# GATB/dsk

Hardware: AMD Instinct MI355X
Metric: distinct k-mers counted/sec (whole node), k=31 (higher is better)
Workload: dtype u64

## Files before the change

### dsk_amd/csrc/dskgpu.hip

```cpp
#include <algorithm>
#include <cstdio>
#include <cstring>
#include <cstdlib>
#include <cmath>
#include <string>
#include <vector>

#include <thread>
#include <system_error>
#include "engine.h"
#include "kernels.h"
#include "superkmer_recv.h"
#include "rawparse.h"

#include <rocprim/device/device_radix_sort.hpp>

#define DSKGPU_VERSION "dskgpu 0.1 (gfx950)"

namespace {

thread_local std::string g_create_err;

__global__ __launch_bounds__(1024) void k_place_probe(unsigned long long* __restrict__ out, unsigned long long n) {
    const unsigned long long per_block = n / gridDim.x, per_stream = per_block / 512;
    unsigned long long* base = out + (unsigned long long)blockIdx.x * per_block;
    const int r = threadIdx.x >> 5, l = threadIdx.x & 31;
    for (unsigned long long off = 0; off + 32 <= per_stream; off += 32)
        for (int p = r; p < 512; p += 32) base[(unsigned long long)p * per_stream + off + l] = off;
}
int g_place_k = -1;
float place_probe_ms(void* p, size_t bytes) {
    hipEvent_t a, b;
    if (hipEventCreate(&a) != hipSuccess || hipEventCreate(&b) != hipSuccess) return 0.f;
    float best = 1e30f;
    for (int i = 0; i < 3; ++i) {
        (void)hipEventRecord(a, 0);
        hipLaunchKernelGGL(k_place_probe, dim3(256), dim3(1024), 0, 0, static_cast<unsigned long long*>(p), (unsigned long long)(bytes / 8));
        (void)hipEventRecord(b, 0);
        (void)hipEventSynchronize(b);
        float ms = 0.f; (void)hipEventElapsedTime(&ms, a, b);
        if (i && ms < best) best = ms;
    }
    (void)hipEventDestroy(a); (void)hipEventDestroy(b);
    return best;
}
}

hipError_t placed_malloc(void** out, size_t bytes) {
    if (g_place_k < 0) { const char* e = getenv("DSKGPU_PLACE"); g_place_k = e ? atoi(e) : 0; }
    size_t free_b = 0, total_b = 0;
    if (g_place_k < 2 || bytes < (size_t(1) << 28) || hipMemGetInfo(&free_b, &total_b) != hipSuccess) return hipMalloc(out, bytes);
    const int K = (int)std::min<size_t>((size_t)g_place_k, free_b / 2 / bytes);
    if (K < 2) return hipMalloc(out, bytes);
    std::vector<void*> cand; std::vector<float> ms;
    for (int i = 0; i < K; ++i) {
        void* q = nullptr;
        if (hipMalloc(&q, bytes) != hipSuccess) { (void)hipGetLastError(); break; }
        static const size_t probe_max = getenv("DSKGPU_PLACE_GB") ? (size_t)(atof(getenv("DSKGPU_PLACE_GB")) * (1ull << 30)) : ~size_t(0);
        cand.push_back(q); ms.push_back(place_probe_ms(q, std::min(bytes, probe_max)));
    }
    if (cand.empty()) return hipErrorOutOfMemory;
    size_t best = 0;
    for (size_t i = 1; i < cand.size(); ++i) if (ms[i] < ms[best]) best = i;
    for (size_t i = 0; i < cand.size(); ++i) if (i != best) (void)hipFree(cand[i]);
    if (getenv("DSKGPU_VERBOSE")) {
        fprintf(stderr, "[dskgpu] placement of %.2f GB: probe ms", bytes * 1e-9);
        for (size_t i = 0; i < cand.size(); ++i) fprintf(stderr, " %.3f%s", ms[i], i == best ? "*" : "");
        fprintf(stderr, "\n");
    }
    *out = cand[best];
    return hipSuccess;
}

namespace {

__global__ void k_gather_back(const u32* __restrict__ sc, const u32* __restrict__ nsolid_total, const u32* __restrict__ nk, const u64* __restrict__ gstats,
                              u64* __restrict__ out) {
    if (threadIdx.x == 0) {
        out[0] = sc[SC_OVERFLOW]; out[1] = *nsolid_total; out[2] = nk ? *nk : 0u; out[3] = sc[SC_OVF2]; out[4] = sc[SC_OVF1]; out[5] = sc[SC_EXT];
        out[6] = gstats[0]; out[7] = gstats[1]; out[8] = gstats[2]; out[9] = gstats[3];
    }
}
struct ScalarSet { u32 v[SC_COUNT]; };
__global__ __launch_bounds__(256) void k_setup_pass(u32* __restrict__ sc, ScalarSet h, u64* __restrict__ ghist, u32 nh, u64* __restrict__ gstats, u32 nstats,
                                                    u32* __restrict__ zero, u64 nzero) {
    const u32 t = blockIdx.x * 256 + threadIdx.x;
    if (t < SC_COUNT) sc[t] = h.v[t];
    if (t < nstats) gstats[t] = 0ull;
    for (u32 i = t; i < nh; i += gridDim.x * 256) ghist[i] = 0ull;
    for (u64 i = t; i < nzero; i += (u64)gridDim.x * 256) zero[i] = 0u;
}
}

namespace {

#define LAND_BYTES (64u << 10)
void* landing(dskgpu_ctx* ctx, size_t bytes) {
    if (bytes > LAND_BYTES) return nullptr;
    if (!ctx->land && hipHostMalloc(reinterpret_cast<void**>(&ctx->land), LAND_BYTES, hipHostMallocDefault) != hipSuccess) { ctx->land = nullptr; (void)hipGetLastError(); }
    return ctx->land;
}

bool sentinel_is_a_kmer(int W, unsigned k) {
    u64 v[4] = {0, 0, 0, 0};
    if (W == 1) v[0] = kunmix(~0ull);
    else if (W == 2) { KN<2> x; x.w[0] = x.w[1] = ~0ull; kunmixN(x); v[0] = x.w[0]; v[1] = x.w[1]; }
    else { KN<4> x; for (int i = 0; i < 4; ++i) x.w[i] = ~0ull; kunmixN(x); for (int i = 0; i < 4; ++i) v[i] = x.w[i]; }
    auto base = [&](const u64* a, unsigned i) { return (unsigned)((a[i >> 5] >> (2 * (i & 31))) & 3u); };
    for (unsigned i = k; i < 128; ++i) if (base(v, i)) return false;
    u64 r[4] = {0, 0, 0, 0};
    for (unsigned i = 0; i < k; ++i) { const unsigned c = base(v, i) ^ 2u, j = k - 1 - i; r[j >> 5] |= (u64)c << (2 * (j & 31)); }
    for (int x = 3; x >= 0; --x) if (v[x] != r[x]) return v[x] < r[x];
    return true;
}


int run_encode(dskgpu_ctx* ctx, const uint8_t* d_bytes, u64 n, u64* nwords_out) {
    const u64 nwords = (n + 31) / 32;
    ctx->enc_fresh = false;
    CK(ctx->packed.ensure((nwords + 1) * 8));
    CK(ctx->inval.ensure((nwords + 1) * 4));
    if (const int rc = encode_into(ctx, d_bytes, n, ctx->packed.as<u64>(), ctx->inval.as<u32>())) return rc;
    *nwords_out = nwords;
    return DSKGPU_OK;
}

}

int encode_current(dskgpu_ctx* ctx, u64* nwords_out) {
    if (ctx->enc_keep) { *nwords_out = (ctx->n_bytes + 31) / 32; ctx->enc_fresh = false; return DSKGPU_OK; }
    if (!ctx->d_reads && ctx->n_bytes) return fail(ctx, DSKGPU_E_STATE, "the reads were released (dskgpu_encode_reads) and their 2-bit form has been overwritten: set the reads again");
    return run_encode(ctx, ctx->d_reads, ctx->n_bytes, nwords_out);
}

int encode_into(dskgpu_ctx* ctx, const uint8_t* d_bytes, u64 n, u64* packed, u32* inval) {
    const u64 nwords = (n + 31) / 32;
    if (!nwords) return DSKGPU_OK;
    const u64 nb = (nwords + 255) / 256;
    const unsigned grid = (unsigned)std::min<u64>(nb, (u64)ctx->num_cu * 16);
    if ((reinterpret_cast<uintptr_t>(d_bytes) & 15) == 0)
        hipLaunchKernelGGL(k_encode<true>, dim3(grid), dim3(256), 0, ctx->stream, d_bytes, n, packed, inval, nwords);
    else
        hipLaunchKernelGGL(k_encode<false>, dim3(grid), dim3(256), 0, ctx->stream, d_bytes, n, packed, inval, nwords);
    CKL("k_encode");
    return DSKGPU_OK;
}

int run_scan(dskgpu_ctx* ctx, u32* a, const u32* d_len, u64 max_len) {
    const u64 nb = std::max<u64>(1, (max_len + SCAN_BLK - 1) / SCAN_BLK);
    CK(ctx->sums.ensure((nb + 1) * 4));
    hipLaunchKernelGGL(k_scan_reduce, dim3((unsigned)nb), dim3(SCAN_NT), 0, ctx->stream, a, d_len, ctx->sums.as<u32>());
    hipLaunchKernelGGL(k_scan_sums, dim3(1), dim3(1024), 0, ctx->stream, ctx->sums.as<u32>(), d_len, a);
    hipLaunchKernelGGL(k_scan_apply, dim3((unsigned)nb), dim3(SCAN_NT), 0, ctx->stream, a, d_len, ctx->sums.as<u32>());
    CKL("k_scan");
    return DSKGPU_OK;
}

int allow_big_lds(dskgpu_ctx* ctx, const void* fn, int bytes) {
    for (const void* f : ctx->big_lds_fns) if (f == fn) return DSKGPU_OK;
    CK(hipFuncSetAttribute(fn, hipFuncAttributeMaxDynamicSharedMemorySize, bytes));
    ctx->big_lds_fns.push_back(fn);
    return DSKGPU_OK;
}

namespace {

size_t scatter_lds(int W, u32 P, bool opt = false) { return (size_t)SC_NT * (16 / W) * 8 * W + (size_t)P * (opt ? 20 : 16) + 4 + 17 * 4 + 16 + (opt ? 8 + L0_MAX_PASSES * 8 : 0); }

template <int W, int SRC, int MODE>
int launch_hist_m(dskgpu_ctx* ctx, const typename KeyT<W>::T* keys, const ChunkDesc* descs, const u32* d_nch,
                  u64 max_chunks, u32* matrix, DigitSpec ds, u32 P) {
    const unsigned grid = (unsigned)std::max<u64>(1, std::min<u64>(max_chunks, (u64)ctx->num_cu));
    hipLaunchKernelGGL((k_hist<W, SRC, MODE>), dim3(grid), dim3(SC_NT), 0, ctx->stream, ctx->packed.as<u64>(),
                       ctx->inval.as<u32>(), keys, descs, d_nch, matrix, (int)ctx->cfg.kmer_size, ds, P);
    CKL("k_hist");
    return DSKGPU_OK;
}
template <int W, int SRC>
int launch_hist(dskgpu_ctx* ctx, const typename KeyT<W>::T* keys, const ChunkDesc* descs, const u32* d_nch,
                u64 max_chunks, u32* matrix, DigitSpec ds, u32 P) {
    const bool mp = ds.mode == 1 && ds.npass > 1;
    if (SRC == 0) return ds.mode == 0 ? launch_hist_m<W, 0, 0>(ctx, keys, descs, d_nch, max_chunks, matrix, ds, P)
                       : mp ? launch_hist_m<W, 0, 3>(ctx, keys, descs, d_nch, max_chunks, matrix, ds, P)
                            : launch_hist_m<W, 0, 1>(ctx, keys, descs, d_nch, max_chunks, matrix, ds, P);
    return ds.mode == 2 ? launch_hist_m<W, 1, 2>(ctx, keys, descs, d_nch, max_chunks, matrix, ds, P)
                   : mp ? launch_hist_m<W, 1, 3>(ctx, keys, descs, d_nch, max_chunks, matrix, ds, P)
                        : launch_hist_m<W, 1, 1>(ctx, keys, descs, d_nch, max_chunks, matrix, ds, P);
}

unsigned scatter_grid(const dskgpu_ctx* ctx, int W, u32 P, u64 max_chunks, bool opt = false) {
    const size_t lds = scatter_lds(W, P, opt);
    const u64 per_cu = std::max<u64>(1, std::min<u64>(2048 / SC_NT, (160 * 1024) / lds));
    return (unsigned)std::max<u64>(1, std::min<u64>(max_chunks, (u64)ctx->num_cu * per_cu));
}
template <int W, int SRC, int MODE, bool OPT = false, bool HEAVY = false>
int launch_scatter_m(dskgpu_ctx* ctx, const typename KeyT<W>::T* keys, const ChunkDesc* descs, const u32* d_nch,
                     u64 max_chunks, const u32* scanned, typename KeyT<W>::T* out, DigitSpec ds, u32 P, Opt1Spec o1 = Opt1Spec{nullptr, 0u, 0u, nullptr, nullptr, 0u, nullptr, nullptr, nullptr, 0u, nullptr, 0ull, {0ull, 0ull, 0ull, 0ull}, 0u}) {
    const size_t lds = scatter_lds(W, P, OPT && !o1.uslice);
    const unsigned grid = scatter_grid(ctx, W, P, max_chunks, OPT && !o1.uslice);
    { const int e = allow_big_lds(ctx, reinterpret_cast<const void*>(&k_scatter<W, SRC, MODE, OPT, HEAVY>)); if (e) return e; }
    hipLaunchKernelGGL((k_scatter<W, SRC, MODE, OPT, HEAVY>), dim3(grid), dim3(SC_NT), lds, ctx->stream, SRC == 2 ? ctx->rec_src : ctx->packed.as<u64>(),
                       SRC == 2 ? nullptr : ctx->inval.as<u32>(), keys, descs, d_nch, scanned, out, (int)ctx->cfg.kmer_size, ds, P, o1);
    CKL("k_scatter");
    return DSKGPU_OK;
}
template <int W, int MODE, bool OPT = false, bool SLICED = false>
int launch_scatter_al(dskgpu_ctx* ctx, const typename KeyT<W>::T* keys, const ChunkDesc* descs, const u32* d_nch,
                      u64 max_chunks, const u32* scanned, typename KeyT<W>::T* out, DigitSpec ds, u32 P, OptSpec os = OptSpec{0u, nullptr, nullptr, nullptr, 0u, 0u, 0ull, 0u, 0u, nullptr, nullptr, nullptr, nullptr, nullptr, nullptr}) {
    const size_t lds = ascatter_lds(W, P);
    const unsigned grid = (unsigned)std::max<u64>(1, std::min<u64>(max_chunks, (u64)ctx->num_cu));
    { const int e = allow_big_lds(ctx, reinterpret_cast<const void*>(&k_scatter_al<W, MODE, OPT, SLICED>)); if (e) return e; }
    hipLaunchKernelGGL((k_scatter_al<W, MODE, OPT, SLICED>), dim3(grid), dim3(SC_NT), lds, ctx->stream, keys, descs, d_nch, scanned, out, ds, P, os);
    CKL("k_scatter_al");
    return DSKGPU_OK;
}

template <int W, int SRC>
int launch_scatter(dskgpu_ctx* ctx, const typename KeyT<W>::T* keys, const ChunkDesc* descs, const u32* d_nch,
                   u64 max_chunks, const u32* scanned, typename KeyT<W>::T* out, DigitSpec ds, u32 P) {
    const bool mp = ds.mode == 1 && ds.npass > 1;
    if (SRC == 1 && ascatter_lds(W, P) <= 160 * 1024 && !ctx->tune.no_aligned)
        return ds.mode == 2 ? launch_scatter_al<W, 2>(ctx, keys, descs, d_nch, max_chunks, scanned, out, ds, P)
                       : mp ? launch_scatter_al<W, 3>(ctx, keys, descs, d_nch, max_chunks, scanned, out, ds, P)
                            : launch_scatter_al<W, 1>(ctx, keys, descs, d_nch, max_chunks, scanned, out, ds, P);
    if (SRC == 0) return ds.mode == 0 ? launch_scatter_m<W, 0, 0>(ctx, keys, descs, d_nch, max_chunks, scanned, out, ds, P)
                       : mp ? launch_scatter_m<W, 0, 3>(ctx, keys, descs, d_nch, max_chunks, scanned, out, ds, P)
                            : launch_scatter_m<W, 0, 1>(ctx, keys, descs, d_nch, max_chunks, scanned, out, ds, P);
    return ds.mode == 2 ? launch_scatter_m<W, 1, 2>(ctx, keys, descs, d_nch, max_chunks, scanned, out, ds, P)
                   : mp ? launch_scatter_m<W, 1, 3>(ctx, keys, descs, d_nch, max_chunks, scanned, out, ds, P)
                        : launch_scatter_m<W, 1, 1>(ctx, keys, descs, d_nch, max_chunks, scanned, out, ds, P);
}

inline void launch_count_impl(dskgpu_ctx* ctx, unsigned grid, u64* keys, u64* solid_keys, u32* solid_ab, u32* ovf, const CountParams& cp) {
    if (cp.cap && cp.cap <= CNT_V3_KEYS * CNT_NT) {
        hipLaunchKernelGGL((k_count1v3<CNT_NT, CNT_KPT, CNT_V3_KEYS>), dim3(grid), dim3(CNT_NT), 0, ctx->stream, keys, solid_keys, solid_ab,
                           ctx->nsolid.as<u32>(), ctx->ghist.as<u64>(), ctx->gstats.as<u64>(), ovf, cp, cp.subcnt);
        return;
    }
    if (cp.cap) hipLaunchKernelGGL(k_count1<true>, dim3(grid), dim3(CNT_NT), 0, ctx->stream, keys, solid_keys, ctx->fstart.as<u32>(), solid_ab,
                                   ctx->nsolid.as<u32>(), ctx->ghist.as<u64>(), ctx->gstats.as<u64>(), ovf, cp, cp.subcnt);
    else hipLaunchKernelGGL(k_count1<false>, dim3(grid), dim3(CNT_NT), 0, ctx->stream, keys, solid_keys, ctx->fstart.as<u32>(), solid_ab,
                            ctx->nsolid.as<u32>(), ctx->ghist.as<u64>(), ctx->gstats.as<u64>(), ovf, cp, (const u32*)ctx->fstart.as<u32>());
}
template <int W>
inline void launch_count_impl(dskgpu_ctx* ctx, unsigned grid, KN<W>* keys, KN<W>* solid_keys, u32* solid_ab, u32* ovf, const CountParams& cp) {
    if constexpr (W == 2) {
        if (cp.cap && cp.cap <= C2V_NKEYS * CNT_NT && !ctx->mw_v3_off) {
            CountParams c2 = cp; c2.maxload = std::min<u32>(cp.maxload, C2V_MAXLOAD);
            hipLaunchKernelGGL((k_count2v3<CNT_NT, C2V_KPT, C2V_NKEYS>), dim3(grid), dim3(CNT_NT), 0, ctx->stream, (const K2*)keys, solid_keys, solid_ab,
                               ctx->nsolid.as<u32>(), ctx->ghist.as<u64>(), ctx->gstats.as<u64>(), ovf, c2, cp.subcnt);
            return;
        }
    }
    if (cp.cap) hipLaunchKernelGGL((k_count_mw<W, true>), dim3(grid), dim3(CNT_NT), 0, ctx->stream, keys, solid_keys, ctx->fstart.as<u32>(), solid_ab,
                                   ctx->nsolid.as<u32>(), ctx->ghist.as<u64>(), ctx->gstats.as<u64>(), ovf, cp);
    else hipLaunchKernelGGL((k_count_mw<W, false>), dim3(grid), dim3(CNT_NT), 0, ctx->stream, keys, solid_keys, ctx->fstart.as<u32>(), solid_ab,
                            ctx->nsolid.as<u32>(), ctx->ghist.as<u64>(), ctx->gstats.as<u64>(), ovf, cp);
}
template <int W>
inline void launch_count(dskgpu_ctx* ctx, unsigned grid, typename KeyT<W>::T* keys, typename KeyT<W>::T* solid_keys, u32* solid_ab, u32* ovf, const CountParams& cp) {
    launch_count_impl(ctx, grid, keys, solid_keys, solid_ab, ovf, cp);
}

struct Plan {
    int levels;
    u32 P1, P2, F;
    DigitSpec d1, d2;
};

#define TARGET_KEYS 2900
#define TARGET_KEYS2 2560
#ifndef TARGET_KEYS4
#define TARGET_KEYS4 640
#endif
#ifndef OPT_GROUPS4
#define OPT_GROUPS4 OPT_GROUPS
#endif
#define MAX_LEVEL_BINS 2048
#define ONE_LEVEL_BINS 1024
#define CH2 65536u
#define OPT_GROUPS 545u
#define OPT_GROUPS2 1023u
inline u32 opt_groups(int W) { return W == 2 ? (AL_G2 == 8 ? 1022u : OPT_GROUPS2) : (W == 1 && AL_G1 == 16) ? 546u : W == 4 ? OPT_GROUPS4 : OPT_GROUPS; }
inline u64 target_keys(int W) { return W == 1 ? TARGET_KEYS : W == 2 ? TARGET_KEYS2 : TARGET_KEYS4; }
#define OPT_CAP 4360u

bool make_plan(u64 n_upper, int extra_bits, int W, u32 num_cu, Plan* pl) {
    const u64 target = target_keys(W);
    u64 F = ((n_upper + target - 1) / target) << extra_bits;
    if (F < 2) F = 2;
    if (F <= ONE_LEVEL_BINS) { pl->levels = 1; pl->P1 = (u32)F; pl->P2 = 1; }
    else {
        u64 p2max = MAX_LEVEL_BINS; while (p2max > 64 && ascatter_lds(W, (u32)p2max) > 160 * 1024) --p2max;
        u64 p1 = 1; while (p1 * p1 < F) ++p1;
        const bool large = F >= (u64)num_cu * 64;
        if (large) {
            p1 = std::max<u64>((F + p2max - 2) / (p2max - 1), num_cu);
            p1 = (p1 + num_cu - 1) / num_cu * num_cu;
            if (p1 > MAX_LEVEL_BINS - 8) p1 = MAX_LEVEL_BINS - 8;
        }
        u64 p2 = (F + p1 - 1) / p1;
        if (p2 % 2 == 0 && p2 + 1 <= p2max) ++p2;
        if (p1 > MAX_LEVEL_BINS || p2 > MAX_LEVEL_BINS) return false;
        pl->levels = 2; pl->P1 = (u32)p1; pl->P2 = (u32)p2;
    }
    pl->F = pl->P1 * pl->P2;
    pl->d1 = DigitSpec{1u, pl->P1, 0u, 1u, 1u, 0u};
    pl->d2 = DigitSpec{2u, pl->P1, pl->P2, 1u, 1u, 0u};
    return true;
}

void build_descs1(dskgpu_ctx* ctx, u64 n_units_total, u64 tile, u64 max_chunks, u32* nch_out) {
    const u64 ntiles = std::max<u64>(1, (n_units_total + tile - 1) / tile);
    u64 nch = std::min<u64>(ntiles, max_chunks);
    const u64 tpc = (ntiles + nch - 1) / nch;
    nch = (ntiles + tpc - 1) / tpc;
    ctx->h_descs1.resize(nch);
    for (u64 c = 0; c < nch; ++c) {
        ChunkDesc d;
        d.begin = c * tpc * tile;
        d.end = std::min<u64>(n_units_total, (c + 1) * tpc * tile);
        if (d.begin > d.end) d.begin = d.end;
        d.flat_base = (u32)c;
        d.stride = (u32)nch;
        ctx->h_descs1[c] = d;
    }
    *nch_out = (u32)nch;
}

void build_descs1_slices(dskgpu_ctx* ctx, u64 tile, u64 max_chunks, u32* nch_out) {
    const size_t S = ctx->rec_slice_end.size();
    ctx->h_descs1.clear(); ctx->h_slice_chunk.assign(S + 1, 0);
    const u64 per_slice = std::max<u64>(1, max_chunks / S);
    u64 rb = 0;
    for (size_t sl = 0; sl < S; ++sl) {
        const u64 re = ctx->rec_slice_end[sl];
        ctx->h_slice_chunk[sl] = (u32)ctx->h_descs1.size();
        if (re > rb) {
            const u64 ntiles = (re - rb + tile - 1) / tile;
            u64 nch = std::min<u64>(ntiles, per_slice);
            const u64 tpc = (ntiles + nch - 1) / nch;
            nch = (ntiles + tpc - 1) / tpc;
            for (u64 c = 0; c < nch; ++c) {
                ChunkDesc d;
                d.begin = rb + c * tpc * tile; d.end = std::min<u64>(re, rb + (c + 1) * tpc * tile);
                d.flat_base = 0; d.stride = 0;
                ctx->h_descs1.push_back(d);
            }
        }
        rb = re;
    }
    ctx->h_slice_chunk[S] = (u32)ctx->h_descs1.size();
    for (auto& d : ctx->h_descs1) d.stride = (u32)ctx->h_descs1.size();
    *nch_out = (u32)ctx->h_descs1.size();
}

#define REC_RESIZE 1001
int rec_gate_upto(dskgpu_ctx* ctx, u32 upto) {
    if (!ctx->rec_gate) return DSKGPU_OK;
    const u32 n = (u32)ctx->rec_slice_end.size();
    for (; ctx->rec_gated < std::min(upto, n); ++ctx->rec_gated)
        if (ctx->rec_gate(ctx->rec_gate_user, ctx->rec_gated) != 0) ctx->rec_gate_failed = true;
    return ctx->rec_gate_failed ? fail(ctx, DSKGPU_E_STATE, "a slice of the exchange did not arrive (the caller's gate failed)") : DSKGPU_OK;
}
int rec_gate_all(dskgpu_ctx* ctx) { return rec_gate_upto(ctx, 0xFFFFFFFFu); }

int sk_sizes(dskgpu_ctx* ctx, u64* total_out) {
    const u64 nrec = ctx->rec_n; const u32 R = ctx->sender.sp.R;
    { const int e = rec_gate_all(ctx); if (e) return e; }
    u64 nch = std::min<u64>((nrec + SKX_NT - 1) / SKX_NT, (u64)ctx->num_cu * 16);
    u64 rpc = (nrec + nch - 1) / nch;
    rpc = (rpc + SKX_NT - 1) / SKX_NT * SKX_NT;
    nch = (nrec + rpc - 1) / rpc;
    if (rpc * SK_MAXN >= 0xFFFFFFFFull) return fail(ctx, DSKGPU_E_ARG, "too many records per chunk");
    CK(ctx->sk_sums.ensure(nch * 4)); CK(ctx->sk_cbase.ensure(nch * 8));
    ctx->h_sk_sums.assign(nch, 0); ctx->h_sk_cbase.assign(nch, 0);
    hipLaunchKernelGGL(k_sk_count, dim3((unsigned)nch), dim3(SKX_NT), 0, ctx->stream, ctx->rec_src, nrec, R, (u32)rpc, ctx->sk_sums.as<u32>());
    CKL("k_sk_count");
    CK(hipMemcpyAsync(ctx->h_sk_sums.data(), ctx->sk_sums.p, nch * 4, hipMemcpyDeviceToHost, ctx->stream));
    CK(hipStreamSynchronize(ctx->stream));
    u64 total = 0;
    for (u64 c = 0; c < nch; ++c) { ctx->h_sk_cbase[c] = total; total += ctx->h_sk_sums[c]; }
    CK(hipMemcpyAsync(ctx->sk_cbase.p, ctx->h_sk_cbase.data(), nch * 8, hipMemcpyHostToDevice, ctx->stream));
    ctx->rec_nch = nch; ctx->rec_rpc = rpc; ctx->rec_sized = true;
    *total_out = total;
    return DSKGPU_OK;
}

template <int W>
int expand_records(dskgpu_ctx* ctx, u64 total) {
    typedef typename KeyT<W>::T Key;
    if (ctx->rec_expanded) return DSKGPU_OK;
    if (!ctx->rec_sized) {
        u64 real = 0;
        const int e = sk_sizes(ctx, &real);
        if (e) return e;
        if (real != total && ctx->rec_hint_est) { ctx->rec_hint = real; return REC_RESIZE; }
        if (real != total) return fail(ctx, DSKGPU_E_ARG, "dskgpu_mg_count_sized: n_kmers does not match the k-mers inside the records");
    }
    { const int e = rec_gate_all(ctx); if (e) return e; }
    CK(ctx->sk_keys.ensure((total + 1) * sizeof(Key)));
    hipLaunchKernelGGL(k_sk_expand<W>, dim3((unsigned)ctx->rec_nch), dim3(SKX_NT), 0, ctx->stream, ctx->rec_src, ctx->rec_n, ctx->sender.sp.R,
                       (int)ctx->cfg.kmer_size, (u32)ctx->rec_rpc, ctx->sk_cbase.as<u64>(), ctx->sk_keys.as<Key>());
    CKL("k_sk_expand");
    ctx->rec_expanded = true;
    ctx->mark("mg_expand");
    return DSKGPU_OK;
}
template <> int expand_records<4>(dskgpu_ctx*, u64) { return DSKGPU_E_STATE; }

template <int W> struct HvLayout { static constexpr size_t keys = 0, counts = (size_t)HV_KEYS * W, rows = (size_t)HV_KEYS * (W + 1), ab = (size_t)HV_KEYS * (2 * W + 1), words = (size_t)HV_KEYS * (2 * W + 2); };
template <int W>
int find_heavy(dskgpu_ctx* ctx, bool from_reads, const typename KeyT<W>::T* d_keys_in, u32 nts, const Plan& pl, std::vector<double>& load, u32* nheavy_out) {
    typedef typename KeyT<W>::T Key;
    struct HK { u64 w[W]; bool operator<(const HK& o) const { for (int x = W - 1; x >= 0; --x) if (w[x] != o.w[x]) return w[x] < o.w[x]; return false; }
                bool operator==(const HK& o) const { for (int x = 0; x < W; ++x) if (w[x] != o.w[x]) return false; return true; } };
    static_assert(sizeof(HK) == sizeof(Key), "host mirror of a device key");
    *nheavy_out = 0;
    const u32 P1 = pl.P1;
    std::vector<double> sorted(load);
    std::nth_element(sorted.begin(), sorted.begin() + P1 / 2, sorted.end());
    const double median = sorted[P1 / 2];
    std::vector<u32> flagged;
    for (u32 b = 0; b < P1; ++b) if (load[b] > 1.2 * median + 4096.0) flagged.push_back(b);
    if (ctx->tune.verbose) fprintf(stderr, "[dskgpu] find_heavy: median load %.0f, %zu bins above 1.2 x\n", median, flagged.size());
    if (flagged.empty()) return DSKGPU_OK;
    std::sort(flagged.begin(), flagged.end(), [&](u32 a, u32 b) { return load[a] > load[b]; });
    if (flagged.size() > HV_SLOTS) flagged.resize(HV_SLOTS);
    ctx->h_hv_lut.assign(P1, 0xFF);
    for (size_t f = 0; f < flagged.size(); ++f) ctx->h_hv_lut[flagged[f]] = (unsigned char)f;
    const size_t nf = flagged.size();
    CK(ctx->hv_lut.ensure(P1));
    const unsigned grid = (unsigned)std::min<u64>(nts, (u64)ctx->num_cu * 2);
    const size_t per_slot = (size_t)grid * HV_BLOCK_KEYS;
    CK(ctx->hv_collect.ensure((size_t)HV_SLOTS * per_slot * sizeof(Key) + (size_t)HV_SLOTS * grid * 4 + HV_SLOTS * 4));
    u32* d_kept = reinterpret_cast<u32*>(ctx->hv_collect.as<Key>() + (size_t)HV_SLOTS * per_slot);
    u32* d_step = d_kept + (size_t)HV_SLOTS * grid;
    ctx->h_hv_step.assign(HV_SLOTS, 1);
    for (size_t f = 0; f < flagged.size(); ++f) ctx->h_hv_step[f] = (u32)std::max<u64>(1, ctx->h_mom[2 * (size_t)flagged[f]] / HV_COLLECT);
    CK(hipMemcpyAsync(ctx->hv_lut.p, ctx->h_hv_lut.data(), P1, hipMemcpyHostToDevice, ctx->stream));
    CK(hipMemcpyAsync(d_step, ctx->h_hv_step.data(), HV_SLOTS * 4, hipMemcpyHostToDevice, ctx->stream));
    u32* sc = ctx->scalars.as<u32>();
    const bool mp = pl.d1.npass > 1;
    auto launch = [&](auto kern) {
        hipLaunchKernelGGL(kern, dim3(grid), dim3(SC_NT), 0, ctx->stream, (const u64*)ctx->packed.as<u64>(), (const u32*)ctx->inval.as<u32>(), d_keys_in,
                           (const ChunkDesc*)ctx->smp_descs.as<ChunkDesc>(), (const u32*)(sc + SC_NCH_S), (int)ctx->cfg.kmer_size, pl.d1, P1,
                           (const unsigned char*)ctx->hv_lut.as<unsigned char>(), d_kept, ctx->hv_collect.as<Key>(), (const u32*)d_step);
    };
    if (from_reads) { if (mp) launch(k_collect_heavy<W, 0, 3>); else launch(k_collect_heavy<W, 0, 1>); }
    else { if (mp) launch(k_collect_heavy<W, 1, 3>); else launch(k_collect_heavy<W, 1, 1>); }
    CKL("k_collect_heavy");
    ctx->h_hv_cnt.resize(nf * grid);
    ctx->h_hv_coll.resize(nf * per_slot * W);
    CK(hipMemcpyAsync(ctx->h_hv_cnt.data(), d_kept, nf * grid * 4, hipMemcpyDeviceToHost, ctx->stream));
    CK(hipMemcpyAsync(ctx->h_hv_coll.data(), ctx->hv_collect.p, nf * per_slot * sizeof(Key), hipMemcpyDeviceToHost, ctx->stream));
    CK(hipStreamSynchronize(ctx->stream));
    struct Cand { double est; HK key; u32 bin; };
    std::vector<Cand> cands;
    for (size_t f = 0; f < nf; ++f) {
        HK* kk = reinterpret_cast<HK*>(ctx->h_hv_coll.data()) + f * per_slot;
        u32 n = 0;
        for (unsigned g = 0; g < grid; ++g) {
            const u32 c = std::min<u32>(ctx->h_hv_cnt[f * grid + g], HV_BLOCK_KEYS);
            for (u32 i = 0; i < c; ++i) kk[n++] = kk[(size_t)g * HV_BLOCK_KEYS + i];
        }
        if (n < 256) continue;
        std::sort(kk, kk + n);
        const u32 bin = flagged[f];
        u32 found = 0;
        for (u32 i = 0; i < n;) {
            u32 j = i + 1;
            while (j < n && kk[j] == kk[i]) ++j;
            if ((u64)(j - i) * 20 >= n) { cands.push_back({load[bin] * (double)(j - i) / (double)n, kk[i], bin}); ++found; }
            i = j;
        }
        if (ctx->tune.verbose) fprintf(stderr, "[dskgpu]   bin %u load %.0f: %u keys collected, %u dominant\n", bin, load[bin], n, found);
    }
    std::sort(cands.begin(), cands.end(), [](const Cand& a, const Cand& b) { return a.est > b.est; });
    if (cands.size() > HV_KEYS) cands.resize(HV_KEYS);
    ctx->h_hv_keys.assign((size_t)HV_KEYS * W, DSK_EMPTY);
    for (size_t x = 0; x < cands.size(); ++x) {
        for (int y = 0; y < W; ++y) ctx->h_hv_keys[x * W + y] = cands[x].key.w[y];
        load[cands[x].bin] -= cands[x].est;
    }
    u32 nheavy = (u32)cands.size();
    if (nheavy) {
        CK(ctx->hv_buf.ensure(HvLayout<W>::words * 8));
        u64* hvb = ctx->hv_buf.as<u64>();
        CK(hipMemsetAsync(hvb + HvLayout<W>::keys, 0xFF, (size_t)HV_KEYS * W * 8, ctx->stream));
        CK(hipMemsetAsync(hvb + HvLayout<W>::counts, 0, HV_KEYS * 8, ctx->stream));
        CK(hipMemcpyAsync(hvb + HvLayout<W>::keys, ctx->h_hv_keys.data(), (size_t)HV_KEYS * W * 8, hipMemcpyHostToDevice, ctx->stream));
    }
    *nheavy_out = nheavy;
    return DSKGPU_OK;
}

template <int W> struct KeySource { bool from_reads, from_rec; const typename KeyT<W>::T* keys; u64 nkeys, nwords; };

template <int W>
struct PassState {
    typedef typename KeyT<W>::T Key;
    KeySource<W>& src;
    u32 pass, npass; u64 cap;
    u64 nvalid;
    u32* sc;
    Plan pl{};
    u32 opt_cap = 0, max_ext = 0; u64 nregions = 0;
    bool opt1 = false; Opt1Spec o1{}; unsigned grid1 = 0;
    u32 nch1 = 0, nheavy = 0;
    std::vector<double> load, spread;
    Key* fkeys = nullptr;
    DevBuf* scratch = nullptr;
    Key* solid_keys = nullptr; u32* solid_ab = nullptr;
    u32 flags = 0, nsolid = 0, nkeys = 0, ovf2 = 0, ovf1 = 0, ext = 0; u64 stats[4] = {0, 0, 0, 0};
    bool too_big = false; u64 rows = 0;
};

template <int W>
int upload_descs1(dskgpu_ctx* ctx, PassState<W>& ps) {
    const KeySource<W>& src = ps.src;
    const u64 max_chunks1 = (u64)ctx->num_cu * 8;
    if (src.from_reads) build_descs1(ctx, src.nwords, Tile<W>::WORDS, max_chunks1, &ps.nch1);
    else if (src.from_rec && ctx->rec_slice_end.size() > 1) build_descs1_slices(ctx, RecTile<W>::NR, max_chunks1, &ps.nch1);
    else if (src.from_rec) build_descs1(ctx, ctx->rec_n, RecTile<W>::NR, max_chunks1, &ps.nch1);
    else build_descs1(ctx, src.nkeys, Tile<W>::KEYS, max_chunks1, &ps.nch1);
    CK(ctx->descs1.ensure(ctx->h_descs1.size() * sizeof(ChunkDesc)));
    CK(hipMemcpyAsync(ctx->descs1.p, ctx->h_descs1.data(), ctx->h_descs1.size() * sizeof(ChunkDesc), hipMemcpyHostToDevice, ctx->stream));
    return DSKGPU_OK;
}

template <int W>
int records_to_keys(dskgpu_ctx* ctx, PassState<W>& ps) {
    const int e = expand_records<W>(ctx, ps.src.nkeys);
    if (e) return e;
    ps.src.keys = ctx->sk_keys.template as<typename KeyT<W>::T>(); ps.src.from_rec = false;
    return upload_descs1(ctx, ps);
}

template <class Hist>
int positional_sample(dskgpu_ctx* ctx, u64 units, u64 tile, u32 P, Hist&& hist, u64* ntiles_out, u64* nts_out, u64* stot_out) {
    u32* sc = ctx->scalars.as<u32>();
    const u64 ntiles = std::max<u64>(1, (units + tile - 1) / tile);
    const u64 nts = std::min<u64>(ntiles, 1024);
    ctx->h_descs_s.resize(nts);
    for (u64 i = 0; i < nts; ++i) {
        const u64 t = i * ntiles / nts;
        ChunkDesc d; d.begin = t * tile; d.end = std::min<u64>(units, (t + 1) * tile); d.flat_base = (u32)i; d.stride = (u32)nts;
        ctx->h_descs_s[i] = d;
    }
    const u64 Ms = (u64)P * nts;
    CK(ctx->smp_descs.ensure(nts * sizeof(ChunkDesc)));
    CK(ctx->smp_mat.ensure((Ms + 4) * 4 + (size_t)P * 16));
    CK(hipMemcpyAsync(ctx->smp_descs.p, ctx->h_descs_s.data(), nts * sizeof(ChunkDesc), hipMemcpyHostToDevice, ctx->stream));
    ctx->h_sc[SC_NCH_S] = (u32)nts;
    CK(hipMemcpyAsync(sc + SC_NCH_S, &ctx->h_sc[SC_NCH_S], 4, hipMemcpyHostToDevice, ctx->stream));
    { const int e = hist(ctx->smp_descs.as<ChunkDesc>(), (const u32*)(sc + SC_NCH_S), nts, ctx->smp_mat.as<u32>()); if (e) return e; }
    u64* mom = reinterpret_cast<u64*>(ctx->smp_mat.as<u32>() + ((Ms + 2) & ~(u64)1));
    hipLaunchKernelGGL(k_bin_moments, dim3((P + 3) / 4), dim3(256), 0, ctx->stream, (const u32*)ctx->smp_mat.as<u32>(), (u32)nts, P, mom);
    CKL("k_bin_moments");
    ctx->h_mom.resize((size_t)P * 2);
    void* lz = landing(ctx, (size_t)P * 16);
    CK(hipMemcpyAsync(lz ? lz : (void*)ctx->h_mom.data(), mom, (size_t)P * 16, hipMemcpyDeviceToHost, ctx->stream));
    CK(hipStreamSynchronize(ctx->stream));
    if (lz) std::memcpy(ctx->h_mom.data(), lz, (size_t)P * 16);
    u64 stot = 0;
    for (u32 b = 0; b < P; ++b) stot += ctx->h_mom[2 * b];
    *ntiles_out = ntiles; *nts_out = nts; *stot_out = stot;
    return DSKGPU_OK;
}

template <int W>
int pass_plan(dskgpu_ctx* ctx, PassState<W>& ps, int extra_bits) {
    typedef typename KeyT<W>::T Key;
    Plan& pl = ps.pl;
    const u64 plan_n = (ps.src.from_reads && ctx->have_nvalid) ? std::min<u64>(ps.cap, ps.npass == 1 ? ps.nvalid + 1 : ps.nvalid / ps.npass + ps.nvalid / ps.npass / 50 + 4096) : ps.cap;
    if (!make_plan(plan_n, extra_bits, W, (u32)ctx->num_cu, &pl))
        return fail(ctx, DSKGPU_E_OVERFLOW, "cannot partition finer (table overflow persists)");
    pl.d1.world = pl.d2.world = ctx->cfg.world_size; pl.d1.npass = pl.d2.npass = ps.npass; pl.d1.pass = pl.d2.pass = ps.pass;
    pl.d1.ones_is_key = pl.d2.ones_is_key = ctx->sentinel_ok ? 0u : 1u;
    { const int e = upload_descs1(ctx, ps); if (e) return e; }
    if (pl.levels == 2 && ctx->sentinel_ok && !ctx->opt2_off && !ctx->tune.no_opt2 && ascatter_lds(W, pl.P2) <= 160 * 1024)
        ps.opt_cap = opt_groups(W) * (8u / W);
    if (ps.opt_cap && ctx->tune.opt_cap) ps.opt_cap = ctx->tune.opt_cap;
    if (W > 1 && (u64)pl.F * ps.opt_cap >= 0xFFFF0000ull) ps.opt_cap = 0;
    const u32 opt_cap = ps.opt_cap;
    if (opt_cap && W <= 2) {
        u64 want = std::min<u64>((u64)pl.F / 8 + 4096, 0x7FFFFFFFull / opt_cap - 1);
        if (ctx->tune.max_ext >= 0) want = (u64)ctx->tune.max_ext;
        if (W > 1) { const u64 room = 0xFFFF0000ull / opt_cap; want = room > (u64)pl.F + 1 ? std::min<u64>(want, room - pl.F - 1) : 0; }
        ps.max_ext = (u32)want;
    }
    ps.nregions = (u64)pl.F + ps.max_ext;
    if (!opt_cap) { CK(ctx->bufA.ensure((ps.cap + 1) * sizeof(Key))); CK(ctx->bufB.ensure((ps.cap + 1) * sizeof(Key))); }
    if (opt_cap) {
        const u64 slots = (u64)pl.F * opt_cap + ATile<W>::KEYS + 16;
        CK(ctx->bufA.ensure(std::max<u64>(W == 1 ? slots * 4 : slots * sizeof(Key), (ps.cap + 1) * sizeof(Key))));
        if (W > 1) CK(ctx->abund2.ensure(slots * 4));
    }
    ps.opt1 = opt_cap && !ctx->opt1_off && !ctx->tune.no_opt1 && (ps.npass == 1 || ps.src.from_reads || W <= 2);
    if (ps.src.from_rec && (!ps.opt1 || W > 2 || ctx->tune.no_recsrc)) { const int e = records_to_keys(ctx, ps); if (e) return e; }
    if (ps.opt1 && scatter_lds(W, pl.P1, false) > 160 * 1024) ps.opt1 = false;
    return DSKGPU_OK;
}

template <int W>
int pass_layout1(dskgpu_ctx* ctx, PassState<W>& ps) {
    typedef typename KeyT<W>::T Key;
    const KeySource<W>& src = ps.src;
    const Plan& pl = ps.pl;
    Opt1Spec& o1 = ps.o1;
    o1 = Opt1Spec{nullptr, 0u, 0u, ps.sc + SC_OVF1, nullptr, ctx->sender.sp.R, ctx->gstats.as<u64>() + 2, nullptr, nullptr, 0u, nullptr, 0ull, {0ull, 0ull, 0ull, 0ull}, 0u};
    const bool uniform1 = scatter_lds(W, pl.P1, true) > 160 * 1024;
    if (ps.opt1) {
        const u32 nch1 = ps.nch1;
        const unsigned grid1 = ps.grid1 = scatter_grid(ctx, W, pl.P1, nch1, !uniform1);
        const u64 cpb = (nch1 + grid1 - 1) / grid1;
        double share = (double)cpb / (double)nch1;
        if (src.from_rec && ctx->rec_slice_end.size() > 1) {
            share = 0.0;
            u64 rb = 0;
            for (size_t sl = 0; sl < ctx->rec_slice_end.size(); ++sl) {
                const u64 re = ctx->rec_slice_end[sl], nc = ctx->h_slice_chunk[sl + 1] - ctx->h_slice_chunk[sl];
                if (nc) share += (double)((nc + grid1 - 1) / grid1) / (double)nc * (double)(re - rb) / (double)ctx->rec_n;
                rb = re;
            }
        }
        const double pass_keys = (double)(ps.nvalid / ps.npass);
        ps.load.assign(pl.P1, pass_keys / pl.P1);
        ps.spread.assign(pl.P1, 0.0);
        bool sampled = false;
        const Key* d_keys_s = src.keys;
        double smp_density = 1.0;
        bool rec_sample_ok = ctx->sentinel_ok;
        u64 rec_units = 0;
        if constexpr (W <= 2) {
          if (src.from_rec && !ctx->tune.no_sample && !uniform1) {
            const u64 nrec_s = ctx->rec_slice_end.size() > 1 ? ctx->rec_slice_end[0] : ctx->rec_n;
            const u64 NR = RecTile<W>::NR;
            const u64 nchk_all = (nrec_s + NR - 1) / NR;
            const u64 nchk = std::min<u64>(nchk_all, 256);
            if (nchk == 0) rec_sample_ok = false;
            else {
                { const int e = rec_gate_upto(ctx, 1); if (e) return e; }
                std::vector<u64>& cbeg = ctx->h_cbeg;
                cbeg.resize(nchk);
                for (u64 i = 0; i < nchk; ++i) cbeg[i] = (i * nchk_all / nchk) * NR;
                rec_units = nchk * NR * SK_MAXN;
                CK(ctx->smp_keys.ensure(rec_units * sizeof(Key) + nchk * 8 + 64));
                u64* d_cbeg = reinterpret_cast<u64*>(ctx->smp_keys.as<char>() + rec_units * sizeof(Key));
                CK(hipMemcpyAsync(d_cbeg, cbeg.data(), nchk * 8, hipMemcpyHostToDevice, ctx->stream));
                hipLaunchKernelGGL(k_sk_sample_keys<W>, dim3((unsigned)nchk), dim3(SKX_NT), 0, ctx->stream, ctx->rec_src, ctx->rec_n, ctx->sender.sp.R, (int)ctx->cfg.kmer_size,
                                   (const u64*)d_cbeg, (u32)NR, ctx->smp_keys.as<Key>());
                CKL("k_sk_sample_keys");
                d_keys_s = ctx->smp_keys.as<Key>();
            }
          }
        }
        const bool smp_rec = src.from_rec && rec_units != 0;
        if ((!src.from_rec || smp_rec) && rec_sample_ok && !ctx->tune.no_sample && !uniform1) {
            const u64 units = src.from_reads ? src.nwords : smp_rec ? rec_units : src.nkeys, tile = src.from_reads ? Tile<W>::WORDS : Tile<W>::KEYS;
            auto hist = [&](const ChunkDesc* dd, const u32* d_nch, u64 n, u32* mat) {
                return src.from_reads ? launch_hist<W, 0>(ctx, nullptr, dd, d_nch, n, mat, pl.d1, pl.P1) : launch_hist<W, 1>(ctx, d_keys_s, dd, d_nch, n, mat, pl.d1, pl.P1);
            };
            u64 ntiles = 0, nts = 0, stot = 0;
            { const int e = positional_sample(ctx, units, tile, pl.P1, hist, &ntiles, &nts, &stot); if (e) return e; }
            if (stot >= (u64)pl.P1 * 64) {
                const double scale = (src.from_reads && ps.npass > 1) ? (double)ntiles / (double)nts : pass_keys / (double)stot;
                if (smp_rec) smp_density = std::max(0.05, (double)stot / ((double)nts * (double)Tile<W>::KEYS));
                const double tiles_per_block = smp_rec ? pass_keys * share / (double)Tile<W>::KEYS : (double)ntiles * share;
                for (u32 b = 0; b < pl.P1; ++b) {
                    const double sum = (double)ctx->h_mom[2 * b], sq = (double)ctx->h_mom[2 * b + 1];
                    const double mean = sum / (double)nts, var = std::max(mean, sq / (double)nts - mean * mean);
                    ps.load[b] = sum * scale;
                    ps.spread[b] = 5.0 * std::sqrt(tiles_per_block * var / smp_density) + 4.0 * std::sqrt((double)nts * var) * scale * share;
                }
                sampled = true;
            }
            if constexpr (W <= 2) {
                if (sampled && ps.opt_cap && !ctx->tune.no_heavy) { const int e = find_heavy<W>(ctx, src.from_reads, d_keys_s, (u32)nts, pl, ps.load, &ps.nheavy); if (e) return e; }
            }
            ctx->mark("sample1");
        }
        ctx->h_boff.resize(pl.P1 + 1);
        u64 area = 0;
        if (uniform1) o1.uslice = 1u;
        for (u32 b = 0; b < pl.P1; ++b) {
            double sl = ps.load[b] * share;
            const double few = (src.from_rec && share * (double)nch1 < 16.0) ? 0.08 : 0.0;
            sl += sampled ? ps.spread[b] + sl * 0.01 + 64.0 : sl * (0.06 + few) + 160.0;
            u64 slice = ((u64)sl + 8) & ~7ull;
            if (uniform1) o1.uslice = (u32)slice;
            if (ctx->tune.opt_slice) slice = ctx->tune.opt_slice;
            ctx->h_boff[b] = (u32)std::min<u64>(area, 0xFFFFFFFFull); area += slice;
        }
        ctx->h_boff[pl.P1] = (u32)std::min<u64>(area, 0xFFFFFFFFull);
        const u64 tail = 2 * Tile<W>::KEYS;
        const u64 cells = (u64)pl.P1 * grid1;
        if (ctx->tune.verbose) fprintf(stderr, "[dskgpu] pass %u/%u: P1 %u P2 %u, %u level-1 blocks, area %llu keys per block (%.2f GB of slices), sampled %d, keys %llu, %u chunks, share %.6f, %zu slices\n", ps.pass, ps.npass, pl.P1, pl.P2, grid1,
                                       (unsigned long long)area, (double)area * grid1 * sizeof(Key) * 1e-9, (int)sampled, (unsigned long long)ps.nvalid, nch1, share, ctx->rec_slice_end.size());
        if (area < 8 || area * grid1 + tail >= 0xFFFF0000ull) ps.opt1 = false;
        else {
            o1.area = (u32)area; o1.dump = (u32)(area * grid1);
            CK(ctx->boff.ensure(((size_t)pl.P1 + 1) * 4));
            CK(hipMemcpyAsync(ctx->boff.p, ctx->h_boff.data(), ((size_t)pl.P1 + 1) * 4, hipMemcpyHostToDevice, ctx->stream));
            o1.boff = ctx->boff.as<u32>();
            CK(ctx->mat1.ensure((cells + 1) * 4));
            o1.fill = ctx->mat1.as<u32>();
            if (grid1 + 1 > SLICED_MAX) ps.opt1 = false;
            CK(ctx->bufA.ensure((area * grid1 + tail + 1) * sizeof(Key)));
        }
    }
    if (src.from_rec && !ps.opt1) { const int e = records_to_keys(ctx, ps); if (e) return e; }
    return DSKGPU_OK;
}

template <int W, int SRC, int MODE, bool HEAVY>
int scatter1_m(dskgpu_ctx* ctx, const PassState<W>& ps, const ChunkDesc* dd1, const u32* d_nch) {
    return launch_scatter_m<W, SRC, MODE, true, HEAVY>(ctx, SRC == 1 ? ps.src.keys : nullptr, dd1, d_nch, ps.nch1, nullptr, ctx->bufA.template as<typename KeyT<W>::T>(),
                                                       ps.pl.d1, ps.pl.P1, ps.o1);
}
template <int W>
int launch_scatter1(dskgpu_ctx* ctx, const PassState<W>& ps, const ChunkDesc* dd1, const u32* d_nch) {
    const bool mp = ps.npass > 1, heavy = ps.nheavy != 0, rec = ps.src.from_rec, reads = ps.src.from_reads;
    if constexpr (W <= 2) {
        if (rec && heavy) return mp ? scatter1_m<W, 2, 3, true>(ctx, ps, dd1, d_nch) : scatter1_m<W, 2, 1, true>(ctx, ps, dd1, d_nch);
        if (rec) return mp ? scatter1_m<W, 2, 3, false>(ctx, ps, dd1, d_nch) : scatter1_m<W, 2, 1, false>(ctx, ps, dd1, d_nch);
        if (heavy && reads) return mp ? scatter1_m<W, 0, 3, true>(ctx, ps, dd1, d_nch) : scatter1_m<W, 0, 1, true>(ctx, ps, dd1, d_nch);
        if (heavy) return mp ? scatter1_m<W, 1, 3, true>(ctx, ps, dd1, d_nch) : scatter1_m<W, 1, 1, true>(ctx, ps, dd1, d_nch);
        if (!reads && mp) return scatter1_m<W, 1, 3, false>(ctx, ps, dd1, d_nch);
    } else if (rec || heavy || (!reads && mp)) return DSKGPU_E_STATE;
    if (reads) return mp ? scatter1_m<W, 0, 3, false>(ctx, ps, dd1, d_nch) : scatter1_m<W, 0, 1, false>(ctx, ps, dd1, d_nch);
    return scatter1_m<W, 1, 1, false>(ctx, ps, dd1, d_nch);
}

template <int W>
int pass_scatter1(dskgpu_ctx* ctx, PassState<W>& ps) {
    typedef typename KeyT<W>::T Key;
    const KeySource<W>& src = ps.src;
    const Plan& pl = ps.pl;
    const u32 nch1 = ps.nch1;
    const u64 M1 = (u64)pl.P1 * nch1;
    u32* h_sc = ctx->h_sc;
    std::memset(h_sc, 0, sizeof(ctx->h_sc));
    h_sc[SC_NCH1] = nch1; h_sc[SC_MLEN1] = (u32)M1; h_sc[SC_F] = pl.F;
    if (ps.opt1) h_sc[SC_NCH2] = pl.P1;
    h_sc[SC_WORK2] = (u32)std::min<u64>(pl.P1, (u64)ctx->num_cu);
    {
        static_assert(sizeof(ctx->h_sc) == sizeof(ScalarSet), "scalar block");
        ScalarSet hs; std::memcpy(hs.v, h_sc, sizeof hs.v);
        const u32 nh = ctx->cfg.histo_max + 1;
        u64 nzero = 0;
        if (pl.levels == 2 && ps.opt_cap) { nzero = ps.nregions + 1; CK(ctx->mat2.ensure((size_t)nzero * 4)); }
        const u64 work = std::max<u64>(nh, nzero);
        hipLaunchKernelGGL(k_setup_pass, dim3((unsigned)std::min<u64>(1024, (work + 255) / 256)), dim3(256), 0, ctx->stream, ps.sc, hs, ctx->ghist.as<u64>(), nh, ctx->gstats.as<u64>(), 4u,
                           nzero ? ctx->mat2.as<u32>() : (u32*)nullptr, nzero);
        CKL("k_setup_pass");
    }
    ctx->mark("setup");
    int rc;
    const ChunkDesc* dd1 = ctx->descs1.as<ChunkDesc>();
    if (ps.opt1) {
        Opt1Spec& o1 = ps.o1;
        if constexpr (W <= 2) { if (ps.nheavy) { o1.hv_keys = ctx->hv_buf.as<u64>() + HvLayout<W>::keys; o1.hv_cnt = reinterpret_cast<unsigned long long*>(ctx->hv_buf.as<u64>() + HvLayout<W>::counts); } }
        if (src.from_rec && ctx->rec_slice_end.size() > 1) {
            const size_t S = ctx->rec_slice_end.size();
            CK(ctx->cur_state.ensure((size_t)ps.grid1 * pl.P1 * 4));
            o1.cur_state = ctx->cur_state.as<u32>();
            rc = DSKGPU_OK;
            for (size_t sl = 0; sl < S && rc == DSKGPU_OK; ++sl) {
                if ((rc = rec_gate_upto(ctx, (u32)sl + 1))) break;
                o1.g0 = ctx->h_slice_chunk[sl]; o1.gn = ctx->h_slice_chunk[sl + 1] - ctx->h_slice_chunk[sl];
                o1.resume = sl > 0 ? 1u : 0u; o1.last = sl + 1 == S ? 1u : 0u;
                rc = launch_scatter1<W>(ctx, ps, dd1, ps.sc + SC_NCH1);
            }
        }
        else if (src.from_rec) { if (!(rc = rec_gate_all(ctx))) rc = launch_scatter1<W>(ctx, ps, dd1, ps.sc + SC_NCH1); }
        else rc = launch_scatter1<W>(ctx, ps, dd1, ps.sc + SC_NCH1);
        if (rc) return rc;
        ctx->mark("scatter1");
        return DSKGPU_OK;
    }
    CK(ctx->mat1.ensure((M1 + 1) * 4));
    if (src.from_reads) rc = launch_hist<W, 0>(ctx, nullptr, dd1, ps.sc + SC_NCH1, nch1, ctx->mat1.as<u32>(), pl.d1, pl.P1);
    else rc = launch_hist<W, 1>(ctx, src.keys, dd1, ps.sc + SC_NCH1, nch1, ctx->mat1.as<u32>(), pl.d1, pl.P1);
    if (rc) return rc;
    ctx->mark("hist1");
    if ((rc = run_scan(ctx, ctx->mat1.as<u32>(), ps.sc + SC_MLEN1, M1))) return rc;
    ctx->mark("scan1");
    if (ps.npass > 1) {
        CK(hipMemcpyAsync(&ps.nkeys, ctx->mat1.as<u32>() + M1, 4, hipMemcpyDeviceToHost, ctx->stream));
        CK(hipStreamSynchronize(ctx->stream));
        if ((u64)ps.nkeys > ps.cap) { ps.too_big = true; return DSKGPU_OK; }
    }
    if (src.from_reads) rc = launch_scatter<W, 0>(ctx, nullptr, dd1, ps.sc + SC_NCH1, nch1, ctx->mat1.as<u32>(), ctx->bufA.as<Key>(), pl.d1, pl.P1);
    else rc = launch_scatter<W, 1>(ctx, src.keys, dd1, ps.sc + SC_NCH1, nch1, ctx->mat1.as<u32>(), ctx->bufA.as<Key>(), pl.d1, pl.P1);
    if (rc) return rc;
    ctx->mark("scatter1");
    return DSKGPU_OK;
}

template <int W>
int pass_scatter2(dskgpu_ctx* ctx, PassState<W>& ps) {
    const Plan& pl = ps.pl;
    int rc;
    ps.fkeys = ctx->bufA.as<typename KeyT<W>::T>();
    ps.scratch = &ctx->bufB;
    CK(ctx->fstart.ensure(((size_t)pl.F + 2) * 4));
    CK(ctx->nsolid.ensure(((size_t)pl.F + 2) * 4));
    if (pl.levels == 2 && ps.opt_cap) {
        CK(ctx->bufB.ensure((ps.nregions * ps.opt_cap + ATile<W>::KEYS + 16) * sizeof(typename KeyT<W>::T)));
        CK(ctx->descs2.ensure(((size_t)pl.P1 * 2 + 1) * sizeof(ChunkDesc)));
        CK(ctx->seg.ensure((size_t)pl.P1 * sizeof(SegInfo)));
        CK(ctx->mat2.ensure(((size_t)ps.nregions + 1) * 4));
        CK(ctx->chain_next.ensure(((size_t)ps.nregions + 1 + ps.max_ext + 1) * 4));
        if (ps.opt1) {
            ctx->h_descs2.resize(pl.P1);
            std::vector<u32> order(pl.P1);
            for (u32 sgm = 0; sgm < pl.P1; ++sgm) order[sgm] = sgm;
            double mean_work = 0.0; for (double w : ps.load) mean_work += w; mean_work = std::max(1.0, mean_work / pl.P1);
            auto wclass = [&](u32 a) { return (long long)(ps.load[a] / (0.05 * mean_work)); };
            std::stable_sort(order.begin(), order.end(), [&](u32 a, u32 b) { return wclass(a) > wclass(b); });
            for (u32 i = 0; i < pl.P1; ++i) {
                const u32 sgm = order[i];
                ChunkDesc d; d.begin = ctx->h_boff[sgm]; d.end = ctx->h_boff[sgm + 1]; d.flat_base = sgm * pl.P2; d.stride = 1;
                ctx->h_descs2[i] = d;
            }
            CK(hipMemcpyAsync(ctx->descs2.p, ctx->h_descs2.data(), (size_t)pl.P1 * sizeof(ChunkDesc), hipMemcpyHostToDevice, ctx->stream));
        } else {
            hipLaunchKernelGGL(k_plan, dim3(1), dim3(1024), 0, ctx->stream, ctx->mat1.as<u32>(), ps.nch1, pl.P1, 0x7FFFFFFFu, pl.P2,
                               ctx->seg.as<SegInfo>(), ctx->descs2.as<ChunkDesc>(), ps.sc + SC_NCH2, ps.sc + SC_MLEN2, 1u);
            CKL("k_plan");
        }
        ctx->mark("plan2");
        OptSpec os{ps.opt_cap, ctx->mat2.as<u32>(), ps.sc + SC_OVF2, ps.opt1 ? ps.o1.fill : nullptr, 0u, ps.grid1, (u64)ps.o1.area,
                   pl.F, ps.max_ext, ctx->chain_next.as<u32>(), ps.sc + SC_EXT, ctx->chain_next.as<u32>() + ps.nregions + 1, ps.sc + SC_NCHAINED,
                   ps.sc + SC_WORK2, nullptr};
        if (ctx->tune.verbose && ps.opt1) { CK(ctx->dbg.ensure((size_t)pl.P1 * 24)); os.dbg = ctx->dbg.as<unsigned long long>(); }
        if (ps.opt1) rc = launch_scatter_al<W, 2, true, true>(ctx, ctx->bufA.as<typename KeyT<W>::T>(), ctx->descs2.as<ChunkDesc>(), ps.sc + SC_NCH2, (u64)pl.P1 * 2, nullptr,
                                                              ctx->bufB.as<typename KeyT<W>::T>(), pl.d2, pl.P2, os);
        else rc = launch_scatter_al<W, 2, true, false>(ctx, ctx->bufA.as<typename KeyT<W>::T>(), ctx->descs2.as<ChunkDesc>(), ps.sc + SC_NCH2, (u64)pl.P1 * 2, nullptr,
                                                       ctx->bufB.as<typename KeyT<W>::T>(), pl.d2, pl.P2, os);
        if (rc) return rc;
        ctx->mark("scatter2");
        if (ctx->tune.verbose && ps.opt1) {
            std::vector<unsigned long long> t((size_t)pl.P1 * 3);
            CK(hipMemcpyAsync(t.data(), ctx->dbg.p, t.size() * 8, hipMemcpyDeviceToHost, ctx->stream));
            CK(hipStreamSynchronize(ctx->stream));
            unsigned long long t0 = ~0ull, t1 = 0; for (u32 i = 0; i < pl.P1; ++i) { t0 = std::min(t0, t[3 * i]); t1 = std::max(t1, t[3 * i + 1]); }
            fprintf(stderr, "[dskgpu] level 2: %u segments, %.3f ms first start -> last end\n", pl.P1, (t1 - t0) * 1e-5);
            for (u32 i = 0; i < pl.P1; ++i)
                if (i < 6 || i + 3 >= pl.P1 || t[3 * i + 1] + 20000 > t1)
                    fprintf(stderr, "[dskgpu]   desc %u (segment %u, load %.0f) block %llu: %.3f .. %.3f ms\n", i, (u32)(ctx->h_descs2[i].flat_base / pl.P2),
                            ps.load[ctx->h_descs2[i].flat_base / pl.P2], t[3 * i + 2], (t[3 * i] - t0) * 1e-5, (t[3 * i + 1] - t0) * 1e-5);
        }
        ps.fkeys = ctx->bufB.as<typename KeyT<W>::T>();
        ps.scratch = &ctx->bufA;
    } else if (pl.levels == 2) {
        const u64 max_chunks2 = ps.cap / CH2 + pl.P1 + 1;
        const u64 M2 = max_chunks2 * pl.P2;
        if (M2 >= 0xFFFFFFFFull) return fail(ctx, DSKGPU_E_ARG, "level-2 matrix too large");
        CK(ctx->descs2.ensure(max_chunks2 * sizeof(ChunkDesc)));
        CK(ctx->seg.ensure((size_t)pl.P1 * sizeof(SegInfo)));
        CK(ctx->mat2.ensure((M2 + 1) * 4));
        hipLaunchKernelGGL(k_plan, dim3(1), dim3(1024), 0, ctx->stream, ctx->mat1.as<u32>(), ps.nch1, pl.P1, CH2, pl.P2,
                           ctx->seg.as<SegInfo>(), ctx->descs2.as<ChunkDesc>(), ps.sc + SC_NCH2, ps.sc + SC_MLEN2, 0u);
        CKL("k_plan");
        ctx->mark("plan2");
        const ChunkDesc* dd2 = ctx->descs2.as<ChunkDesc>();
        if ((rc = launch_hist<W, 1>(ctx, ctx->bufA.as<typename KeyT<W>::T>(), dd2, ps.sc + SC_NCH2, max_chunks2, ctx->mat2.as<u32>(), pl.d2, pl.P2))) return rc;
        ctx->mark("hist2");
        if ((rc = run_scan(ctx, ctx->mat2.as<u32>(), ps.sc + SC_MLEN2, M2))) return rc;
        ctx->mark("scan2");
        if ((rc = launch_scatter<W, 1>(ctx, ctx->bufA.as<typename KeyT<W>::T>(), dd2, ps.sc + SC_NCH2, max_chunks2, ctx->mat2.as<u32>(), ctx->bufB.as<typename KeyT<W>::T>(), pl.d2, pl.P2))) return rc;
        ctx->mark("scatter2");
        ps.fkeys = ctx->bufB.as<typename KeyT<W>::T>();
        ps.scratch = &ctx->bufA;
        hipLaunchKernelGGL(k_final_offsets, dim3((pl.F + 256) / 256), dim3(256), 0, ctx->stream, ctx->mat2.as<u32>(),
                           ctx->seg.as<SegInfo>(), pl.P2, 0u, ps.sc + SC_MLEN2, ctx->fstart.as<u32>(), pl.F);
    } else {
        hipLaunchKernelGGL(k_final_offsets, dim3((pl.F + 256) / 256), dim3(256), 0, ctx->stream, ctx->mat1.as<u32>(),
                           (const SegInfo*)nullptr, pl.P1, ps.nch1, ps.sc + SC_MLEN1, ctx->fstart.as<u32>(), pl.F);
    }
    CKL("k_final_offsets");
    ctx->mark("offsets");
    return DSKGPU_OK;
}

template <int W>
int count_and_sizes(dskgpu_ctx* ctx, PassState<W>& ps, const CountParams& cp) {
    typedef typename KeyT<W>::T Key;
    const Plan& pl = ps.pl;
    const unsigned cgrid = (unsigned)std::min<u64>(pl.F, (u64)ctx->num_cu * 2);
    launch_count<W>(ctx, cgrid, ps.fkeys, ps.solid_keys, ps.solid_ab, ps.sc + SC_OVERFLOW, cp);
    CKL("k_count");
    if constexpr (W <= 2) {
        if (ps.opt_cap && ps.max_ext) {
            auto kern = [] { if constexpr (W == 1) return k_count_chained; else return k_count_chained_mw<2>; }();
            hipLaunchKernelGGL(kern, dim3((unsigned)std::min<u64>(ps.max_ext, (u64)ctx->num_cu * 2)), dim3(CNT_NT), 0, ctx->stream, ps.fkeys, ps.solid_keys, ps.solid_ab,
                               ctx->nsolid.as<u32>(), ctx->ghist.as<u64>(), ctx->gstats.as<u64>(), ps.sc + SC_OVERFLOW, cp, (const u32*)cp.subcnt,
                               (const u32*)ctx->chain_next.as<u32>(), (const u32*)(ctx->chain_next.as<u32>() + ps.nregions + 1), (const u32*)(ps.sc + SC_NCHAINED), ps.max_ext);
            CKL(W == 1 ? "k_count_chained" : "k_count_chained_mw");
        }
        if (ps.nheavy) {
            const u32 slots = HV_KEYS;
            u64* hvb = ctx->hv_buf.as<u64>();
            hipLaunchKernelGGL(k_heavy_rows<W>, dim3((slots + 255) / 256), dim3(256), 0, ctx->stream, reinterpret_cast<const Key*>(hvb + HvLayout<W>::keys),
                               (const unsigned long long*)(hvb + HvLayout<W>::counts), slots, cp.amin, cp.amax, cp.histo_max, ctx->ghist.as<u64>(), ctx->gstats.as<u64>(),
                               hvb + HvLayout<W>::rows, reinterpret_cast<u32*>(hvb + HvLayout<W>::ab));
            CKL("k_heavy_rows");
        }
    }
    ctx->mark("count");
    if (int e = run_scan(ctx, ctx->nsolid.as<u32>(), ps.sc + SC_F, pl.F)) return e;
    ctx->mark("scan_solid");
    CK(ctx->back_dev.ensure(16 * 8));
    if (!ctx->back_host) CK(hipHostMalloc(reinterpret_cast<void**>(&ctx->back_host), 16 * 8, hipHostMallocDefault));
    const u32* nkp = ps.opt1 ? nullptr : (ps.opt_cap ? ctx->mat1.as<u32>() + (u64)pl.P1 * ps.nch1 : ctx->fstart.as<u32>() + pl.F);
    hipLaunchKernelGGL(k_gather_back, dim3(1), dim3(64), 0, ctx->stream, (const u32*)ps.sc, (const u32*)(ctx->nsolid.as<u32>() + pl.F), nkp,
                       (const u64*)ctx->gstats.as<u64>(), ctx->back_dev.as<u64>());
    CKL("k_gather_back");
    CK(hipMemcpyAsync(ctx->back_host, ctx->back_dev.p, 10 * 8, hipMemcpyDeviceToHost, ctx->stream));
    CK(hipStreamSynchronize(ctx->stream));
    const u64* bh = ctx->back_host;
    ps.flags = (u32)bh[0]; ps.nsolid = (u32)bh[1]; if (!ps.opt1) ps.nkeys = (u32)bh[2];
    ps.ovf2 = (u32)bh[3]; ps.ovf1 = (u32)bh[4]; ps.ext = (u32)bh[5];
    for (int x = 0; x < 4; ++x) ps.stats[x] = bh[6 + x];
    return DSKGPU_OK;
}

template <int W>
int pass_count(dskgpu_ctx* ctx, PassState<W>& ps) {
    CountParams cp;
    cp.F = ps.pl.F;
    cp.maxload = W == 1 ? CNT_MAXLOAD : C2_MAXLOAD;
    if (ctx->tune.table_maxload) cp.maxload = std::min<u32>(cp.maxload, ctx->tune.table_maxload);
    cp.amin = ctx->cfg.abundance_min; cp.amax = ctx->cfg.abundance_max; cp.histo_max = ctx->cfg.histo_max;
    cp.cap = ps.opt_cap; cp.subcnt = ps.opt_cap ? ctx->mat2.as<u32>() : nullptr;
    ps.solid_keys = W == 1 ? ps.fkeys : ps.scratch->template as<typename KeyT<W>::T>();
    ps.solid_ab = W == 1 ? ps.scratch->template as<u32>() : ctx->abund2.as<u32>();
    if constexpr (W == 2) CK(hipMemcpyAsync(ctx->gstats.as<u64>() + 3, ctx->gstats.as<u64>() + 2, 8, hipMemcpyDeviceToDevice, ctx->stream));
    if (int e = count_and_sizes<W>(ctx, ps, cp)) return e;
    if constexpr (W == 2) {
        if ((ps.flags & (CNT_OVF_VERIFY | CNT_OVF_SENTINEL)) && !((ps.opt_cap && ps.ovf2) || (ps.opt1 && ps.ovf1))) {
            if (ctx->tune.verbose) fprintf(stderr, "[dskgpu] pass %u/%u: the top-word table met k-mers it cannot tell apart (flags %u): counting again with k_count_mw\n", ps.pass, ps.npass, ps.flags);
            ctx->mw_v3_off = true;
            ctx->stats.n_retries += 1;
            CK(hipMemsetAsync(ctx->ghist.p, 0, ((size_t)ctx->cfg.histo_max + 1) * 8, ctx->stream));
            CK(hipMemsetAsync(ctx->gstats.p, 0, 2 * 8, ctx->stream));
            CK(hipMemcpyAsync(ctx->gstats.as<u64>() + 2, ctx->gstats.as<u64>() + 3, 8, hipMemcpyDeviceToDevice, ctx->stream));
            CK(hipMemsetAsync(ps.sc + SC_OVERFLOW, 0, 4, ctx->stream));
            if (int e = count_and_sizes<W>(ctx, ps, cp)) return e;
        }
    }
    if (ps.opt1) ps.nkeys = (u32)ps.stats[2];
    return DSKGPU_OK;
}

template <int W>
SparseRows sparse_rows(dskgpu_ctx* ctx, const PassState<W>& ps, const RowsOut& ro, const u32* rows_ab, u32 n_tail) {
    SparseRows r;
    r.W = W; r.keys = ps.solid_keys; r.ab = (const u32*)ps.solid_ab; r.soff = ctx->nsolid.as<u32>(); r.fstart = ctx->fstart.as<u32>(); r.cap = ps.opt_cap; r.F = ps.pl.F;
    r.n_sparse = ps.nsolid; r.n_tail = W <= 2 ? n_tail : 0u;
    if (r.n_tail) { for (int x = 0; x < W; ++x) r.tail_w.w[x] = ro.w[x] + r.n_sparse; r.tail_ab = rows_ab + r.n_sparse; }
    return r;
}

template <int W>
int pass_rows(dskgpu_ctx* ctx, PassState<W>& ps) {
    typedef typename KeyT<W>::T Key;
    const Plan& pl = ps.pl;
    const u32 h_nsolid = ps.nsolid;
    const u64 nhs = ps.nheavy ? ps.stats[1] : 0;
    const u64 ns = ps.rows = h_nsolid + nhs;
    const bool to_sink = ctx->sink.active && ctx->sink.rows + ns + 1 <= ctx->sink.cap;
    RowsOut ro{};
    u32* rows_ab = nullptr;
    if (to_sink) {
        rows_ab = ctx->sink.ab + ctx->sink.rows;
        for (int x = 0; x < W; ++x) ro.w[x] = ctx->sink.w[x] + ctx->sink.rows;
        ctx->sink.took = true;
    } else {
        CK(ctx->out_ab.ensure((ns + 1) * 4));
        rows_ab = ctx->out_ab.as<u32>();
        for (int x = 0; x < W; ++x) { CK(ctx->out_w[x].ensure((ns + 1) * 8)); ro.w[x] = ctx->out_w[x].as<u64>(); }
    }
    if constexpr (W <= 2) {
      if (nhs) {
        for (int x = 0; x < W; ++x)
            CK(hipMemcpyAsync(ro.w[x] + h_nsolid, ctx->hv_buf.as<u64>() + HvLayout<W>::rows + (size_t)x * HV_KEYS, nhs * 8, hipMemcpyDeviceToDevice, ctx->stream));
        CK(hipMemcpyAsync(rows_ab + h_nsolid, ctx->hv_buf.as<u64>() + HvLayout<W>::ab, nhs * 4, hipMemcpyDeviceToDevice, ctx->stream));
      }
    }
    ctx->stats.n_heavy += ps.nheavy;
    bool sparse_sort = false;
    if constexpr (W <= 2) {
        sparse_sort = ps.npass == 1 && ctx->job_passes == 1 && ns > 0 && ns <= rs_max_rows(ctx) && !(ctx->cfg.flags & DSKGPU_F_NO_SORT) &&
                      !ctx->tune.rs_slab_rows && !ctx->bank_job.active && (W == 1 || 2u * ctx->cfg.kmer_size > 64u);
    } else {
        sparse_sort = (ctx->cfg.flags & DSKGPU_F_PARTITION_ORDER) && ps.npass == 1 && ctx->job_passes == 1 && ns > 0 && ns < 0xFFFF0000ull &&
                      !(ctx->cfg.flags & DSKGPU_F_NO_SORT) && !ctx->tune.rs_slab_rows && !ctx->bank_job.active;
    }
    if (sparse_sort) ctx->sp_rows = sparse_rows<W>(ctx, ps, ro, rows_ab, (u32)nhs);
    PartPasses& mp = ctx->rs.mp;
    bool mp_part = false;
    {
        mp_part = !sparse_sort && ctx->job_passes > 1 && mp.ok && ns > 0 && h_nsolid < 0xFFFF0000ull && (W == 1 || 2u * ctx->cfg.kmer_size > 64u);
        if (!sparse_sort && ctx->job_passes > 1 && ns > 0 && !mp_part) mp.ok = false;
        if (mp_part) {
            const SparseRows rows = sparse_rows<W>(ctx, ps, ro, rows_ab, (u32)nhs);
            if (mp.part_off.ensure_keep(((size_t)mp.off_used + part_sort_nparts(rows) + 2) * 4, (size_t)mp.off_used * 4, ctx->stream)) return fail(ctx, DSKGPU_E_NOMEM, "partition offsets");
            u32 np = 0;
            if (const int prc = launch_part_sort(ctx, rows, ro, rows_ab, mp.part_off.as<u32>() + mp.off_used, mp.flag.as<u32>(), &np)) return prc;
            mp.passes.push_back(PartPasses::Pass{mp.row_base, np, mp.off_used});
            mp.off_used += np + 1;
        }
    }
    if (!sparse_sort && !mp_part) {
        hipLaunchKernelGGL(k_compact<W>, dim3((pl.F + 3) / 4), dim3(256), 0, ctx->stream, (const Key*)ps.solid_keys, (const u32*)ps.solid_ab,
                           ctx->fstart.as<u32>(), ctx->nsolid.as<u32>(), pl.F, ro, rows_ab, ps.opt_cap);
        CKL("k_compact");
    }
    ctx->mark("compact");
    ctx->stats.n_ext_regions += std::min<u32>(ps.ext, ps.max_ext);
    return DSKGPU_OK;
}

struct PassResult { u64 rows = 0, kmers = 0, distinct = 0, keys_seen = 0; Plan plan{}; bool too_big = false; };

template <int W>
int run_one_pass(dskgpu_ctx* ctx, bool from_reads, const typename KeyT<W>::T* d_keys_in, u64 nkeys_in, u64 nwords,
                 u32 pass, u32 npass, u64 cap, PassResult* res) {
    ctx->take_sparse_rows();
    KeySource<W> src{from_reads, !from_reads && d_keys_in == nullptr, d_keys_in, nkeys_in, nwords};
    const u64 nvalid = from_reads ? ctx->h_nvalid : nkeys_in;
    int extra_bits = 0, table_retries = 0;
    for (;;) {
        PassState<W> ps{src, pass, npass, cap, nvalid, ctx->scalars.as<u32>()};
        int e;
        if ((e = pass_plan<W>(ctx, ps, extra_bits)) || (e = pass_layout1<W>(ctx, ps)) || (e = pass_scatter1<W>(ctx, ps))) return e;
        if (ps.too_big) { ctx->resolve_marks(); res->too_big = true; res->keys_seen = ps.nkeys; return DSKGPU_OK; }
        if ((e = pass_scatter2<W>(ctx, ps)) || (e = pass_count<W>(ctx, ps))) return e;
        const bool ovf1 = ps.opt1 && ps.ovf1, ovf2 = ps.opt_cap && ps.ovf2;
        if (ovf1 || ovf2) {
            ctx->resolve_marks();
            if (ctx->tune.verbose) fprintf(stderr, "[dskgpu] pass %u/%u: %s overflowed: the exact path takes over\n", pass, npass, ovf1 ? "a level-1 slice" : "the level-2 extension pool");
            if (ovf1) ctx->opt1_off = true;
            else { ctx->opt2_off = true; ctx->opt1_off = true; }
            ctx->stats.n_retries += 1;
            ctx->mark("start");
            continue;
        }
        if (ps.flags & 1u) {
            ctx->resolve_marks();
            if (table_retries >= 3) return fail(ctx, DSKGPU_E_OVERFLOW, "hash table overflow after 3 retries");
            ++table_retries; extra_bits += 1;
            ctx->stats.n_retries += 1;
            ctx->mark("start");
            continue;
        }
        if ((e = pass_rows<W>(ctx, ps))) return e;
        res->rows = ps.rows; res->kmers = res->keys_seen = ps.nkeys; res->distinct = ps.stats[0]; res->plan = ps.pl;
        return DSKGPU_OK;
    }
}

int level0_materialise(dskgpu_ctx* ctx, u64 nwords, u32 lo, u32 npass, u64 reserve_bytes, u32* G_out, u64 (&region_keys)[L0_MAX_PASSES], u64 (&obase)[L0_MAX_PASSES]) {
    *G_out = 0;
    const u64 nper = ctx->h_nvalid / npass + 1;
    u32 nch1 = 0;
    build_descs1(ctx, nwords, Tile<1>::WORDS, (u64)ctx->num_cu * 8, &nch1);
    const unsigned grid = (unsigned)std::max<u64>(1, std::min<u64>(nch1, (u64)ctx->num_cu));
    const u64 cpb = (nch1 + grid - 1) / grid;
    const double share = (double)cpb / (double)nch1;
    const u64 tail = 2 * Tile<1>::KEYS;
    const u64 uslice = (((u64)((double)nper * share * 1.02) + 4096) + 7) & ~7ull;
    const u64 uregion = uslice * grid + tail;
    if (uregion >= 0xFFFF0000ull) return DSKGPU_OK;
    size_t free_b = 0, total_b = 0;
    CK(hipMemGetInfo(&free_b, &total_b));
    const u64 have = ctx->bufA.cap + ctx->bufB.cap + ctx->l0buf.cap;
    const u64 need = nper * 30ull + (4ull << 30) + reserve_bytes;
    const u64 room = free_b + have > need ? free_b + have - need : 0;
    u32 G = (u32)std::min<u64>(std::min<u64>(L0_MAX_PASSES, npass - lo), room / (uregion * 8));
    if (ctx->tune.l0_passes) G = std::min<u32>(std::min<u32>(ctx->tune.l0_passes, L0_MAX_PASSES), npass - lo);
    if (G < 2 && !(ctx->tune.l0_passes)) return DSKGPU_OK;
    if (G == 0) return DSKGPU_OK;
    CK(ctx->descs1.ensure(ctx->h_descs1.size() * sizeof(ChunkDesc)));
    CK(hipMemcpyAsync(ctx->descs1.p, ctx->h_descs1.data(), ctx->h_descs1.size() * sizeof(ChunkDesc), hipMemcpyHostToDevice, ctx->stream));
    u32* sc = ctx->scalars.as<u32>();
    DigitSpec ds{4u, G, 0u, ctx->cfg.world_size, npass, lo};
    std::vector<u64> slice(G, uslice);
    if (!ctx->tune.no_sample) {
        auto hist = [&](const ChunkDesc* dd, const u32* d_nch, u64 n, u32* mat) { return launch_hist_m<1, 0, 4>(ctx, nullptr, dd, d_nch, n, mat, ds, G); };
        u64 ntiles = 0, nts = 0, stot = 0;
        { const int e = positional_sample(ctx, nwords, Tile<1>::WORDS, G, hist, &ntiles, &nts, &stot); if (e) return e; }
        if (stot >= (u64)G * 4096) {
            const double scale = (double)ntiles / (double)nts, tiles_per_block = (double)ntiles * share;
            for (u32 b = 0; b < G; ++b) {
                const double sum = (double)ctx->h_mom[2 * b], sq = (double)ctx->h_mom[2 * b + 1];
                const double mean = sum / (double)nts, var = std::max(mean, sq / (double)nts - mean * mean);
                const double sl = sum * scale * share * 1.01 + 5.0 * std::sqrt(tiles_per_block * var) + 4.0 * std::sqrt((double)nts * var) * scale * share + 64.0;
                slice[b] = ((u64)sl + 8) & ~7ull;
            }
        }
        ctx->mark("sample0");
    }
    for (;;) {
        u64 tot = 0; bool ok = true;
        for (u32 b = 0; b < G; ++b) { const u64 region = slice[b] * grid + tail; if (region >= 0xFFFF0000ull) ok = false; obase[b] = tot; region_keys[b] = slice[b] * grid; tot += region; }
        if (ok && (tot * 8 <= room || ctx->tune.l0_passes)) { CK(ctx->l0buf.ensure(tot * 8 + 64)); break; }
        if (--G < 2) return DSKGPU_OK;
    }
    ds.pa = G;
    ctx->h_sc[SC_NCH1] = nch1; ctx->h_sc[SC_OVF1] = 0;
    CK(hipMemcpyAsync(sc + SC_NCH1, &ctx->h_sc[SC_NCH1], 4, hipMemcpyHostToDevice, ctx->stream));
    CK(hipMemsetAsync(sc + SC_OVF1, 0, 4, ctx->stream));
    ctx->h_boff.assign(L0_MAX_PASSES + 1 + 3 + 2 * L0_MAX_PASSES, 0);
    u64 hob[L0_MAX_PASSES];
    for (u32 i = 0; i < L0_MAX_PASSES; ++i) { ctx->h_boff[i] = (u32)slice[std::min(i, G - 1)]; hob[i] = obase[std::min(i, G - 1)]; }
    std::memcpy(&ctx->h_boff[L0_MAX_PASSES + 4], hob, sizeof hob);
    CK(ctx->boff.ensure(ctx->h_boff.size() * 4));
    CK(hipMemcpyAsync(ctx->boff.p, ctx->h_boff.data(), ctx->h_boff.size() * 4, hipMemcpyHostToDevice, ctx->stream));
    const u32* d_slen = ctx->boff.as<u32>();
    const u64* d_obase = reinterpret_cast<const u64*>(ctx->boff.as<u32>() + L0_MAX_PASSES + 4);
    hipLaunchKernelGGL(k_level0, dim3(grid), dim3(SC_NT), 0, ctx->stream, (const u64*)ctx->packed.as<u64>(), (const u32*)ctx->inval.as<u32>(), (const ChunkDesc*)ctx->descs1.as<ChunkDesc>(),
                       (const u32*)(sc + SC_NCH1), ctx->l0buf.as<u64>(), (int)ctx->cfg.kmer_size, ds, G, d_slen, d_obase, sc + SC_OVF1);
    CKL("k_level0");
    ctx->mark("level0");
    CK(hipMemcpyAsync(&ctx->h_ovf1, sc + SC_OVF1, 4, hipMemcpyDeviceToHost, ctx->stream));
    CK(hipStreamSynchronize(ctx->stream));
    if (ctx->tune.verbose) {
        u64 tot = 0; for (u32 b = 0; b < G; ++b) tot += region_keys[b];
        fprintf(stderr, "[dskgpu] level 0: passes %u..%u of %u materialised, %.2f GB in all (%.2f GB free before)%s\n", lo, lo + G - 1, npass, (double)tot * 8e-9, (double)free_b * 1e-9,
                ctx->h_ovf1 ? " -- a slice overflowed: these passes read the reads" : "");
    }
    if (ctx->h_ovf1) return DSKGPU_OK;
    *G_out = G;
    return DSKGPU_OK;
}

template <int W>
int run_pipeline(dskgpu_ctx* ctx, bool from_reads, const typename KeyT<W>::T* d_keys_in, u64 nkeys_in) {
    typedef typename KeyT<W>::T Key;
    ctx->drop_result();
    ctx->sink = dskgpu_ctx::RowSink{};
    if (from_reads) { ctx->st_names.clear(); ctx->st_ms.clear(); }
    ctx->marks.clear(); ctx->ev_used = 0;
    const u64 n_upper = from_reads ? ctx->n_bytes : nkeys_in;
    u64 nwords = 0;
    ctx->mark("start");
    if (from_reads) {
        int rc = encode_current(ctx, &nwords);
        if (rc) return rc;
        ctx->mark("encode");
    }
    CK(ctx->scalars.ensure(SC_COUNT * 4));
    CK(ctx->ghist.ensure(((size_t)ctx->cfg.histo_max + 1 + 2) * 8));
    CK(ctx->gstats.ensure(4 * 8));
    ctx->have_nvalid = false;
    if (from_reads && nwords) {
        CK(hipMemsetAsync(ctx->gstats.p, 0, 4 * 8, ctx->stream));
        hipLaunchKernelGGL(k_count_valid, dim3((unsigned)std::min<u64>((nwords + 255) / 256, (u64)ctx->num_cu * 8)), dim3(256), 0, ctx->stream,
                           ctx->inval.as<u32>(), nwords, (int)ctx->cfg.kmer_size, ctx->gstats.as<u64>() + 3);
        CKL("k_count_valid");
        {
            void* lz = landing(ctx, 8);
            CK(hipMemcpyAsync(lz ? lz : (void*)&ctx->h_nvalid, ctx->gstats.as<u64>() + 3, 8, hipMemcpyDeviceToHost, ctx->stream));
            CK(hipStreamSynchronize(ctx->stream));
            if (lz) std::memcpy(&ctx->h_nvalid, lz, 8);
        }
        ctx->have_nvalid = true;
    }
    const u64 max_keys = ctx->max_keys_per_pass ? ctx->max_keys_per_pass : 0xD0000000ull;
    const u64 n_keys = (from_reads && ctx->have_nvalid) ? std::max<u64>(1, ctx->h_nvalid) : n_upper;
    u64 pass_keys = max_keys;
    if (W == 1 && from_reads && ctx->have_nvalid && n_keys > max_keys && !ctx->max_keys_per_pass && !ctx->tune.no_level0)
        pass_keys = ctx->tune.mp_pass_mkeys ? (u64)ctx->tune.mp_pass_mkeys * 1000000ull : 1000000000ull;
    const u64 hard_max = W == 2 && !ctx->max_keys_per_pass ? std::min<u64>(max_keys, 2400000000ull) : max_keys;
    u32 npass = (u32)std::max<u64>(1, (n_keys + pass_keys - 1) / pass_keys);
    bool rec_l0 = W <= 2 && from_reads && ctx->have_nvalid && ctx->sk_mode && ctx->cfg.world_size == 1 && !ctx->tune.no_level0 && !ctx->tune.l0_keys && !ctx->rec_l0_off &&
                  (npass > 1 || n_keys > hard_max);
    RecL0 rl;
    if (rec_l0) {
        ctx->sender.prepared = false; ctx->enc_fresh = false;
        u64 want = ctx->max_keys_per_pass ? max_keys : ctx->tune.mp_pass_mkeys ? (u64)ctx->tune.mp_pass_mkeys * 1000000ull : (W == 1 ? 1200000000ull : 1000000000ull);
        u64 G = (n_keys + want - 1) / want;
        if (G < 2) G = 2;
        if (G > SK_MAX_OWNERS) G = SK_MAX_OWNERS;
        if (n_keys / G + n_keys / G / 7 > hard_max && !ctx->max_keys_per_pass) rec_l0 = false;
        else {
            const int rc = rec_l0_prepare(ctx, ctx->l0_sender, nwords, (u32)G, &rl);
            if (rc == REC_L0_NO) rec_l0 = false; else if (rc) return rc;
            else npass = (u32)G;
        }
    }
    u64 cap_floor = 0;
    for (;;) {
        if (npass > 4096) return fail(ctx, DSKGPU_E_OVERFLOW, "too many passes (one k-mer alone exceeds a pass)");
        const u64 cap = npass == 1 ? n_upper : std::min<u64>(n_upper, std::max<u64>(cap_floor, n_keys / npass + n_keys / npass / 16 + (1u << 20)));
        if (cap >= 0xFFFF0000ull) { npass *= 2; cap_floor = 0; continue; }
        if (W > 1) CK(ctx->abund2.ensure((cap + 1) * 4));
        ctx->hist.assign((size_t)ctx->cfg.histo_max + 1, 0);
        std::vector<u64> pass_hist(ctx->hist.size());
        u64 tot_rows = 0, tot_kmers = 0, tot_distinct = 0;
        Plan pl{};
        bool too_big = false; u64 seen = 0;
        u32 l0_lo = 0, l0_n = 0; u64 l0_keys[L0_MAX_PASSES] = {0}; u64 l0_base[L0_MAX_PASSES] = {0};
        bool l0_try = W == 1 && from_reads && npass > 1 && ctx->have_nvalid && !ctx->tune.no_level0 && !rec_l0;
        u32 r_hi = 0; u64 r_base[SK_MAX_OWNERS] = {0};
        bool restart = false;
        u64 sweeps = 0;
        bool rows_sized = false;
        ctx->job_passes = npass;
        PartPasses& mp = ctx->rs.mp;
        mp.passes.clear(); mp.off_used = 0;
        mp.ok = npass > 1 && (ctx->cfg.flags & DSKGPU_F_PARTITION_ORDER) && !(ctx->cfg.flags & DSKGPU_F_NO_SORT) && !ctx->bank_job.active;
        if (mp.ok) { CK(mp.flag.ensure(256)); CK(hipMemsetAsync(mp.flag.p, 0, 4, ctx->stream)); }
        for (u32 p = 0; p < npass; ++p) {
            PassResult r{};
            r.plan = pl;
            int rc;
            mp.row_base = tot_rows;
            ctx->sink = dskgpu_ctx::RowSink{};
            if (npass > 1 && rows_sized) {
                ctx->sink.active = true; ctx->sink.rows = tot_rows; ctx->sink.ab = ctx->acc_ab.as<u32>();
                u64 cap_rows = ctx->acc_ab.cap / 4;
                for (int x = 0; x < W; ++x) { ctx->sink.w[x] = ctx->acc_w[x].as<u64>(); cap_rows = std::min<u64>(cap_rows, ctx->acc_w[x].cap / 8); }
                ctx->sink.cap = cap_rows;
            }
            if (npass > 1) { ctx->opt1_off = false; ctx->opt2_off = false; ctx->mw_v3_off = false; }
            if (rec_l0) {
                if (p >= r_hi) {
                    size_t free_b = 0, total_b = 0;
                    CK(hipMemGetInfo(&free_b, &total_b));
                    const u64 nper = n_keys / npass + 1;
                    const u64 have = ctx->bufA.cap + ctx->bufB.cap + ctx->l0buf.cap;
                    const u64 rows_have = ctx->acc_ab.cap + ctx->acc_w[0].cap + (W > 1 ? ctx->acc_w[1].cap : 0);
                    const u64 rows_want = rows_sized ? 0 : n_keys / 16 * (8ull * W + 4);
                    const u64 need = nper * (W == 1 ? 30ull : 50ull) + (4ull << 30) + (rows_want > rows_have ? rows_want - rows_have : 0);
                    const u64 room = free_b + have > need ? free_b + have - need : 0;
                    const u64 R8 = (u64)ctx->l0_sender.sp.R * 8;
                    u64 left = 0; for (u32 o = p; o < npass; ++o) left += rl.region[o] * R8;
                    const u64 nsw = std::max<u64>(1, (left + std::max<u64>(room, 1) - 1) / std::max<u64>(room, 1));
                    const u64 target = (left + nsw - 1) / nsw;
                    u64 acc = 0; u32 hi = p;
                    while (hi < npass && (hi == p || (acc + rl.region[hi] * R8 <= room && acc < target))) { acc += rl.region[hi] * R8; ++hi; }
// ... 254 lines not shown
                   (ctx->cfg.flags & DSKGPU_F_HISTO2D) ? 1u : 0u};
    u64 n_solid = 0;
    if (nu) {
        RowsIn ri{}; RowsOut ro{};
        for (int x = 0; x < W; ++x) ri.w[x] = ctx->s_w[x].as<u64>();
        hipLaunchKernelGGL(k_merge_banks<W>, dim3(gb), dim3(256), 0, ctx->stream, ri,
                           ctx->s_val.as<u64>(), nu, mp, ctx->m_flag.as<u32>(), ctx->m_sum.as<u32>(), ctx->ghist.as<u64>(), ctx->gh2d.as<u64>(), ctx->gstats.as<u64>());
        hipLaunchKernelGGL(k_copy_u32, dim3(gb), dim3(256), 0, ctx->stream, ctx->m_pos.as<u32>(), ctx->m_flag.as<u32>(), nu);
        CKL("k_merge_banks");
        ctx->h_sc[SC_F] = (u32)nu;
        CK(hipMemcpyAsync(ctx->scalars.as<u32>() + SC_F, &ctx->h_sc[SC_F], 4, hipMemcpyHostToDevice, ctx->stream));
        if ((rc = run_scan(ctx, ctx->m_pos.as<u32>(), ctx->scalars.as<u32>() + SC_F, nu))) return rc;
        CK(hipMemcpyAsync(&ctx->h_back[1], ctx->m_pos.as<u32>() + nu, 4, hipMemcpyDeviceToHost, ctx->stream));
        CK(hipStreamSynchronize(ctx->stream));
        n_solid = ctx->h_back[1];
        CK(ctx->out_ab.ensure((n_solid + 1) * 4));
        for (int x = 0; x < W; ++x) { CK(ctx->out_w[x].ensure((n_solid + 1) * 8)); ro.w[x] = ctx->out_w[x].as<u64>(); }
        hipLaunchKernelGGL(k_pick_rows<W>, dim3(gb), dim3(256), 0, ctx->stream, ri,
                           ctx->m_sum.as<u32>(), ctx->m_flag.as<u32>(), ctx->m_pos.as<u32>(), nu, ro, ctx->out_ab.as<u32>());
        CKL("k_pick_rows");
    }
    ctx->hist.assign(nh, 0); ctx->hist2d.assign(nh * 11, 0);
    CK(hipMemcpyAsync(ctx->hist.data(), ctx->ghist.p, nh * 8, hipMemcpyDeviceToHost, ctx->stream));
    CK(hipMemcpyAsync(ctx->hist2d.data(), ctx->gh2d.p, nh * 11 * 8, hipMemcpyDeviceToHost, ctx->stream));
    CK(hipMemcpyAsync(&ctx->h_stats[0], ctx->gstats.p, 32, hipMemcpyDeviceToHost, ctx->stream));
    CK(hipStreamSynchronize(ctx->stream));
    for (int x = 0; x < 4; ++x) ctx->res_w[x] = x < W ? ctx->out_w[x].as<u64>() : nullptr;
    ctx->res_ab = ctx->out_ab.as<u32>();
    ctx->n_rows = n_solid;
    ctx->stats.n_bytes = total; ctx->stats.n_kmers = tot_kmers; ctx->stats.n_distinct = ctx->h_stats[0]; ctx->stats.n_solid = n_solid;
    ctx->stats.n_passes = passes; ctx->stats.n_retries = retries;
    ctx->stats.n_partitions = ctx->cfg.nb_partitions ? ctx->cfg.nb_partitions : 4u;
    ctx->have_result = true;
    return DSKGPU_OK;
}
template <int W>
int run_banks(dskgpu_ctx* ctx) {
    int rc = banks_begin(ctx);
    if (rc) return rc;
    const u32 B = (u32)ctx->bank_job.ends.size();
    for (u32 b = 0; b < B; ++b) {
        banks_select(ctx, b);
        if ((rc = run_pipeline<W>(ctx, true, nullptr, 0)) || (rc = banks_add<W>(ctx, b))) { banks_abort(ctx); return rc; }
    }
    return banks_finish<W>(ctx);
}

}

__attribute__((visibility("hidden"))) bool dskgpu_i_per_bank(dskgpu_ctx* ctx) {
    const bool banks = ctx->bank_ends.size() > 1 || (!ctx->bank_ends.empty() && ctx->bank_ends.back() < ctx->n_bytes);
    return banks && (ctx->cfg.solidity_kind != DSKGPU_SOLIDITY_SUM || (ctx->cfg.flags & DSKGPU_F_HISTO2D));
}
__attribute__((visibility("hidden"))) uint32_t dskgpu_i_banks(dskgpu_ctx* ctx) { return banks_of(ctx); }
__attribute__((visibility("hidden"))) int dskgpu_i_banks_begin(dskgpu_ctx* ctx) { return banks_begin(ctx); }
__attribute__((visibility("hidden"))) void dskgpu_i_banks_select(dskgpu_ctx* ctx, uint32_t b) { banks_select(ctx, b); }
__attribute__((visibility("hidden"))) void dskgpu_i_banks_abort(dskgpu_ctx* ctx) { banks_abort(ctx); }
__attribute__((visibility("hidden"))) int dskgpu_i_banks_add(dskgpu_ctx* ctx, uint32_t b) {
    return ctx->W == 1 ? banks_add<1>(ctx, b) : ctx->W == 2 ? banks_add<2>(ctx, b) : banks_add<4>(ctx, b);
}
__attribute__((visibility("hidden"))) int dskgpu_i_banks_finish(dskgpu_ctx* ctx) {
    return ctx->W == 1 ? banks_finish<1>(ctx) : ctx->W == 2 ? banks_finish<2>(ctx) : banks_finish<4>(ctx);
}

static_assert(((size_t)32 << 20) / RP_BLOCK <= (size_t)RP_NT * RP_SCAN_PER, "k_rp_scan walks the block summaries of one staging piece (PIN_CHUNK) with RP_SCAN_PER per thread");
template <int FMT>
static void launch_raw_chunk(dskgpu_ctx* ctx, u32 n, uint8_t* out) {
    const u32 nb = (n + RP_BLOCK - 1) / RP_BLOCK;
    const unsigned char* in = ctx->raw_in.as<unsigned char>();
    RawState* st = ctx->raw_state.as<RawState>();
    hipLaunchKernelGGL((k_rp_count<FMT>), dim3(nb), dim3(RP_NT), 0, ctx->stream, in, n, ctx->raw_blk.as<RpBlock>());
    hipLaunchKernelGGL((k_rp_scan<FMT>), dim3(1), dim3(RP_NT), 0, ctx->stream, in, n, nb, ctx->raw_blk.as<RpBlock>(), st,
                       ctx->raw_boff.as<unsigned long long>(), ctx->raw_bstate.as<u32>(), out);
    hipLaunchKernelGGL((k_rp_write<FMT>), dim3(nb), dim3(RP_NT), 0, ctx->stream, in, n, ctx->raw_boff.as<unsigned long long>(),
                       ctx->raw_bstate.as<u32>(), st, out);
}

int raw_finish(dskgpu_ctx* ctx, u64* lines) {
    if (!ctx->raw_pending) return DSKGPU_OK;
    RawState s;
    CK(hipMemcpyAsync(&s, ctx->raw_state.p, sizeof(RawState), hipMemcpyDeviceToHost, ctx->stream));
    CK(hipStreamSynchronize(ctx->stream));
    ctx->raw_pending = false;
    uint8_t* dst = ctx->reads_own.as<uint8_t>();
    if (!rp_file_ok(s)) s.bad = 1;
    if (s.bad) {
        ctx->reads_len = ctx->raw_base;
        ctx->d_reads = dst; ctx->n_bytes = ctx->reads_len;
        return fail(ctx, DSKGPU_E_FORMAT, "dskgpu_push_raw: the text is not 4-line FASTQ / FASTA as declared (the raw pushes were dropped: parse on the host and push the reads)");
    }
    if (s.out_len + 1 > ctx->reads_own.cap) return fail(ctx, DSKGPU_E_STATE, "dskgpu_push_raw: stream longer than its bound");
    CK(hipMemsetAsync(dst + s.out_len, '\n', 1, ctx->stream));
    ctx->reads_len = s.out_len + 1;
    if (lines) *lines = s.recs;
    ctx->d_reads = dst; ctx->n_bytes = ctx->reads_len; ctx->enc_keep = false; ctx->reads_changed();
    return DSKGPU_OK;
}

extern "C" {

const char* dskgpu_version(void) { return DSKGPU_VERSION; }

int dskgpu_device_count(void) { int n = 0; return hipGetDeviceCount(&n) == hipSuccess ? n : 0; }

const char* dskgpu_last_error(const dskgpu_ctx* ctx) { return ctx ? ctx->err.c_str() : g_create_err.c_str(); }

int dskgpu_create(const dskgpu_config* cfg, dskgpu_ctx** out) {
    if (!cfg || !out) { g_create_err = "null argument"; return DSKGPU_E_ARG; }
    *out = nullptr;
    if (cfg->kmer_size < 1 || cfg->kmer_size > 128) { g_create_err = "kmer_size must be in 1..128"; return DSKGPU_E_ARG; }
    if (cfg->solidity_kind > DSKGPU_SOLIDITY_CUSTOM) { g_create_err = "unknown solidity_kind"; return DSKGPU_E_ARG; }
    if (g_place_k < 0) { const char* e = getenv("DSKGPU_PLACE"); g_place_k = e ? atoi(e) : 0; }
    if ((cfg->flags & DSKGPU_F_PLACE) && g_place_k < 2) g_place_k = 8;
    const u32 ws = cfg->world_size ? cfg->world_size : 1;
    if ((ws & (ws - 1)) != 0 || ws > 64 || cfg->rank >= ws) { g_create_err = "world_size must be a power of two <= 64 and rank < world_size"; return DSKGPU_E_ARG; }
    int ndev = 0;
    hipError_t e = hipGetDeviceCount(&ndev);
    if (e != hipSuccess || ndev == 0) { g_create_err = std::string("no HIP device: ") + hipGetErrorString(e); return DSKGPU_E_DEVICE; }
    if (cfg->device < 0 || cfg->device >= ndev) { g_create_err = "bad device ordinal"; return DSKGPU_E_ARG; }
    e = hipSetDevice(cfg->device);
    if (e != hipSuccess) { g_create_err = std::string("hipSetDevice: ") + hipGetErrorString(e); return DSKGPU_E_DEVICE; }
    dskgpu_ctx* ctx = new dskgpu_ctx();
    ctx->cfg = *cfg;
    ctx->cfg.world_size = ws;
    if (ctx->cfg.histo_max == 0) ctx->cfg.histo_max = 10000;
    if (ctx->cfg.abundance_max == 0) ctx->cfg.abundance_max = 0x7FFFFFFFu;
    if (ctx->cfg.minimizer_size == 0) ctx->cfg.minimizer_size = 10;
    ctx->W = cfg->kmer_size <= 32 ? 1 : cfg->kmer_size <= 64 ? 2 : 4;
    ctx->words_out = (int)((cfg->kmer_size + 31) / 32);
    ctx->sentinel_ok = !sentinel_is_a_kmer(ctx->W, cfg->kmer_size);
    ctx->max_keys_per_pass = (u64)cfg->max_pass_mkeys * 1000000ull;
    ctx->tune.read();
    ctx->sk_mode = cfg->kmer_size >= 20 && cfg->kmer_size <= 64 && !(cfg->flags & DSKGPU_F_MG_EXPLICIT);
    if (ctx->sk_mode) {
        SkParams& sp = ctx->sender.sp;
        sp.k = cfg->kmer_size; sp.G = ws;
        sp.m = std::min<u32>(std::min<u32>(ctx->cfg.minimizer_size, 16u), cfg->kmer_size - 15u);
        sp.R = sk_record_words(cfg->kmer_size);
        ctx->l0_sender.sp = sp;
    }
    { int cus = 0; if (hipDeviceGetAttribute(&cus, hipDeviceAttributeMultiprocessorCount, cfg->device) == hipSuccess && cus > 0) ctx->num_cu = cus; }
    e = hipStreamCreateWithFlags(&ctx->stream, hipStreamNonBlocking);
    if (e != hipSuccess) { g_create_err = std::string("hipStreamCreate: ") + hipGetErrorString(e); delete ctx; return DSKGPU_E_DEVICE; }
    ctx->own_stream = true;
    *out = ctx;
    return DSKGPU_OK;
}

void dskgpu_destroy(dskgpu_ctx* ctx) {
    if (!ctx) return;
    (void)hipSetDevice(ctx->cfg.device);
    (void)hipStreamSynchronize(ctx->stream);
    DevBuf* bufs[] = {&ctx->reads_own, &ctx->raw_in, &ctx->raw_blk, &ctx->raw_boff, &ctx->raw_bstate, &ctx->raw_state, &ctx->packed, &ctx->inval, &ctx->bufA, &ctx->bufB, &ctx->mat1, &ctx->mat2, &ctx->sums,
                      &ctx->descs1, &ctx->descs2, &ctx->seg, &ctx->fstart, &ctx->nsolid, &ctx->scalars, &ctx->ghist, &ctx->gstats, &ctx->chain_next, &ctx->smp_mat, &ctx->smp_descs, &ctx->boff, &ctx->hv_lut, &ctx->hv_collect, &ctx->hv_buf, &ctx->dbg, &ctx->l0buf,
                      &ctx->out_ab, &ctx->srt_ab, &ctx->srt_tmp,
                      &ctx->srt_idx, &ctx->srt_idx2, &ctx->srt_k, &ctx->srt_k2, &ctx->abund2, &ctx->acc_ab, &ctx->u_val,
                      &ctx->s_val, &ctx->m_flag, &ctx->m_pos, &ctx->m_sum, &ctx->gh2d,
                      &ctx->sk_sums, &ctx->sk_cbase, &ctx->sk_keys, &ctx->cur_state, &ctx->smp_keys, &ctx->back_dev};
    if (ctx->back_host) (void)hipHostFree(ctx->back_host);
    ctx->rs.release();
    ctx->sender.release(); ctx->l0_sender.release();
    ctx->query.release();
    ctx->unitigs.release();
    ctx->threading.release();
    ctx->variants.release();
    ctx->readsum.release();
    ctx->colors.release();
    ctx->filtered.release();
    if (ctx->land) (void)hipHostFree(ctx->land);
    for (DevBuf* b : bufs) b->release();
    for (int i = 0; i < 4; ++i) { ctx->out_w[i].release(); ctx->srt_w[i].release(); ctx->acc_w[i].release(); ctx->u_w[i].release(); ctx->s_w[i].release(); }
    for (hipEvent_t e : ctx->ev_pool) (void)hipEventDestroy(e);
    for (int i = 0; i < 2; ++i) { if (ctx->pin[i]) (void)hipHostFree(ctx->pin[i]); if (ctx->pin_ev[i]) (void)hipEventDestroy(ctx->pin_ev[i]); }
    if (ctx->own_stream) (void)hipStreamDestroy(ctx->stream);
    delete ctx;
}

int dskgpu_set_stream(dskgpu_ctx* ctx, void* hip_stream) {
    if (!ctx) return DSKGPU_E_ARG;
    CK(hipSetDevice(ctx->cfg.device));
    CK(hipStreamSynchronize(ctx->stream));
    if (hip_stream) {
        if (ctx->own_stream) { (void)hipStreamDestroy(ctx->stream); ctx->own_stream = false; }
        ctx->stream = reinterpret_cast<hipStream_t>(hip_stream);
    } else if (!ctx->own_stream) {
        CK(hipStreamCreateWithFlags(&ctx->stream, hipStreamNonBlocking));
        ctx->own_stream = true;
    }
    return DSKGPU_OK;
}

#define PIN_CHUNK ((size_t)32 << 20)
static_assert(PIN_CHUNK == ((size_t)32 << 20), "launch_raw_chunk's capacity check is written for 32 MB pieces");
static void stage_copy(void* dst, const void* src, size_t n) {
    const unsigned T = n >= ((size_t)16 << 20) ? 8u : n >= ((size_t)8 << 20) ? 4u : n >= ((size_t)2 << 20) ? 2u : 1u;
    if (T == 1) { std::memcpy(dst, src, n); return; }
    const size_t per = (((n + T - 1) / T) + 4095) & ~(size_t)4095;
    auto part = [=](unsigned t) { const size_t a = (size_t)t * per; if (a < n) std::memcpy((char*)dst + a, (const char*)src + a, std::min(per, n - a)); };
    std::thread th[7];
    unsigned started = 1;
    try { for (; started < T; ++started) th[started - 1] = std::thread(part, started); }
    catch (const std::system_error&) {}
    part(0);
    for (unsigned t = started; t < T; ++t) part(t);
    for (unsigned t = 1; t < started; ++t) th[t - 1].join();
}

static int ensure_pinned(dskgpu_ctx* ctx) {
    if (ctx->pin[0] && ctx->pin[1]) return DSKGPU_OK;
    for (int i = 0; i < 2; ++i) {
        if (!ctx->pin[i]) CK(hipHostMalloc(&ctx->pin[i], PIN_CHUNK, hipHostMallocDefault));
        if (!ctx->pin_ev[i]) CK(hipEventCreateWithFlags(&ctx->pin_ev[i], hipEventDisableTiming));
    }
    return DSKGPU_OK;
}

int dskgpu_push_reads(dskgpu_ctx* ctx, const char* bytes, uint64_t nbytes) {
    if (!ctx || (!bytes && nbytes)) return DSKGPU_E_ARG;
    CK(hipSetDevice(ctx->cfg.device));
    if (ctx->raw_pending) { const int e = raw_finish(ctx, nullptr); if (e) return e; }
    const u64 need = ctx->reads_len + nbytes + 1;
    if (need > ctx->reads_own.cap) {
        DevBuf nb;
        CK(nb.ensure(std::max<u64>(need, std::max<u64>(ctx->reads_own.cap * 2, (u64)256 << 20))));
        if (ctx->reads_len) CK(hipMemcpyAsync(nb.p, ctx->reads_own.p, ctx->reads_len, hipMemcpyDeviceToDevice, ctx->stream));
        CK(hipStreamSynchronize(ctx->stream));
        ctx->reads_own.release();
        ctx->reads_own = nb;
    }
    uint8_t* dst = ctx->reads_own.as<uint8_t>();
    if (nbytes) {
        const size_t CH = PIN_CHUNK;
        { const int e = ensure_pinned(ctx); if (e) return e; }
        for (u64 off = 0; off < nbytes; off += CH, ctx->pin_next ^= 1) {
            const int slot = ctx->pin_next;
            const size_t len = (size_t)std::min<u64>(CH, nbytes - off);
            if (ctx->pin_used[slot]) CK(hipEventSynchronize(ctx->pin_ev[slot]));
            stage_copy(ctx->pin[slot], bytes + off, len);
            CK(hipMemcpyAsync(dst + ctx->reads_len + off, ctx->pin[slot], len, hipMemcpyHostToDevice, ctx->stream));
            CK(hipEventRecord(ctx->pin_ev[slot], ctx->stream));
            ctx->pin_used[slot] = true;
        }
    }
    CK(hipMemsetAsync(dst + ctx->reads_len + nbytes, '\n', 1, ctx->stream));
    ctx->reads_len += nbytes + 1;
    ctx->d_reads = dst; ctx->n_bytes = ctx->reads_len; ctx->enc_keep = false; ctx->reads_changed();
    return DSKGPU_OK;
}

int dskgpu_raw_finish(dskgpu_ctx* ctx, uint64_t* stream_bytes, uint64_t* records) {
    if (!ctx) return DSKGPU_E_ARG;
    CK(hipSetDevice(ctx->cfg.device));
    u64 ln = 0;
    const int rc = raw_finish(ctx, &ln);
    if (stream_bytes) *stream_bytes = ctx->reads_len;
    if (records) *records = ln;
    return rc;
}

int dskgpu_push_raw(dskgpu_ctx* ctx, const char* text, uint64_t nbytes, int format, int new_file) {
    if (!ctx || (!text && nbytes) || (format != DSKGPU_RAW_FASTA && format != DSKGPU_RAW_FASTQ)) return DSKGPU_E_ARG;
    CK(hipSetDevice(ctx->cfg.device));
    if (!ctx->raw_pending) {
        CK(ctx->raw_state.ensure(sizeof(RawState)));
        CK(ctx->raw_in.ensure(PIN_CHUNK));
        const u64 maxb = PIN_CHUNK / RP_BLOCK;
        CK(ctx->raw_blk.ensure(maxb * sizeof(RpBlock)));
        CK(ctx->raw_boff.ensure(maxb * 8));
        CK(ctx->raw_bstate.ensure((maxb + 1) * 4));
        ctx->raw_base = ctx->raw_ub = ctx->reads_len;
        hipLaunchKernelGGL(k_rp_init, dim3(1), dim3(1), 0, ctx->stream, ctx->raw_state.as<RawState>(), (unsigned long long)ctx->reads_len);
        CKL("k_rp_init");
        ctx->raw_pending = true;
    } else if (new_file) {
        hipLaunchKernelGGL(k_rp_fresh, dim3(1), dim3(1), 0, ctx->stream, ctx->raw_state.as<RawState>());
        CKL("k_rp_fresh");
    }
    const u64 need = ctx->raw_ub + nbytes + 2;
    if (need > ctx->reads_own.cap) {
        DevBuf nb;
        CK(nb.ensure(std::max<u64>(need, std::max<u64>(ctx->reads_own.cap * 2, (u64)256 << 20))));
        if (ctx->raw_ub) CK(hipMemcpyAsync(nb.p, ctx->reads_own.p, ctx->raw_ub, hipMemcpyDeviceToDevice, ctx->stream));
        CK(hipStreamSynchronize(ctx->stream));
        ctx->reads_own.release();
        ctx->reads_own = nb;
    }
    uint8_t* out = ctx->reads_own.as<uint8_t>();
    if (nbytes) {
        const size_t CH = PIN_CHUNK;
        { const int e = ensure_pinned(ctx); if (e) return e; }
        for (u64 off = 0; off < nbytes; off += CH, ctx->pin_next ^= 1) {
            const int slot = ctx->pin_next;
            const size_t len = (size_t)std::min<u64>(CH, nbytes - off);
            if (ctx->pin_used[slot]) CK(hipEventSynchronize(ctx->pin_ev[slot]));
            stage_copy(ctx->pin[slot], text + off, len);
            CK(hipMemcpyAsync(ctx->raw_in.p, ctx->pin[slot], len, hipMemcpyHostToDevice, ctx->stream));
            CK(hipEventRecord(ctx->pin_ev[slot], ctx->stream));
            ctx->pin_used[slot] = true;
            if (format == DSKGPU_RAW_FASTQ) launch_raw_chunk<RP_FASTQ>(ctx, (u32)len, out);
            else launch_raw_chunk<RP_FASTA>(ctx, (u32)len, out);
            CKL("k_rp_write");
        }
    }
    ctx->raw_ub += nbytes + 1;
    return DSKGPU_OK;
}

int dskgpu_stream_bytes(dskgpu_ctx* ctx, uint64_t* stream_bytes) {
    if (!ctx || !stream_bytes) return DSKGPU_E_ARG;
    CK(hipSetDevice(ctx->cfg.device));
    RAW_SYNC(ctx);
    *stream_bytes = ctx->reads_len;
// ... 321 lines not shown
```

### dsk_amd/csrc/engine.h

```cpp
#pragma once
#include <algorithm>
#include <cstring>
#include <string>
#include <vector>

#include "../../include/dskgpu.h"
#include "layouts.h"

hipError_t placed_malloc(void** out, size_t bytes);

struct DevBuf {
    void* p = nullptr;
    size_t cap = 0;
    hipError_t ensure(size_t bytes) {
        if (bytes <= cap) return hipSuccess;
        size_t want = ((p ? bytes + bytes / 16 : bytes) + 255) & ~size_t(255);
        if (p) { (void)hipFree(p); p = nullptr; cap = 0; }
        hipError_t e = placed_malloc(&p, want);
        if (e == hipSuccess) cap = want; else p = nullptr;
        return e;
    }
    int ensure_keep(size_t bytes, size_t keep, hipStream_t stream) {
        if (bytes <= cap) return 0;
        void* np = nullptr;
// ... 59 lines not shown
        rs_block_rows = (u32)num("DSKGPU_RS_BLOCK_ROWS", 0); rs_bbits = (u32)num("DSKGPU_RS_BBITS", 0); rs_heavy = (u32)num("DSKGPU_RS_HEAVY", 0);
    }
};

struct SparseRows {
    int W = 0;
    const void* keys = nullptr; const u32 *ab = nullptr, *soff = nullptr, *fstart = nullptr; u32 cap = 0, F = 0;
    u64 n_sparse = 0; u32 n_tail = 0; RowsIn tail_w{}; const u32* tail_ab = nullptr;
    template <class S> S as(u32 qpc = 0) const { return S{static_cast<decltype(S::keys)>(keys), ab, soff, fstart, cap, F, qpc}; }
    Rows2C tail2() const { return Rows2C{tail_w.w[1], tail_w.w[0], tail_ab}; }
};

struct PartPasses {
    struct Pass { u64 row_base; u32 nparts, off_index; };
    std::vector<Pass> passes; DevBuf part_off, flag; u32 off_used = 0; bool ok = false; u64 row_base = 0;
    std::vector<u32> h_off;
};

struct RowSort {
    DevBuf fix_list;
    DevBuf g[4];
    DevBuf del, lens;
    std::vector<u64> h_del; std::vector<u32> h_lens, h_lin;
    DevBuf ovs;
    u32 flag = 0, listed = 0;
    u64* hist_pin = nullptr; size_t hist_pin_n = 0;
    bool part_mode = false; u32 n_parts = 0; u32* h_part_off = nullptr; size_t h_part_cap = 0; DevBuf part_off;
    std::vector<u64> h_part_off64;
    PartPasses mp;
    void release() {
        for (DevBuf* b : {&fix_list, &g[0], &g[1], &g[2], &g[3], &del, &lens, &ovs, &part_off, &mp.part_off, &mp.flag}) b->release();
        if (hist_pin) (void)hipHostFree(hist_pin);
        if (h_part_off) (void)hipHostFree(h_part_off);
        hist_pin = nullptr; h_part_off = nullptr;
    }
};

struct Query {
    DevBuf table, packed, inval, deg;
    u64 cap = 0;
    bool valid = false;
    void release() { table.release(); packed.release(); inval.release(); deg.release(); cap = 0; valid = false; }
    void invalidate() { valid = false; }
};

struct Components {
    DevBuf comp, first, cols;
    dskgpu_component_stats stats{};
    bool valid = false;
    void release() { for (DevBuf* b : {&comp, &first, &cols}) b->release(); stats = dskgpu_component_stats{}; valid = false; }
    void invalidate() { stats = dskgpu_component_stats{}; valid = false; }
};

struct Unitigs {
    DevBuf unitig, pos, offsets, ab_sum, kind;
    DevBuf ends, e_offsets, e_targets;
    Components cc;
    dskgpu_unitig_stats stats{};
    dskgpu_unitig_edge_stats e_stats{};
    bool valid = false;
    bool e_valid = false;
    void release_edges() { for (DevBuf* b : {&ends, &e_offsets, &e_targets}) b->release(); e_stats = dskgpu_unitig_edge_stats{}; e_valid = false; cc.release(); }
    void release() { for (DevBuf* b : {&unitig, &pos, &offsets, &ab_sum, &kind}) b->release(); stats = dskgpu_unitig_stats{}; valid = false; release_edges(); }
    void invalidate() { stats = dskgpu_unitig_stats{}; e_stats = dskgpu_unitig_edge_stats{}; valid = false; e_valid = false; cc.invalidate(); }
};

struct Threading {
    DevBuf offsets, steps, first, last, ends, usup, esup;
    dskgpu_thread_stats stats{};
    u64 n_unitigs = 0, n_edges = 0;
    bool valid = false;
    void release() { for (DevBuf* b : {&offsets, &steps, &first, &last, &ends, &usup, &esup}) b->release(); stats = dskgpu_thread_stats{}; n_unitigs = n_edges = 0; valid = false; }
};

struct Variants {
    DevBuf rec, off, stream;
    dskgpu_variant_stats stats{};
    bool valid = false;
    void release() { for (DevBuf* b : {&rec, &off, &stream}) b->release(); stats = dskgpu_variant_stats{}; valid = false; }
};

struct ReadSummaries {
    DevBuf table;
    dskgpu_read_summary_stats stats{};
    bool valid = false;
    void release() { table.release(); stats = dskgpu_read_summary_stats{}; valid = false; }
};

struct Colors {
    DevBuf C;
    u32 n_colors = 0;
    u64 n_rows = 0;
    bool valid = false;
    void release() { C.release(); n_colors = 0; n_rows = 0; valid = false; }
};

struct Filtered {
    DevBuf w[2][4], ab[2];
    int cur = -1;
    std::vector<u64> part_off;
    DevBuf scan, tmp, rec, off_in, info, len, bits, keep, ends;
    void release() {
        for (int s = 0; s < 2; ++s) { for (int x = 0; x < 4; ++x) w[s][x].release(); ab[s].release(); }
        for (DevBuf* b : {&scan, &tmp, &rec, &off_in, &info, &len, &bits, &keep, &ends}) b->release();
        cur = -1; part_off.clear();
    }
};

struct Sender {
    SkParams sp{};
    std::vector<uint8_t> h_table;
    bool table_dirty = true;
    DevBuf table, load;
    DevBuf sent;
    DevBuf lay;
    DevBuf cb64;
    bool prepared = false;
    bool slices = false;
    bool exact = false;
    u32 nslices = 0;
    std::vector<u64> h_rstart;
    std::vector<u32> h_cells;
    std::vector<u64> h_cb64;
    u64 h_sent[SK_MAX_OWNERS] = {0};
    u64 h_est[SK_MAX_OWNERS] = {0};
    void release() { for (DevBuf* b : {&table, &load, &sent, &lay, &cb64}) b->release(); table_dirty = true; prepared = false; nslices = 0; }
};

struct BankJob { dskgpu_config cfg; const uint8_t* base; u64 total; std::vector<u64> ends; u64 nu, tot_kmers; u32 passes, retries; bool active = false; };

struct dskgpu_ctx {
    dskgpu_config cfg{};
    BankJob bank_job{};
    Tuning tune;
    int W = 1;
    int words_out = 1;
    hipStream_t stream = nullptr;
    bool own_stream = false;
    int num_cu = 256;
    std::string err;

    DevBuf reads_own; u64 reads_len = 0;
    void* pin[2] = {nullptr, nullptr}; hipEvent_t pin_ev[2] = {nullptr, nullptr}; bool pin_used[2] = {false, false}; int pin_next = 0;
    const uint8_t* d_reads = nullptr; u64 n_bytes = 0;
    DevBuf raw_in, raw_blk, raw_boff, raw_bstate, raw_state;
    bool raw_pending = false; u64 raw_base = 0, raw_ub = 0;

    DevBuf packed, inval;
    DevBuf bufA, bufB;
    DevBuf mat1, mat2, sums, descs1, descs2, seg, fstart, nsolid, scalars, ghist, gstats, chain_next;
    RowSort rs;
    DevBuf smp_keys;
    DevBuf smp_mat, smp_descs, boff;
    DevBuf dbg, l0buf; DevBuf hv_lut, hv_collect, hv_buf;
    std::vector<unsigned char> h_hv_lut; std::vector<u32> h_hv_cnt, h_hv_step; std::vector<u64> h_hv_coll, h_hv_keys;
    std::vector<ChunkDesc> h_descs_s, h_descs1, h_descs2; std::vector<u64> h_cbeg; std::vector<u32> h_boff; std::vector<u64> h_mom;
    DevBuf out_w[4], srt_w[4], acc_w[4];
    DevBuf out_ab, srt_ab, srt_tmp, srt_idx, srt_idx2, srt_k, srt_k2, abund2, acc_ab;
    u64 max_keys_per_pass = 0;
    std::vector<u64> bank_ends;
    DevBuf u_w[4], s_w[4], u_val, s_val, m_flag, m_pos, m_sum, gh2d;
    std::vector<u64> hist2d;
    std::vector<u32> h_starts;
    bool enc_keep = false;
    bool enc_fresh = false;
    bool sk_mode = false;
    Sender sender, l0_sender;
    DevBuf sk_sums, sk_cbase, sk_keys;
    std::vector<u32> h_sk_sums; std::vector<u64> h_sk_cbase;
    const u64* rec_src = nullptr; u64 rec_n = 0; u64 rec_nch = 0, rec_rpc = 0; bool rec_expanded = false;
    bool rec_sized = false;
    u64 rec_hint = 0;
    bool rec_hint_est = false;
    std::vector<u64> rec_slice_end;
    dskgpu_slice_gate rec_gate = nullptr; void* rec_gate_user = nullptr; u32 rec_gated = 0;
    bool rec_gate_failed = false;
    std::vector<u32> h_slice_chunk;
    DevBuf cur_state;
    u64 last_rows = 0;
    bool rec_l0_off = false;
    u64* land = nullptr;
    DevBuf back_dev; u64* back_host = nullptr;
    u32 h_back[3] = {0}; u64 h_stats[4] = {0}; u32 h_ovf1 = 0; u64 h_nvalid = 0; bool have_nvalid = false;
    bool sentinel_ok = true;
    bool opt1_off = false;
    bool mw_v3_off = false;
    bool opt2_off = false;
    std::vector<const void*> big_lds_fns;
    u32 h_sc[SC_COUNT] = {0};

    u32 job_passes = 1;
    SparseRows sp_rows;
    SparseRows take_sparse_rows() { const SparseRows r = sp_rows; sp_rows = SparseRows{}; return r; }
    struct RowSink { bool active = false, took = false; u32* ab = nullptr; u64* w[4] = {nullptr, nullptr, nullptr, nullptr}; u64 rows = 0, cap = 0; } sink;
    bool have_result = false;
    u64 n_rows = 0;
    const u64* res_w[4] = {nullptr, nullptr, nullptr, nullptr}; const u32* res_ab = nullptr;
    dskgpu_stats stats{};
    std::vector<u64> hist;
    Query query;
    Unitigs unitigs;
    Threading threading;
    Variants variants;
    ReadSummaries readsum;
    Colors colors;
    Filtered filtered;
    void drop_result() { have_result = false; query.release(); unitigs.release(); threading.release(); variants.release(); readsum.release(); colors.release(); filtered.release(); }
    void reads_changed() { enc_fresh = false; sender.prepared = false; sender.exact = false; opt2_off = false; opt1_off = false; mw_v3_off = false; rec_l0_off = false; last_rows = 0; }

    std::vector<Stage> marks;
    std::vector<hipEvent_t> ev_pool; size_t ev_used = 0;
    std::vector<const char*> st_names; std::vector<float> st_ms;

    void mark(const char* name) {
        if (!(cfg.flags & DSKGPU_F_TIMING)) return;
        if (ev_used == ev_pool.size()) { hipEvent_t e; (void)hipEventCreate(&e); ev_pool.push_back(e); }
        hipEvent_t e = ev_pool[ev_used++];
        (void)hipEventRecord(e, stream);
        marks.push_back({name, e});
    }
    void resolve_marks() {
        for (size_t i = 0; i + 1 < marks.size(); ++i) {
            float ms = 0; (void)hipEventElapsedTime(&ms, marks[i].ev, marks[i + 1].ev);
            size_t at = 0;
            while (at < st_names.size() && std::strcmp(st_names[at], marks[i + 1].name) != 0) ++at;
            if (at == st_names.size()) { st_names.push_back(marks[i + 1].name); st_ms.push_back(ms); } else st_ms[at] += ms;
        }
        marks.clear(); ev_used = 0;
    }
};

#define CK(expr)                                                                             \
    do {                                                                                     \
        hipError_t e_ = (expr);                                                              \
        if (e_ != hipSuccess) {                                                              \
            ctx->err = std::string(#expr) + ": " + hipGetErrorString(e_);                    \
            return (e_ == hipErrorOutOfMemory) ? DSKGPU_E_NOMEM : DSKGPU_E_DEVICE;           \
        }                                                                                    \
    } while (0)

#define CKL(what)                                                                            \
    do {                                                                                     \
        hipError_t e_ = hipGetLastError();                                                   \
        if (e_ != hipSuccess) {                                                              \
            ctx->err = std::string(what) + ": " + hipGetErrorString(e_);                     \
            return DSKGPU_E_DEVICE;                                                          \
        }                                                                                    \
    } while (0)

inline int fail(dskgpu_ctx* ctx, int code, const std::string& msg) { ctx->err = msg; return code; }
inline unsigned blocks(u64 items, u64 per_block) { return (unsigned)((items + per_block - 1) / per_block); }

int encode_current(dskgpu_ctx* ctx, u64* nwords_out);
int raw_finish(dskgpu_ctx* ctx, u64* lines);
#define RAW_SYNC(ctx) do { if ((ctx)->raw_pending) { const int e_ = raw_finish(ctx, nullptr); if (e_) return e_; } } while (0)
int encode_into(dskgpu_ctx* ctx, const uint8_t* d_bytes, u64 n, u64* packed, u32* inval);
int run_scan(dskgpu_ctx* ctx, u32* a, const u32* d_len, u64 max_len);
int allow_big_lds(dskgpu_ctx* ctx, const void* fn, int bytes = 160 * 1024);

#define REC_L0_NO 2001
struct RecL0 { u32 G = 0; u64 nch = 0; u32 slice[SK_MAX_OWNERS] = {0}; u64 region[SK_MAX_OWNERS] = {0}; };
int rec_l0_prepare(dskgpu_ctx* ctx, Sender& s, u64 nwords, u32 G, RecL0* rl);
int rec_l0_sweep(dskgpu_ctx* ctx, Sender& s, const RecL0& rl, u32 olo, u32 ohi, u64 (&base_words)[SK_MAX_OWNERS]);
uint64_t sk_send_capacity_words(dskgpu_ctx* ctx);
int sk_scatter(dskgpu_ctx* ctx, void* d_send, uint64_t capacity_words, uint64_t* send_words);

int order_rows(dskgpu_ctx* ctx, u64 n, u32 npass);
u64 rs_max_rows(const dskgpu_ctx* ctx);
int sort_index_multiword(dskgpu_ctx* ctx, const u64* const* rows, u64 n, int W);
u32 part_sort_nparts(const SparseRows& rows);
int launch_part_sort(dskgpu_ctx* ctx, const SparseRows& rows, RowsOut out, u32* out_ab, u32* d_part_off, u32* d_flag, u32* nparts_out);
u32 rows_partitions(const dskgpu_ctx* ctx);
void rows_partition_range(const dskgpu_ctx* ctx, u32 p, u64* b, u64* e);

struct QTable;
int ensure_index(dskgpu_ctx* ctx);
QTable query_table(const dskgpu_ctx* ctx);
int query_ensure(dskgpu_ctx* ctx, DevBuf& b, size_t bytes, const char* what);
void query_begin(dskgpu_ctx* ctx);
int query_finish(dskgpu_ctx* ctx);

int ensure_compaction(dskgpu_ctx* ctx, const char* who);
int ensure_edges(dskgpu_ctx* ctx, const char* who);

enum { REC_COUNTERS = 4, REC_ROWS = 3 };
int abandon(dskgpu_ctx* ctx, int rc);
int begin_record(dskgpu_ctx* ctx, bool with_offsets, std::vector<u64>& old_off);
int filter_scan(dskgpu_ctx* ctx, const unsigned char* keep, const std::vector<u64>& old_off);
int read_record(dskgpu_ctx* ctx, std::vector<u64>& h, u64 n_off);
int filter_apply(dskgpu_ctx* ctx, const unsigned char* keep, const u64* new_off, u64 n_off);
int flag_rows(dskgpu_ctx* ctx, unsigned char* d_row_flag, bool want_keep);
typedef int (*RoundEnqueue)(dskgpu_ctx* ctx, const void* params, unsigned char* d_row_flag, bool want_keep);
int round_once(dskgpu_ctx* ctx, const char* who, const char* stage, RoundEnqueue enqueue, const void* params, void* d_row_flag, void* d_unitig_bits, u64* counters);
int rounds_run(dskgpu_ctx* ctx, const char* who, const char* stage, u64 max_rounds, RoundEnqueue enqueue, const void* params, u64* counters, u64* n_rounds);

int bubble_candidates(dskgpu_ctx* ctx, u32 max_nodes);
```

### dsk_amd/csrc/kernels.h

```cpp
#pragma once
#include "layouts.h"

#ifndef SC_NT
#define SC_NT 1024
#endif
template <int W> struct Tile {
    static constexpr int KPT = 16 / W;
    static constexpr int KEYS = SC_NT * KPT;
    static constexpr int WORDS = KEYS / 32;
};
#define MAX_BINS 2048


template <bool ALIGNED>
__global__ __launch_bounds__(256) void k_encode(const uint8_t* __restrict__ s, u64 n,
                                                u64* __restrict__ packed, u32* __restrict__ inval, u64 nwords) {
    const u64 stride = (u64)gridDim.x * blockDim.x;
    for (u64 w = (u64)blockIdx.x * blockDim.x + threadIdx.x; w < nwords; w += stride) {
        const u64 base = w * 32;
        u32 x[8];
        if (ALIGNED && base + 32 <= n) {
            const uint4 a = *reinterpret_cast<const uint4*>(s + base);
            const uint4 b = *reinterpret_cast<const uint4*>(s + base + 16);
            x[0] = a.x; x[1] = a.y; x[2] = a.z; x[3] = a.w; x[4] = b.x; x[5] = b.y; x[6] = b.z; x[7] = b.w;
        } else {
#pragma unroll
            for (int q = 0; q < 8; ++q) {
                u32 v = 0;
#pragma unroll
                for (int b = 0; b < 4; ++b) {
                    const u64 p = base + q * 4 + b;
                    const u32 c = p < n ? s[p] : (u32)'\n';
                    v |= c << (8 * b);
                }
                x[q] = v;
            }
        }
        u64 pk = 0; u32 iv = 0;
        constexpr u32 BASES = (1u << 1) | (1u << 3) | (1u << 7) | (1u << 20);
#pragma unroll
        for (int q = 0; q < 8; ++q) {
            const u32 xx = x[q];
            const u32 codes = ((((xx >> 1) & 0x03030303u) * 0x40100401u) >> 24);
            const u32 hi = (xx & 0xC0C0C0C0u) ^ 0x40404040u;
            u32 ok = 0;
#pragma unroll
            for (int b = 0; b < 4; ++b) ok |= ((BASES >> ((xx >> (8 * b)) & 31u)) & 1u) << (8 * b);
            const u32 hz = (((hi & 0x7F7F7F7Fu) + 0x7F7F7F7Fu) | hi) >> 7;
            const u32 good = ok & ~hz & 0x01010101u;
            const u32 bad4 = (((good ^ 0x01010101u) * 0x08040201u) >> 24) & 0xFu;
            pk |= (u64)codes << (56 - 8 * q);
            iv |= bad4 << (28 - 4 * q);
        }
        packed[w] = pk;
        inval[w] = iv;
    }
}

template <int W> struct KeyT { typedef KN<W> T; };
template <> struct KeyT<1> { typedef u64 T; };

__device__ __forceinline__ u64 digit_word(u64 h) { return h; }
template <int W> __device__ __forceinline__ u64 digit_word(const KN<W>& h) { return h.w[W - 1]; }

struct DigitSpec { u32 mode, pa, pb, world, npass, pass, ones_is_key; };
__device__ __forceinline__ u32 key_pass(u64 w, const DigitSpec& ds) {
    const u32 frac = (((u32)(w >> 12) & 0xFFFFFu) * ds.world) & 0xFFFFFu;
    return (frac * ds.npass) >> 20;
}
template <int MODE>
__device__ __forceinline__ u32 key_digit(u64 w, const DigitSpec& ds) {
    if (MODE == 1 || MODE == 3) return __umulhi((u32)(w >> 32), ds.pa);
    if (MODE == 2) return __umulhi((u32)(w >> 32) * ds.pa, ds.pb);
    if (MODE == 4) return key_pass(w, ds) - ds.pass;
    return (((u32)(w >> 12) & 0xFFFFFu) * ds.pa) >> 20;
}
template <int MODE>
__device__ __forceinline__ bool key_in_pass(u64 w, const DigitSpec& ds) {
    if (MODE == 3) return key_pass(w, ds) == ds.pass;
    if (MODE == 4) return key_pass(w, ds) - ds.pass < ds.pa;
    return true;
}

template <int NP>
__device__ __forceinline__ u32 gen_kmers_multi(const u64* __restrict__ packed, const u32* __restrict__ inval, u64 wi, int t0, int k, K2 (&c)[NP]) {
    return gen_kmers2<NP>(packed, inval, wi, t0, k, c);
}
template <int W, int NP>
__device__ __forceinline__ u32 gen_kmers_multi(const u64* __restrict__ packed, const u32* __restrict__ inval, u64 wi, int t0, int k, KN<W> (&c)[NP]) {
    return gen_kmersN<W, NP>(packed, inval, wi, t0, k, c);
}

template <int W>
__device__ __forceinline__ u32 tile_keys_reads(const u64* __restrict__ packed, const u32* __restrict__ inval,
                                               u64 w0, u64 wend, int k, KN<W> (&h)[Tile<W>::KPT]) {
    constexpr int KPT = Tile<W>::KPT, TPW = 32 / KPT;
    const u64 wi = w0 + (threadIdx.x / TPW);
    if (wi >= wend) return 0u;
    const u32 vm = gen_kmers_multi(packed, inval, wi, (int)(threadIdx.x % TPW) * KPT, k, h);
#pragma unroll
    for (int j = 0; j < KPT; ++j) kmixN(h[j]);
    return vm;
}
__device__ __forceinline__ u32 tile_keys_reads(const u64* __restrict__ packed, const u32* __restrict__ inval,
                                               u64 w0, u64 wend, int k, u64 (&h)[16]) {
    const u64 wi = w0 + (threadIdx.x >> 1);
    if (wi >= wend) return 0u;
    const u32 vm = gen_kmers1<16>(packed, inval, wi, (threadIdx.x & 1) * 16, k, h);
#pragma unroll
    for (int j = 0; j < 16; ++j) h[j] = kmix(h[j]);
    return vm;
}

__device__ __forceinline__ bool is_pad_key(u64 h, const DigitSpec&) { return h == DSK_EMPTY; }
template <int W> __device__ __forceinline__ bool is_pad_key(const KN<W>& h, const DigitSpec& ds) {
    bool e = !ds.ones_is_key;
#pragma unroll
    for (int x = 0; x < W; ++x) e = e && (h.w[x] == DSK_EMPTY);
    return e;
}
__device__ __forceinline__ bool keys_same(u64 a, u64 b) { return a == b; }
template <int W> __device__ __forceinline__ bool keys_same(const KN<W>& a, const KN<W>& b) { return key_eq(a, b); }
template <int W>
__device__ __forceinline__ u32 tile_keys_array(const typename KeyT<W>::T* __restrict__ in, u64 k0, u64 kend,
                                               typename KeyT<W>::T (&h)[Tile<W>::KPT], const DigitSpec& ds) {
    const typename KeyT<W>::T* base = in + k0;
    const u64 left = kend - k0;
    const u32 n = left < (u64)Tile<W>::KEYS ? (u32)left : (u32)Tile<W>::KEYS;
    u32 vm = 0;
#pragma unroll
    for (int j = 0; j < Tile<W>::KPT; ++j) {
        const u32 o = threadIdx.x + (u32)j * SC_NT;
        const bool ok = o < n;
        h[j] = base[ok ? o : n - 1];
        vm |= ((ok && !is_pad_key(h[j], ds)) ? 1u : 0u) << j;
    }
    return vm;
}

template <int W, int SRC, int MODE>
__global__ __launch_bounds__(SC_NT) void k_hist(const u64* __restrict__ packed, const u32* __restrict__ inval,
                                                const typename KeyT<W>::T* __restrict__ keys,
                                                const ChunkDesc* __restrict__ descs, const u32* __restrict__ d_nchunks,
                                                u32* __restrict__ matrix, int k, DigitSpec ds, u32 P) {
    __shared__ u32 lh[MAX_BINS + 1];
    constexpr int KPT = Tile<W>::KPT;
    const u32 nchunks = *d_nchunks;
    for (u32 g = blockIdx.x; g < nchunks; g += gridDim.x) {
        const ChunkDesc d = descs[g];
        for (u32 b = threadIdx.x; b <= P; b += SC_NT) lh[b] = 0;
        __syncthreads();
        const u64 step = SRC == 0 ? Tile<W>::WORDS : Tile<W>::KEYS;
        typename KeyT<W>::T ha[KPT], hb[KPT]; u32 vma = 0, vmb = 0;
        auto process = [&](typename KeyT<W>::T (&h)[KPT], u32 vm) {
            u32 dg[KPT];
#pragma unroll
            for (int j = 0; j < KPT; ++j)
                dg[j] = ((vm & (1u << j)) && key_in_pass<MODE>(digit_word(h[j]), ds)) ? key_digit<MODE>(digit_word(h[j]), ds) : P;
#pragma unroll
            for (int j = 0; j < KPT; ++j) atomicAdd(&lh[dg[j]], 1u);
        };
        if (SRC == 0) {
            for (u64 t0 = d.begin; t0 < d.end; t0 += step) {
                vma = tile_keys_reads(packed, inval, t0, d.end, k, ha);
                process(ha, vma);
            }
        } else {
            if (d.begin < d.end) vma = tile_keys_array<W>(keys, d.begin, d.end, ha, ds);
            for (u64 t0 = d.begin; t0 < d.end; t0 += 2 * step) {
                if (t0 + step < d.end) vmb = tile_keys_array<W>(keys, t0 + step, d.end, hb, ds);
                process(ha, vma);
                const u64 t1 = t0 + step;
                if (t1 >= d.end) break;
                if (t1 + step < d.end) vma = tile_keys_array<W>(keys, t1 + step, d.end, ha, ds);
                process(hb, vmb);
            }
        }
        __syncthreads();
        for (u32 b = threadIdx.x; b < P; b += SC_NT) matrix[d.flat_base + (u64)b * d.stride] = lh[b];
        __syncthreads();
    }
}

#define SCAN_NT 256
#define SCAN_IPT 16
#define SCAN_BLK (SCAN_NT * SCAN_IPT)

__global__ __launch_bounds__(SCAN_NT) void k_scan_reduce(const u32* __restrict__ a, const u32* __restrict__ d_len,
                                                         u32* __restrict__ sums) {
    __shared__ u32 ws[SCAN_NT / 64];
    const u64 len = *d_len;
    const u64 b0 = (u64)blockIdx.x * SCAN_BLK;
    if (b0 >= len) return;
    u32 s = 0;
#pragma unroll
    for (int j = 0; j < SCAN_IPT; ++j) {
        const u64 i = b0 + threadIdx.x + (u64)j * SCAN_NT;
        if (i < len) s += a[i];
    }
#pragma unroll
    for (int d = 32; d >= 1; d >>= 1) s += __shfl_down(s, d);
    if ((threadIdx.x & 63) == 0) ws[threadIdx.x >> 6] = s;
    __syncthreads();
    if (threadIdx.x == 0) { u32 t = 0; for (int i = 0; i < SCAN_NT / 64; ++i) t += ws[i]; sums[blockIdx.x] = t; }
}

__global__ __launch_bounds__(1024) void k_scan_sums(u32* __restrict__ sums, const u32* __restrict__ d_len,
                                                    u32* __restrict__ a) {
    __shared__ u32 ws[16]; __shared__ u32 carry_s;
    const u64 len = *d_len;
    const u32 nb = (u32)((len + SCAN_BLK - 1) / SCAN_BLK);
    const int lane = threadIdx.x & 63, wave = threadIdx.x >> 6;
    if (threadIdx.x == 0) carry_s = 0;
    __syncthreads();
    for (u32 c0 = 0; c0 < nb; c0 += 1024) {
        const u32 i = c0 + threadIdx.x;
        const u32 x = i < nb ? sums[i] : 0u;
        u32 y = x;
#pragma unroll
        for (int d = 1; d < 64; d <<= 1) { const u32 t = __shfl_up(y, d); if (lane >= d) y += t; }
        if (lane == 63) ws[wave] = y;
        __syncthreads();
        if (wave == 0) {
            const u32 wx = lane < 16 ? ws[lane] : 0u; u32 wy = wx;
#pragma unroll
            for (int d = 1; d < 16; d <<= 1) { const u32 t = __shfl_up(wy, d); if (lane >= d) wy += t; }
            if (lane < 16) ws[lane] = wy - wx;
        }
        __syncthreads();
        const u32 carry = carry_s;
        const u32 excl = carry + ws[wave] + y - x;
        if (i < nb) sums[i] = excl;
        __syncthreads();
        if (threadIdx.x == 1023) carry_s = excl + x;
        __syncthreads();
    }
    if (threadIdx.x == 0) a[len] = carry_s;
}

__global__ __launch_bounds__(SCAN_NT) void k_scan_apply(u32* __restrict__ a, const u32* __restrict__ d_len,
                                                        const u32* __restrict__ sums) {
    __shared__ u32 ws[SCAN_NT / 64];
    const u64 len = *d_len;
    const u64 b0 = (u64)blockIdx.x * SCAN_BLK;
    if (b0 >= len) return;
    const u64 i0 = b0 + (u64)threadIdx.x * SCAN_IPT;
    u32 v[SCAN_IPT]; u32 s = 0;
#pragma unroll
    for (int j = 0; j < SCAN_IPT; ++j) { v[j] = (i0 + j < len) ? a[i0 + j] : 0u; s += v[j]; }
    const int lane = threadIdx.x & 63, wave = threadIdx.x >> 6;
    u32 y = s;
#pragma unroll
    for (int d = 1; d < 64; d <<= 1) { const u32 t = __shfl_up(y, d); if (lane >= d) y += t; }
    if (lane == 63) ws[wave] = y;
    __syncthreads();
    u32 wpre = 0;
    for (int w = 0; w < wave; ++w) wpre += ws[w];
    u32 run = sums[blockIdx.x] + wpre + y - s;
#pragma unroll
    for (int j = 0; j < SCAN_IPT; ++j) { if (i0 + j < len) a[i0 + j] = run; run += v[j]; }
}


struct OptSpec { u32 cap; u32* subcnt; u32* ovf; const u32* fill; u32 slice, nsl; u64 sstride;
                 u32 F, max_ext; u32* next; u32* ext_cursor; u32* chain_list; u32* chain_cnt;
                 u32* work;
                 unsigned long long* dbg; };
#define CHAIN_BIT 0x80000000u
#define HV_KEYS 4
__device__ __forceinline__ bool is_empty_key(u64 h) { return h == DSK_EMPTY; }
template <int W> __device__ __forceinline__ bool is_empty_key(const KN<W>& h) {
    bool e = true;
#pragma unroll
    for (int x = 0; x < W; ++x) e = e && (h.w[x] == DSK_EMPTY);
    return e;
}
template <int W> __device__ __forceinline__ typename KeyT<W>::T empty_key();
template <> __device__ __forceinline__ u64 empty_key<1>() { return DSK_EMPTY; }
template <> __device__ __forceinline__ K2 empty_key<2>() { K2 k; k.w[0] = k.w[1] = DSK_EMPTY; return k; }
template <> __device__ __forceinline__ KN<4> empty_key<4>() { KN<4> k; k.w[0] = k.w[1] = k.w[2] = k.w[3] = DSK_EMPTY; return k; }


__device__ __forceinline__ u64 sk_key1(const u64* r, int j, int k);
__device__ __forceinline__ K2 sk_key2(const u64* r, int j, int k);
__device__ __forceinline__ void sk_key(const u64* r, int j, int k, u64& out) { out = sk_key1(r, j, k); }
__device__ __forceinline__ void sk_key(const u64* r, int j, int k, K2& out) { out = sk_key2(r, j, k); }
template <int W> __device__ __forceinline__ void sk_key(const u64*, int, int, KN<W>&) {}

template <int W> struct RecTile { static constexpr int NR = W == 1 ? 3 * SC_NT : SC_NT; static constexpr int RPT = NR / SC_NT;
                                  static constexpr int RS = W == 1 ? 2 : 3; };
template <int W> struct RecPre { u64 w[RecTile<W>::RPT * RecTile<W>::RS]; };
template <int W>
__device__ __forceinline__ void rec_prefetch(RecPre<W>& pre, const u64* __restrict__ rec, u32 R, u64 r0, u64 rend) {
    constexpr int RPT = RecTile<W>::RPT, RS = RecTile<W>::RS;
#pragma unroll
    for (int u = 0; u < RPT; ++u) {
        const u64 r = r0 + (u64)threadIdx.x * RPT + u;
        const u64* p = rec + (r < rend ? r : r0) * R;
        pre.w[u * RS] = p[0]; pre.w[u * RS + 1] = p[1];
        if (RS == 3) pre.w[u * RS + 2] = (R == 3) ? p[2] : 0ull;
    }
}
// ... 1609 lines not shown
    const u64 wi = t >> 1;
    if (wi >= nwords) return;
    const int t0 = (int)(t & 1) * 16;
    u32 vm;
    if (W == 1) {
        u64 c[16];
        vm = gen_kmers1<16>(packed, inval, wi, t0, k, c);
        for (int j = 0; j < 16; ++j) {
            const u64 p = wi * 32 + t0 + j;
            if (p < nbytes) { const bool v = vm & (1u << j); out[p] = v ? c[j] : 0ull; valid[p] = v; }
        }
    } else {
        constexpr int WW = W > 1 ? W : 2;
        KN<WW> c[16];
        vm = gen_kmers_multi(packed, inval, wi, t0, k, c);
        for (int j = 0; j < 16; ++j) {
            const u64 p = wi * 32 + t0 + j;
            if (p < nbytes) {
                const bool v = vm & (1u << j);
                for (int x = 0; x < WW; ++x) if (x < ow) out[(u64)ow * p + x] = v ? c[j].w[x] : 0ull;
                valid[p] = v;
            }
        }
    }
}

__global__ __launch_bounds__(256) void k_minimizers(const u64* __restrict__ packed, const u32* __restrict__ inval,
                                                    u64 nwords, u64 nbytes, int k, int m,
                                                    u32* __restrict__ minim, uint8_t* __restrict__ valid) {
    const u64 t = (u64)blockIdx.x * blockDim.x + threadIdx.x;
    const u64 p0 = t * 16;
    if (p0 >= nbytes) return;
    const u32 mmask = (m == 16) ? 0xFFFFFFFFu : ((1u << (2 * m)) - 1);
    const int halo = k - 1;
    const long long s0 = (long long)p0 - halo;
    u32 cm[16 + 127];
    u32 f = 0, r = 0; int run = 0;
    int runs[16];
    for (int i = 0; i < halo + 16; ++i) {
        const long long pos = s0 + i;
        bool ok = false; u32 c = 0;
        if (pos >= 0 && (u64)pos < nbytes) {
            const u64 w = (u64)pos >> 5; const int j = (int)(pos & 31);
            ok = !((inval[w] >> (31 - j)) & 1u);
            c = (u32)(packed[w] >> (62 - 2 * j)) & 3u;
        }
        if (!ok) { run = 0; f = 0; r = 0; }
        else { f = ((f << 2) | c) & mmask; r = (r >> 2) | ((c ^ 2u) << (2 * (m - 1))); ++run; }
        cm[i] = f < r ? f : r;
        if (i >= halo) runs[i - halo] = run;
    }
    for (int j = 0; j < 16; ++j) {
        const u64 p = p0 + j;
        if (p >= nbytes) break;
        const bool v = runs[j] >= k;
        u32 best = 0xFFFFFFFFu;
        if (v) for (int e = halo + j - (k - m); e <= halo + j; ++e) best = cm[e] < best ? cm[e] : best;
        minim[p] = v ? best : 0u;
        valid[p] = v ? 1 : 0;
    }
}

struct MergeParams { u32 nbanks, kind, mask, amin, amax, hmax, want2d; };
#define MB_LH 256
#define MB_L2 32
template <int W>
__device__ __forceinline__ bool rows_same(const RowsIn& r, u64 a, u64 b) {
    bool e = true;
#pragma unroll
    for (int x = 0; x < W; ++x) e = e && (r.w[x][a] == r.w[x][b]);
    return e;
}
template <int W>
__global__ __launch_bounds__(256) void k_merge_banks(RowsIn rows, const u64* __restrict__ val,
                                                     u64 n, MergeParams mp, u32* __restrict__ flag, u32* __restrict__ sumv,
                                                     u64* __restrict__ ghist, u64* __restrict__ gh2d, u64* __restrict__ gstats) {
    __shared__ u32 lh[MB_LH];
    __shared__ u32 l2[MB_L2 * 11];
    for (int b = threadIdx.x; b < MB_LH; b += 256) lh[b] = 0;
    for (int b = threadIdx.x; b < MB_L2 * 11; b += 256) l2[b] = 0;
    __syncthreads();
    const u64 i = (u64)blockIdx.x * 256 + threadIdx.x;
    u32 ndist = 0;
    if (i < n) {
        const bool head = i == 0 || !rows_same<W>(rows, i - 1, i);
        u32 f = 0, sv = 0;
        if (head) {
            u64 sum = 0; u32 mx = 0, genome = 0, present = 0, inwin = 0, nonzero = 0, nb = 0; u32 mn = 0xFFFFFFFFu;
            for (u64 j = i; j < n && rows_same<W>(rows, i, j) && nb < mp.nbanks; ++j, ++nb) {
                const u64 v = val[j]; const u32 bank = (u32)(v >> 32), c = (u32)v;
                sum += c; mx = c > mx ? c : mx; mn = c < mn ? c : mn;
                if (bank == 0) genome = c;
                nonzero |= 1u << bank;
                if (c >= mp.amin) present |= 1u << bank;
                if (c >= mp.amin && c <= mp.amax) inwin |= 1u << bank;
            }
            if (nb < mp.nbanks) mn = 0;
            const u32 all = mp.nbanks >= 32 ? 0xFFFFFFFFu : ((1u << mp.nbanks) - 1);
            const u32 s32 = sum > 0xFFFFFFFFull ? 0xFFFFFFFFu : (u32)sum;
            bool solid;
            switch (mp.kind) {
                case 1: solid = mn >= mp.amin && mn <= mp.amax; break;
                case 2: solid = mx >= mp.amin && mx <= mp.amax; break;
                case 3: solid = inwin != 0; break;
                case 4: solid = inwin == all; break;
                case 5: solid = (present & mp.mask) == (mp.mask & all) && (nonzero & ~mp.mask) == 0; break;
                default: solid = s32 >= mp.amin && s32 <= mp.amax;
            }
            f = solid ? 1u : 0u; sv = s32; ndist = 1;
            const u32 hb = s32 < mp.hmax ? s32 : mp.hmax;
            if (hb < MB_LH) atomicAdd(&lh[hb], 1u); else atomicAdd(&ghist[hb], 1ull);
            if (mp.want2d) {
                const u64 reads = sum - genome;
                const u32 r = reads < mp.hmax ? (u32)reads : mp.hmax, gcol = genome < 10 ? genome : 10u;
                if (r < MB_L2) atomicAdd(&l2[r * 11 + gcol], 1u); else atomicAdd(&gh2d[(u64)r * 11 + gcol], 1ull);
            }
        }
        flag[i] = f; sumv[i] = sv;
    }
    for (int d = 32; d >= 1; d >>= 1) ndist += __shfl_down(ndist, d);
    if ((threadIdx.x & 63) == 0 && ndist) atomicAdd(&gstats[0], (u64)ndist);
    __syncthreads();
    for (int b = threadIdx.x; b < MB_LH; b += 256) if (lh[b]) atomicAdd(&ghist[b < (int)mp.hmax ? b : (int)mp.hmax], (u64)lh[b]);
    if (mp.want2d) for (int b = threadIdx.x; b < MB_L2 * 11; b += 256) if (l2[b]) atomicAdd(&gh2d[b], (u64)l2[b]);
}

template <int W>
__global__ __launch_bounds__(256) void k_pick_rows(RowsIn rows, const u32* __restrict__ sumv,
                                                   const u32* __restrict__ flag_in, const u32* __restrict__ posx, u64 n,
                                                   RowsOut out, u32* __restrict__ out_ab) {
    const u64 i = (u64)blockIdx.x * 256 + threadIdx.x;
    if (i >= n || !flag_in[i]) return;
    const u32 p = posx[i];
#pragma unroll
    for (int x = 0; x < W; ++x) out.w[x][p] = rows.w[x][i];
    out_ab[p] = sumv[i];
}
__global__ void k_pack_bank(u64* __restrict__ dst, const u32* __restrict__ ab, u64 n, u32 bank) {
    const u64 i = (u64)blockIdx.x * blockDim.x + threadIdx.x;
    if (i < n) dst[i] = ((u64)bank << 32) | ab[i];
}
__global__ __launch_bounds__(256) void k_bin_moments(const u32* __restrict__ matrix, u32 nch, u32 P, u64* __restrict__ mom) {
    const u32 b = blockIdx.x * 4 + (threadIdx.x >> 6), lane = threadIdx.x & 63;
    if (b >= P) return;
    u64 s = 0, q = 0;
    for (u32 c = lane; c < nch; c += 64) { const u64 x = matrix[(u64)b * nch + c]; s += x; q += x * x; }
#pragma unroll
    for (int d = 32; d >= 1; d >>= 1) { s += __shfl_down(s, d); q += __shfl_down(q, d); }
    if (lane == 0) { mom[2 * b] = s; mom[2 * b + 1] = q; }
}
#define HV_SLOTS 16
#define HV_COLLECT 2048
#define HV_BLOCK_KEYS 32
template <int W, int SRC, int MODE>
__global__ __launch_bounds__(SC_NT) void k_collect_heavy(const u64* __restrict__ packed, const u32* __restrict__ inval, const typename KeyT<W>::T* __restrict__ keys,
                                                         const ChunkDesc* __restrict__ descs, const u32* __restrict__ d_nchunks, int k, DigitSpec ds, u32 P,
                                                         const unsigned char* __restrict__ lut, u32* __restrict__ kept, typename KeyT<W>::T* __restrict__ out, const u32* __restrict__ keep_step) {
    typedef typename KeyT<W>::T Key;
    constexpr int KPT = Tile<W>::KPT;
    __shared__ unsigned char slut[MAX_BINS + 8];
    __shared__ u32 lcnt[HV_SLOTS], lstep[HV_SLOTS];
    const int lane = threadIdx.x & 63;
    for (u32 b = threadIdx.x; b < P; b += SC_NT) slut[b] = lut[b];
    if (threadIdx.x < HV_SLOTS) { const u32 st = keep_step[threadIdx.x]; lstep[threadIdx.x] = st; lcnt[threadIdx.x] = (blockIdx.x * 7919u) % st; }
    __syncthreads();
    const u32 nchunks = *d_nchunks;
    for (u32 g = blockIdx.x; g < nchunks; g += gridDim.x) {
        const ChunkDesc d = descs[g];
        const u64 step = SRC == 0 ? Tile<W>::WORDS : Tile<W>::KEYS;
        for (u64 t0 = d.begin; t0 < d.end; t0 += step) {
            Key h[KPT];
            u32 vm;
            if constexpr (SRC == 0) vm = tile_keys_reads(packed, inval, t0, d.end, k, h); else vm = tile_keys_array<W>(keys, t0, d.end, h, ds);
#pragma unroll
            for (int j = 0; j < KPT; ++j) {
                u32 f = 0xFFu;
                if ((vm & (1u << j)) && key_in_pass<MODE>(digit_word(h[j]), ds)) f = slut[key_digit<MODE>(digit_word(h[j]), ds)];
                u64 todo = __ballot(f != 0xFFu);
                while (todo) {
                    const int lead = __ffsll((unsigned long long)todo) - 1;
                    const u32 fl = (u32)__shfl((int)f, lead);
                    const u64 grp = __ballot(f == fl);
                    u32 base = 0;
                    if (lane == lead) base = atomicAdd(&lcnt[fl], (u32)__popcll(grp));
                    base = (u32)__shfl((int)base, lead);
                    if (f == fl) {
                        const u32 idx = base + (u32)__popcll(grp & ((1ull << lane) - 1)), st = lstep[fl];
                        const u32 p0 = ((blockIdx.x * 7919u) % st + st - 1) / st;
                        if (idx % st == 0u && idx / st - p0 < HV_BLOCK_KEYS) out[((u64)fl * gridDim.x + blockIdx.x) * HV_BLOCK_KEYS + idx / st - p0] = h[j];
                    }
                    todo &= ~grp;
                }
            }
        }
    }
    __syncthreads();
    if (threadIdx.x < HV_SLOTS) {
        const u32 st = lstep[threadIdx.x];
        const u32 n = (lcnt[threadIdx.x] + st - 1) / st - ((blockIdx.x * 7919u) % st + st - 1) / st;
        kept[threadIdx.x * gridDim.x + blockIdx.x] = n < HV_BLOCK_KEYS ? n : HV_BLOCK_KEYS;
    }
}
template <int W>
__global__ void k_heavy_rows(const typename KeyT<W>::T* __restrict__ hv_keys, const unsigned long long* __restrict__ hv_cnt, u32 nslots, u32 amin, u32 amax, u32 histo_max,
                             u64* __restrict__ ghist, u64* __restrict__ gstats, u64* __restrict__ rows_k , u32* __restrict__ rows_ab) {
    const u32 i = blockIdx.x * blockDim.x + threadIdx.x;
    if (i >= nslots) return;
    const typename KeyT<W>::T key = hv_keys[i];
    const unsigned long long c64 = hv_cnt[i];
    if (is_empty_key(key) || c64 == 0ull) return;
    const u32 c = c64 > 0xFFFFFFFFull ? 0xFFFFFFFFu : (u32)c64;
    atomicAdd(&ghist[c < histo_max ? c : histo_max], 1ull);
    atomicAdd(&gstats[0], 1ull);
    atomicAdd(&gstats[2], c64);
    if (c >= amin && c <= amax) {
        const u64 at = atomicAdd(&gstats[1], 1ull);
        if constexpr (W == 1) rows_k[at] = kunmix(key);
        else {
            KN<W> kx = key; kunmixN(kx);
#pragma unroll
            for (int x = 0; x < W; ++x) rows_k[(u64)x * nslots + at] = kx.w[x];
        }
        rows_ab[at] = c;
    }
}
__global__ void k_copy_u32(u32* __restrict__ dst, const u32* __restrict__ src, u64 n) {
    const u64 i = (u64)blockIdx.x * blockDim.x + threadIdx.x;
    if (i < n) dst[i] = src[i];
}
```

### dsk_amd/csrc/layouts.h

```cpp
#pragma once
#include "kmer_device.h"

__device__ __forceinline__ void lds_barrier() { asm volatile("s_waitcnt lgkmcnt(0)\n\ts_barrier" ::: "memory"); }

struct SliceGuard { const u32* lim; u32 dump; u32 uslice, first; };
template <int NT>
__device__ __forceinline__ void tile_scan(u32* cnt, u32* off, u32* delta, u32* cur, int P, u32* wsum, u32* tot, SliceGuard sg = SliceGuard{nullptr, 0u, 0u, 0u}) {
    const int tid = threadIdx.x, lane = tid & 63, wave = tid >> 6;
    const int ipt = (P + NT - 1) / NT;
    const int base = tid * ipt;
    u32 v[4]; u32 s = 0;
#pragma unroll
    for (int j = 0; j < 4; ++j) {
        const int idx = base + j;
        v[j] = (j < ipt && idx < P) ? cnt[idx] : 0u;
        s += v[j];
    }
    const u32 inc = wave_incl_scan(s);
    if (lane == 63) wsum[wave] = inc;
    lds_barrier();
    if (wave == 0) {
        const u32 x = lane < NT / 64 ? wsum[lane] : 0u;
        const u32 y = wave_incl_scan(x);
        if (lane < NT / 64) wsum[lane] = y - x;
        if (lane == NT / 64 - 1) { *tot = y; off[P] = y; }
    }
    lds_barrier();
    u32 run = wsum[wave] + inc - s;
#pragma unroll
    for (int j = 0; j < 4; ++j) {
        const int idx = base + j;
        if (j < ipt && idx < P) {
            const u32 c = cur[idx];
            const u32 end = sg.lim ? sg.lim[idx] : sg.uslice ? sg.first + (u32)(idx + 1) * sg.uslice : 0xFFFFFFFFu;
            const bool fits = (sg.lim || sg.uslice) ? c + v[j] <= end : true;
            off[idx] = run; delta[idx] = fits ? c - run : sg.dump; cur[idx] = fits ? c + v[j] : end + 1u; cnt[idx] = 0;
            run += v[j];
        }
    }
}

struct ChunkDesc {
    u64 begin, end;
    u32 flat_base;
    u32 stride;
};

#define SK_MAX_OWNERS 64
#define SK_BUCKETS 4096
struct SkParams {
    u64 ngroups;
    u64 ntiles;
    u32 tiles_per_chunk, nchunks;
    u32 k, m, G, R;
    u32 sample_step;
    u32 slice;
    u32 c0, c0g, clen;
    u64 rbase;
    const unsigned char* table;
    u32 has_split;
    u32 olo, ohi;
    const u32* oslice; const unsigned long long* obase;
};

struct RowsOut { u64* w[4]; };
struct RowsIn { const u64* w[4]; };
struct Rows2 { u64* hi; u64* lo; u32* ab; };
struct Rows2C { const u64* hi; const u64* lo; const u32* ab; };
struct RsSparse { const u64* keys; const u32* ab; const u32* soff; const u32* fstart; u32 cap, F, qpc; };
struct Rs2Sparse { const K2* keys; const u32* ab; const u32* soff; const u32* fstart; u32 cap, F, qpc; };
struct Rs4Sparse { const KN<4>* keys; const u32* ab; const u32* soff; const u32* fstart; u32 cap, F, qpc; };

template <class T>
__global__ void k_gather(T* __restrict__ dst, const T* __restrict__ src, const u32* __restrict__ idx, u64 n) {
    const u64 i = (u64)blockIdx.x * blockDim.x + threadIdx.x;
    if (i < n) dst[i] = src[idx[i]];
}
```

Baseline: 27.61 billion.

## Generate chunk descriptors on device and batch small host-to-device parameter uploads

```diff
diff --git a/dsk_amd/csrc/dskgpu.hip b/dsk_amd/csrc/dskgpu.hip
--- a/dsk_amd/csrc/dskgpu.hip
+++ b/dsk_amd/csrc/dskgpu.hip
@@ -81,14 +81,51 @@
         out[6] = gstats[0]; out[7] = gstats[1]; out[8] = gstats[2]; out[9] = gstats[3];
     }
 }
+#define SCAN_BACK_MAXNB 1024
+__global__ __launch_bounds__(SCAN_NT) void k_scan_apply_back(u32* __restrict__ a, const u32* __restrict__ d_len, const u32* __restrict__ sums,
+                                                             const u32* __restrict__ sc, const u32* __restrict__ nk, const u64* __restrict__ gstats, u64* __restrict__ out) {
+    __shared__ u32 ws[SCAN_NT / 64], ps[SCAN_NT / 64];
+    const u64 len = *d_len;
+    const u32 nb = (u32)((len + SCAN_BLK - 1) / SCAN_BLK), last = nb ? nb - 1 : 0u;
+    if (blockIdx.x > last) return;
+    const int lane = threadIdx.x & 63, wave = threadIdx.x >> 6;
+    u32 pre = 0;
+    for (u32 i = threadIdx.x; i < blockIdx.x; i += SCAN_NT) pre += sums[i];
+#pragma unroll
+    for (int d = 32; d >= 1; d >>= 1) pre += __shfl_down(pre, d);
+    if (lane == 0) ps[wave] = pre;
+    const u64 i0 = (u64)blockIdx.x * SCAN_BLK + (u64)threadIdx.x * SCAN_IPT;
+    u32 v[SCAN_IPT]; u32 s = 0;
+#pragma unroll
+    for (int j = 0; j < SCAN_IPT; ++j) { v[j] = (i0 + j < len) ? a[i0 + j] : 0u; s += v[j]; }
+    u32 y = s;
+#pragma unroll
+    for (int d = 1; d < 64; d <<= 1) { const u32 t = __shfl_up(y, d); if (lane >= d) y += t; }
+    if (lane == 63) ws[wave] = y;
+    __syncthreads();
+    u32 base = 0, wpre = 0, all = 0;
+    for (int w = 0; w < SCAN_NT / 64; ++w) { base += ps[w]; if (w < wave) wpre += ws[w]; all += ws[w]; }
+    u32 run = base + wpre + y - s;
+#pragma unroll
+    for (int j = 0; j < SCAN_IPT; ++j) { if (i0 + j < len) a[i0 + j] = run; run += v[j]; }
+    if (blockIdx.x == last && threadIdx.x == 0) {
+        const u32 total = base + all;
+        a[len] = total;
+        out[0] = sc[SC_OVERFLOW]; out[1] = total; out[2] = nk ? *nk : 0u; out[3] = sc[SC_OVF2]; out[4] = sc[SC_OVF1]; out[5] = sc[SC_EXT];
+        out[6] = gstats[0]; out[7] = gstats[1]; out[8] = gstats[2]; out[9] = gstats[3];
+    }
+}
 struct ScalarSet { u32 v[SC_COUNT]; };
 __global__ __launch_bounds__(256) void k_setup_pass(u32* __restrict__ sc, ScalarSet h, u64* __restrict__ ghist, u32 nh, u64* __restrict__ gstats, u32 nstats,
-                                                    u32* __restrict__ zero, u64 nzero) {
+                                                    u32* __restrict__ zero, u64 nzero, ChunkDesc* __restrict__ descs1, DescSpec d1s,
+                                                    const u32* __restrict__ pb_src, u32 pb_words, u32* __restrict__ pb_dst) {
     const u32 t = blockIdx.x * 256 + threadIdx.x;
     if (t < SC_COUNT) sc[t] = h.v[t];
     if (t < nstats) gstats[t] = 0ull;
     for (u32 i = t; i < nh; i += gridDim.x * 256) ghist[i] = 0ull;
     for (u64 i = t; i < nzero; i += (u64)gridDim.x * 256) zero[i] = 0u;
+    for (u32 i = t; i < d1s.nch; i += gridDim.x * 256) descs1[i] = chunk_desc(d1s, i);
+    for (u32 i = t; i < pb_words; i += gridDim.x * 256) pb_dst[i] = pb_src[i];
 }
 }
 
@@ -169,23 +206,23 @@
 
 template <int W, int SRC, int MODE>
 int launch_hist_m(dskgpu_ctx* ctx, const typename KeyT<W>::T* keys, const ChunkDesc* descs, const u32* d_nch,
-                  u64 max_chunks, u32* matrix, DigitSpec ds, u32 P) {
+                  u64 max_chunks, u32* matrix, DigitSpec ds, u32 P, DescSpec sp = DescSpec{0ull, 0ull, 0ull, 0u, 0u, 0ull, 0u}, ChunkDesc* descs_out = nullptr) {
     const unsigned grid = (unsigned)std::max<u64>(1, std::min<u64>(max_chunks, (u64)ctx->num_cu));
     hipLaunchKernelGGL((k_hist<W, SRC, MODE>), dim3(grid), dim3(SC_NT), 0, ctx->stream, ctx->packed.as<u64>(),
-                       ctx->inval.as<u32>(), keys, descs, d_nch, matrix, (int)ctx->cfg.kmer_size, ds, P);
+                       ctx->inval.as<u32>(), keys, descs, d_nch, matrix, (int)ctx->cfg.kmer_size, ds, P, sp, descs_out);
     CKL("k_hist");
     return DSKGPU_OK;
 }
 template <int W, int SRC>
 int launch_hist(dskgpu_ctx* ctx, const typename KeyT<W>::T* keys, const ChunkDesc* descs, const u32* d_nch,
-                u64 max_chunks, u32* matrix, DigitSpec ds, u32 P) {
+                u64 max_chunks, u32* matrix, DigitSpec ds, u32 P, DescSpec sp = DescSpec{0ull, 0ull, 0ull, 0u, 0u, 0ull, 0u}, ChunkDesc* descs_out = nullptr) {
     const bool mp = ds.mode == 1 && ds.npass > 1;
-    if (SRC == 0) return ds.mode == 0 ? launch_hist_m<W, 0, 0>(ctx, keys, descs, d_nch, max_chunks, matrix, ds, P)
-                       : mp ? launch_hist_m<W, 0, 3>(ctx, keys, descs, d_nch, max_chunks, matrix, ds, P)
-                            : launch_hist_m<W, 0, 1>(ctx, keys, descs, d_nch, max_chunks, matrix, ds, P);
-    return ds.mode == 2 ? launch_hist_m<W, 1, 2>(ctx, keys, descs, d_nch, max_chunks, matrix, ds, P)
-                   : mp ? launch_hist_m<W, 1, 3>(ctx, keys, descs, d_nch, max_chunks, matrix, ds, P)
-                        : launch_hist_m<W, 1, 1>(ctx, keys, descs, d_nch, max_chunks, matrix, ds, P);
+    if (SRC == 0) return ds.mode == 0 ? launch_hist_m<W, 0, 0>(ctx, keys, descs, d_nch, max_chunks, matrix, ds, P, sp, descs_out)
+                       : mp ? launch_hist_m<W, 0, 3>(ctx, keys, descs, d_nch, max_chunks, matrix, ds, P, sp, descs_out)
+                            : launch_hist_m<W, 0, 1>(ctx, keys, descs, d_nch, max_chunks, matrix, ds, P, sp, descs_out);
+    return ds.mode == 2 ? launch_hist_m<W, 1, 2>(ctx, keys, descs, d_nch, max_chunks, matrix, ds, P, sp, descs_out)
+                   : mp ? launch_hist_m<W, 1, 3>(ctx, keys, descs, d_nch, max_chunks, matrix, ds, P, sp, descs_out)
+                        : launch_hist_m<W, 1, 1>(ctx, keys, descs, d_nch, max_chunks, matrix, ds, P, sp, descs_out);
 }
 
 unsigned scatter_grid(const dskgpu_ctx* ctx, int W, u32 P, u64 max_chunks, bool opt = false) {
@@ -311,21 +348,10 @@
 }
 
 void build_descs1(dskgpu_ctx* ctx, u64 n_units_total, u64 tile, u64 max_chunks, u32* nch_out) {
-    const u64 ntiles = std::max<u64>(1, (n_units_total + tile - 1) / tile);
-    u64 nch = std::min<u64>(ntiles, max_chunks);
-    const u64 tpc = (ntiles + nch - 1) / nch;
-    nch = (ntiles + tpc - 1) / tpc;
-    ctx->h_descs1.resize(nch);
-    for (u64 c = 0; c < nch; ++c) {
-        ChunkDesc d;
-        d.begin = c * tpc * tile;
-        d.end = std::min<u64>(n_units_total, (c + 1) * tpc * tile);
-        if (d.begin > d.end) d.begin = d.end;
-        d.flat_base = (u32)c;
-        d.stride = (u32)nch;
-        ctx->h_descs1[c] = d;
-    }
-    *nch_out = (u32)nch;
+    const DescSpec sp = level1_spec(n_units_total, tile, max_chunks);
+    ctx->h_descs1.resize(sp.nch);
+    for (u32 c = 0; c < sp.nch; ++c) ctx->h_descs1[c] = chunk_desc(sp, c);
+    *nch_out = sp.nch;
 }
 
 void build_descs1_slices(dskgpu_ctx* ctx, u64 tile, u64 max_chunks, u32* nch_out) {
@@ -435,17 +461,15 @@
     const size_t per_slot = (size_t)grid * HV_BLOCK_KEYS;
     CK(ctx->hv_collect.ensure((size_t)HV_SLOTS * per_slot * sizeof(Key) + (size_t)HV_SLOTS * grid * 4 + HV_SLOTS * 4));
     u32* d_kept = reinterpret_cast<u32*>(ctx->hv_collect.as<Key>() + (size_t)HV_SLOTS * per_slot);
-    u32* d_step = d_kept + (size_t)HV_SLOTS * grid;
-    ctx->h_hv_step.assign(HV_SLOTS, 1);
-    for (size_t f = 0; f < flagged.size(); ++f) ctx->h_hv_step[f] = (u32)std::max<u64>(1, ctx->h_mom[2 * (size_t)flagged[f]] / HV_COLLECT);
+    HvSteps steps;
+    for (u32 f = 0; f < HV_SLOTS; ++f) steps.v[f] = 1u;
+    for (size_t f = 0; f < flagged.size(); ++f) steps.v[f] = (u32)std::max<u64>(1, ctx->h_mom[2 * (size_t)flagged[f]] / HV_COLLECT);
     CK(hipMemcpyAsync(ctx->hv_lut.p, ctx->h_hv_lut.data(), P1, hipMemcpyHostToDevice, ctx->stream));
-    CK(hipMemcpyAsync(d_step, ctx->h_hv_step.data(), HV_SLOTS * 4, hipMemcpyHostToDevice, ctx->stream));
-    u32* sc = ctx->scalars.as<u32>();
     const bool mp = pl.d1.npass > 1;
     auto launch = [&](auto kern) {
         hipLaunchKernelGGL(kern, dim3(grid), dim3(SC_NT), 0, ctx->stream, (const u64*)ctx->packed.as<u64>(), (const u32*)ctx->inval.as<u32>(), d_keys_in,
-                           (const ChunkDesc*)ctx->smp_descs.as<ChunkDesc>(), (const u32*)(sc + SC_NCH_S), (int)ctx->cfg.kmer_size, pl.d1, P1,
-                           (const unsigned char*)ctx->hv_lut.as<unsigned char>(), d_kept, ctx->hv_collect.as<Key>(), (const u32*)d_step);
+                           (const ChunkDesc*)ctx->smp_descs.as<ChunkDesc>(), nts, (int)ctx->cfg.kmer_size, pl.d1, P1,
+                           (const unsigned char*)ctx->hv_lut.as<unsigned char>(), d_kept, ctx->hv_collect.as<Key>(), steps);
     };
     if (from_reads) { if (mp) launch(k_collect_heavy<W, 0, 3>); else launch(k_collect_heavy<W, 0, 1>); }
     else { if (mp) launch(k_collect_heavy<W, 1, 3>); else launch(k_collect_heavy<W, 1, 1>); }
@@ -478,7 +502,9 @@
     }
     std::sort(cands.begin(), cands.end(), [](const Cand& a, const Cand& b) { return a.est > b.est; });
     if (cands.size() > HV_KEYS) cands.resize(HV_KEYS);
+    static_assert(HvLayout<W>::counts == HvLayout<W>::keys + (size_t)HV_KEYS * W, "the counts follow the keys: one copy sets both");
     ctx->h_hv_keys.assign((size_t)HV_KEYS * W, DSK_EMPTY);
+    ctx->h_hv_keys.resize((size_t)HV_KEYS * (W + 1), 0ull);
     for (size_t x = 0; x < cands.size(); ++x) {
         for (int y = 0; y < W; ++y) ctx->h_hv_keys[x * W + y] = cands[x].key.w[y];
         load[cands[x].bin] -= cands[x].est;
@@ -487,9 +513,7 @@
     if (nheavy) {
         CK(ctx->hv_buf.ensure(HvLayout<W>::words * 8));
         u64* hvb = ctx->hv_buf.as<u64>();
-        CK(hipMemsetAsync(hvb + HvLayout<W>::keys, 0xFF, (size_t)HV_KEYS * W * 8, ctx->stream));
-        CK(hipMemsetAsync(hvb + HvLayout<W>::counts, 0, HV_KEYS * 8, ctx->stream));
-        CK(hipMemcpyAsync(hvb + HvLayout<W>::keys, ctx->h_hv_keys.data(), (size_t)HV_KEYS * W * 8, hipMemcpyHostToDevice, ctx->stream));
+        CK(hipMemcpyAsync(hvb + HvLayout<W>::keys, ctx->h_hv_keys.data(), (size_t)HV_KEYS * (W + 1) * 8, hipMemcpyHostToDevice, ctx->stream));
     }
     *nheavy_out = nheavy;
     return DSKGPU_OK;
@@ -508,6 +532,9 @@
     u32 opt_cap = 0, max_ext = 0; u64 nregions = 0;
     bool opt1 = false; Opt1Spec o1{}; unsigned grid1 = 0;
     u32 nch1 = 0, nheavy = 0;
+    DescSpec d1s{};
+    const ChunkDesc* dd2 = nullptr;
+    const u32* pb_src = nullptr; u32 pb_words = 0;
     std::vector<double> load, spread;
     Key* fkeys = nullptr;
     DevBuf* scratch = nullptr;
@@ -520,12 +547,18 @@
 int upload_descs1(dskgpu_ctx* ctx, PassState<W>& ps) {
     const KeySource<W>& src = ps.src;
     const u64 max_chunks1 = (u64)ctx->num_cu * 8;
-    if (src.from_reads) build_descs1(ctx, src.nwords, Tile<W>::WORDS, max_chunks1, &ps.nch1);
-    else if (src.from_rec && ctx->rec_slice_end.size() > 1) build_descs1_slices(ctx, RecTile<W>::NR, max_chunks1, &ps.nch1);
-    else if (src.from_rec) build_descs1(ctx, ctx->rec_n, RecTile<W>::NR, max_chunks1, &ps.nch1);
-    else build_descs1(ctx, src.nkeys, Tile<W>::KEYS, max_chunks1, &ps.nch1);
-    CK(ctx->descs1.ensure(ctx->h_descs1.size() * sizeof(ChunkDesc)));
-    CK(hipMemcpyAsync(ctx->descs1.p, ctx->h_descs1.data(), ctx->h_descs1.size() * sizeof(ChunkDesc), hipMemcpyHostToDevice, ctx->stream));
+    ps.d1s = DescSpec{0ull, 0ull, 0ull, 0u, 0u, 0ull, 0u};
+    if (src.from_rec && ctx->rec_slice_end.size() > 1) {
+        build_descs1_slices(ctx, RecTile<W>::NR, max_chunks1, &ps.nch1);
+        CK(ctx->descs1.ensure(ctx->h_descs1.size() * sizeof(ChunkDesc)));
+        CK(hipMemcpyAsync(ctx->descs1.p, ctx->h_descs1.data(), ctx->h_descs1.size() * sizeof(ChunkDesc), hipMemcpyHostToDevice, ctx->stream));
+        return DSKGPU_OK;
+    }
+    if (src.from_reads) ps.d1s = level1_spec(src.nwords, Tile<W>::WORDS, max_chunks1);
+    else if (src.from_rec) ps.d1s = level1_spec(ctx->rec_n, RecTile<W>::NR, max_chunks1);
+    else ps.d1s = level1_spec(src.nkeys, Tile<W>::KEYS, max_chunks1);
+    ps.nch1 = ps.d1s.nch;
+    CK(ctx->descs1.ensure((size_t)ps.nch1 * sizeof(ChunkDesc)));
     return DSKGPU_OK;
 }
 
@@ -539,22 +572,12 @@
 
 template <class Hist>
 int positional_sample(dskgpu_ctx* ctx, u64 units, u64 tile, u32 P, Hist&& hist, u64* ntiles_out, u64* nts_out, u64* stot_out) {
-    u32* sc = ctx->scalars.as<u32>();
-    const u64 ntiles = std::max<u64>(1, (units + tile - 1) / tile);
-    const u64 nts = std::min<u64>(ntiles, 1024);
-    ctx->h_descs_s.resize(nts);
-    for (u64 i = 0; i < nts; ++i) {
-        const u64 t = i * ntiles / nts;
-        ChunkDesc d; d.begin = t * tile; d.end = std::min<u64>(units, (t + 1) * tile); d.flat_base = (u32)i; d.stride = (u32)nts;
-        ctx->h_descs_s[i] = d;
-    }
+    const DescSpec sp = sample_spec(units, tile);
+    const u64 ntiles = sp.ntiles, nts = sp.nch;
     const u64 Ms = (u64)P * nts;
+    CK(ctx->smp_mat.ensure((Ms + 4) * 4 + (size_t)P * 16));
     CK(ctx->smp_descs.ensure(nts * sizeof(ChunkDesc)));
-    CK(ctx->smp_mat.ensure((Ms + 4) * 4 + (size_t)P * 16));
-    CK(hipMemcpyAsync(ctx->smp_descs.p, ctx->h_descs_s.data(), nts * sizeof(ChunkDesc), hipMemcpyHostToDevice, ctx->stream));
-    ctx->h_sc[SC_NCH_S] = (u32)nts;
-    CK(hipMemcpyAsync(sc + SC_NCH_S, &ctx->h_sc[SC_NCH_S], 4, hipMemcpyHostToDevice, ctx->stream));
-    { const int e = hist(ctx->smp_descs.as<ChunkDesc>(), (const u32*)(sc + SC_NCH_S), nts, ctx->smp_mat.as<u32>()); if (e) return e; }
+    { const int e = hist(sp, ctx->smp_descs.as<ChunkDesc>(), ctx->smp_mat.as<u32>()); if (e) return e; }
     u64* mom = reinterpret_cast<u64*>(ctx->smp_mat.as<u32>() + ((Ms + 2) & ~(u64)1));
     hipLaunchKernelGGL(k_bin_moments, dim3((P + 3) / 4), dim3(256), 0, ctx->stream, (const u32*)ctx->smp_mat.as<u32>(), (u32)nts, P, mom);
     CKL("k_bin_moments");
@@ -566,6 +589,35 @@
     u64 stot = 0;
     for (u32 b = 0; b < P; ++b) stot += ctx->h_mom[2 * b];
     *ntiles_out = ntiles; *nts_out = nts; *stot_out = stot;
+    return DSKGPU_OK;
+}
+
+void order_segments2(dskgpu_ctx* ctx, const Plan& pl, const std::vector<double>& load) {
+    ctx->h_descs2.resize(pl.P1);
+    std::vector<u32> order(pl.P1);
+    for (u32 sgm = 0; sgm < pl.P1; ++sgm) order[sgm] = sgm;
+    double mean_work = 0.0; for (double w : load) mean_work += w; mean_work = std::max(1.0, mean_work / pl.P1);
+    auto wclass = [&](u32 a) { return (long long)(load[a] / (0.05 * mean_work)); };
+    std::stable_sort(order.begin(), order.end(), [&](u32 a, u32 b) { return wclass(a) > wclass(b); });
+    for (u32 i = 0; i < pl.P1; ++i) {
+        const u32 sgm = order[i];
+        ChunkDesc d; d.begin = ctx->h_boff[sgm]; d.end = ctx->h_boff[sgm + 1]; d.flat_base = sgm * pl.P2; d.stride = 1;
+        ctx->h_descs2[i] = d;
+    }
+}
+
+int pblk_slot(dskgpu_ctx* ctx, size_t bytes, char** out) {
+    dskgpu_ctx::ParamBlock& pb = ctx->pblk;
+    const u32 s = pb.next; pb.next ^= 1u;
+    if (pb.busy[s]) { CK(hipStreamSynchronize(ctx->stream)); pb.busy[0] = pb.busy[1] = false; }
+    if (pb.cap[s] < bytes) {
+        if (pb.host[s]) { CK(hipHostFree(pb.host[s])); pb.host[s] = nullptr; pb.cap[s] = 0; }
+        const size_t want = std::max<size_t>((bytes + bytes / 4 + 4095) & ~size_t(4095), 64u << 10);
+        CK(hipHostMalloc(reinterpret_cast<void**>(&pb.host[s]), want, hipHostMallocDefault));
+        pb.cap[s] = want;
+    }
+    pb.busy[s] = true;
+    *out = pb.host[s];
     return DSKGPU_OK;
 }
 
@@ -659,8 +711,8 @@
         const bool smp_rec = src.from_rec && rec_units != 0;
         if ((!src.from_rec || smp_rec) && rec_sample_ok && !ctx->tune.no_sample && !uniform1) {
             const u64 units = src.from_reads ? src.nwords : smp_rec ? rec_units : src.nkeys, tile = src.from_reads ? Tile<W>::WORDS : Tile<W>::KEYS;
-            auto hist = [&](const ChunkDesc* dd, const u32* d_nch, u64 n, u32* mat) {
-                return src.from_reads ? launch_hist<W, 0>(ctx, nullptr, dd, d_nch, n, mat, pl.d1, pl.P1) : launch_hist<W, 1>(ctx, d_keys_s, dd, d_nch, n, mat, pl.d1, pl.P1);
+            auto hist = [&](const DescSpec& sp, ChunkDesc* dout, u32* mat) {
+                return src.from_reads ? launch_hist<W, 0>(ctx, nullptr, nullptr, nullptr, sp.nch, mat, pl.d1, pl.P1, sp, dout) : launch_hist<W, 1>(ctx, d_keys_s, nullptr, nullptr, sp.nch, mat, pl.d1, pl.P1, sp, dout);
             };
             u64 ntiles = 0, nts = 0, stot = 0;
             { const int e = positional_sample(ctx, units, tile, pl.P1, hist, &ntiles, &nts, &stot); if (e) return e; }
@@ -701,9 +753,19 @@
         if (area < 8 || area * grid1 + tail >= 0xFFFF0000ull) ps.opt1 = false;
         else {
             o1.area = (u32)area; o1.dump = (u32)(area * grid1);
-            CK(ctx->boff.ensure(((size_t)pl.P1 + 1) * 4));
-            CK(hipMemcpyAsync(ctx->boff.p, ctx->h_boff.data(), ((size_t)pl.P1 + 1) * 4, hipMemcpyHostToDevice, ctx->stream));
-            o1.boff = ctx->boff.as<u32>();
+            const bool seg2 = pl.levels == 2 && ps.opt_cap;
+            if (seg2) order_segments2(ctx, pl, ps.load);
+            const size_t nd = seg2 ? (size_t)pl.P1 * sizeof(ChunkDesc) : 0, nbo = ((size_t)pl.P1 + 1) * 4;
+            char* hb = nullptr;
+            { const int e = pblk_slot(ctx, nd + nbo, &hb); if (e) return e; }
+            if (nd) std::memcpy(hb, ctx->h_descs2.data(), nd);
+            std::memcpy(hb + nd, ctx->h_boff.data(), nbo);
+            CK(ctx->pblk.dev.ensure(nd + nbo));
+            void* hb_dev = nullptr;
+            if (hipHostGetDevicePointer(&hb_dev, hb, 0) == hipSuccess && hb_dev) { ps.pb_src = static_cast<const u32*>(hb_dev); ps.pb_words = (u32)((nd + nbo) / 4); }
+            else { (void)hipGetLastError(); CK(hipMemcpyAsync(ctx->pblk.dev.p, hb, nd + nbo, hipMemcpyHostToDevice, ctx->stream)); }
+            if (seg2) ps.dd2 = ctx->pblk.dev.as<ChunkDesc>();
+            o1.boff = reinterpret_cast<const u32*>(ctx->pblk.dev.as<char>() + nd);
             CK(ctx->mat1.ensure((cells + 1) * 4));
             o1.fill = ctx->mat1.as<u32>();
             if (grid1 + 1 > SLICED_MAX) ps.opt1 = false;
@@ -751,9 +813,10 @@
         const u32 nh = ctx->cfg.histo_max + 1;
         u64 nzero = 0;
         if (pl.levels == 2 && ps.opt_cap) { nzero = ps.nregions + 1; CK(ctx->mat2.ensure((size_t)nzero * 4)); }
-        const u64 work = std::max<u64>(nh, nzero);
+        const u64 work = std::max<u64>(std::max<u64>(nh, nzero), std::max<u32>(ps.d1s.nch, ps.pb_words));
         hipLaunchKernelGGL(k_setup_pass, dim3((unsigned)std::min<u64>(1024, (work + 255) / 256)), dim3(256), 0, ctx->stream, ps.sc, hs, ctx->ghist.as<u64>(), nh, ctx->gstats.as<u64>(), 4u,
-                           nzero ? ctx->mat2.as<u32>() : (u32*)nullptr, nzero);
+                           nzero ? ctx->mat2.as<u32>() : (u32*)nullptr, nzero, ctx->descs1.as<ChunkDesc>(), ps.d1s,
+                           ps.pb_src, ps.pb_words, ctx->pblk.dev.as<u32>());
         CKL("k_setup_pass");
     }
     ctx->mark("setup");
@@ -814,18 +877,7 @@
         CK(ctx->mat2.ensure(((size_t)ps.nregions + 1) * 4));
         CK(ctx->chain_next.ensure(((size_t)ps.nregions + 1 + ps.max_ext + 1) * 4));
         if (ps.opt1) {
-            ctx->h_descs2.resize(pl.P1);
-            std::vector<u32> order(pl.P1);
-            for (u32 sgm = 0; sgm < pl.P1; ++sgm) order[sgm] = sgm;
-            double mean_work = 0.0; for (double w : ps.load) mean_work += w; mean_work = std::max(1.0, mean_work / pl.P1);
-            auto wclass = [&](u32 a) { return (long long)(ps.load[a] / (0.05 * mean_work)); };
-            std::stable_sort(order.begin(), order.end(), [&](u32 a, u32 b) { return wclass(a) > wclass(b); });
-            for (u32 i = 0; i < pl.P1; ++i) {
-                const u32 sgm = order[i];
-                ChunkDesc d; d.begin = ctx->h_boff[sgm]; d.end = ctx->h_boff[sgm + 1]; d.flat_base = sgm * pl.P2; d.stride = 1;
-                ctx->h_descs2[i] = d;
-            }
-            CK(hipMemcpyAsync(ctx->descs2.p, ctx->h_descs2.data(), (size_t)pl.P1 * sizeof(ChunkDesc), hipMemcpyHostToDevice, ctx->stream));
+            if (!ps.dd2) return fail(ctx, DSKGPU_E_STATE, "level 2 over block-owned slices without its segment order");
         } else {
             hipLaunchKernelGGL(k_plan, dim3(1), dim3(1024), 0, ctx->stream, ctx->mat1.as<u32>(), ps.nch1, pl.P1, 0x7FFFFFFFu, pl.P2,
                                ctx->seg.as<SegInfo>(), ctx->descs2.as<ChunkDesc>(), ps.sc + SC_NCH2, ps.sc + SC_MLEN2, 1u);
@@ -836,7 +888,7 @@
                    pl.F, ps.max_ext, ctx->chain_next.as<u32>(), ps.sc + SC_EXT, ctx->chain_next.as<u32>() + ps.nregions + 1, ps.sc + SC_NCHAINED,
                    ps.sc + SC_WORK2, nullptr};
         if (ctx->tune.verbose && ps.opt1) { CK(ctx->dbg.ensure((size_t)pl.P1 * 24)); os.dbg = ctx->dbg.as<unsigned long long>(); }
-        if (ps.opt1) rc = launch_scatter_al<W, 2, true, true>(ctx, ctx->bufA.as<typename KeyT<W>::T>(), ctx->descs2.as<ChunkDesc>(), ps.sc + SC_NCH2, (u64)pl.P1 * 2, nullptr,
+        if (ps.opt1) rc = launch_scatter_al<W, 2, true, true>(ctx, ctx->bufA.as<typename KeyT<W>::T>(), ps.dd2, ps.sc + SC_NCH2, (u64)pl.P1 * 2, nullptr,
                                                               ctx->bufB.as<typename KeyT<W>::T>(), pl.d2, pl.P2, os);
         else rc = launch_scatter_al<W, 2, true, false>(ctx, ctx->bufA.as<typename KeyT<W>::T>(), ctx->descs2.as<ChunkDesc>(), ps.sc + SC_NCH2, (u64)pl.P1 * 2, nullptr,
                                                        ctx->bufB.as<typename KeyT<W>::T>(), pl.d2, pl.P2, os);
@@ -911,16 +963,27 @@
         }
     }
     ctx->mark("count");
-    if (int e = run_scan(ctx, ctx->nsolid.as<u32>(), ps.sc + SC_F, pl.F)) return e;
-    ctx->mark("scan_solid");
     CK(ctx->back_dev.ensure(16 * 8));
     if (!ctx->back_host) CK(hipHostMalloc(reinterpret_cast<void**>(&ctx->back_host), 16 * 8, hipHostMallocDefault));
     const u32* nkp = ps.opt1 ? nullptr : (ps.opt_cap ? ctx->mat1.as<u32>() + (u64)pl.P1 * ps.nch1 : ctx->fstart.as<u32>() + pl.F);
-    hipLaunchKernelGGL(k_gather_back, dim3(1), dim3(64), 0, ctx->stream, (const u32*)ps.sc, (const u32*)(ctx->nsolid.as<u32>() + pl.F), nkp,
-                       (const u64*)ctx->gstats.as<u64>(), ctx->back_dev.as<u64>());
-    CKL("k_gather_back");
+    const u64 nb = std::max<u64>(1, ((u64)pl.F + SCAN_BLK - 1) / SCAN_BLK);
+    if (nb <= SCAN_BACK_MAXNB) {
+        CK(ctx->sums.ensure((nb + 1) * 4));
+        hipLaunchKernelGGL(k_scan_reduce, dim3((unsigned)nb), dim3(SCAN_NT), 0, ctx->stream, (const u32*)ctx->nsolid.as<u32>(), (const u32*)(ps.sc + SC_F), ctx->sums.as<u32>());
+        hipLaunchKernelGGL(k_scan_apply_back, dim3((unsigned)nb), dim3(SCAN_NT), 0, ctx->stream, ctx->nsolid.as<u32>(), (const u32*)(ps.sc + SC_F), (const u32*)ctx->sums.as<u32>(),
+                           (const u32*)ps.sc, nkp, (const u64*)ctx->gstats.as<u64>(), ctx->back_dev.as<u64>());
+        CKL("k_scan_apply_back");
+        ctx->mark("scan_solid");
+    } else {
+        if (int e = run_scan(ctx, ctx->nsolid.as<u32>(), ps.sc + SC_F, pl.F)) return e;
+        ctx->mark("scan_solid");
+        hipLaunchKernelGGL(k_gather_back, dim3(1), dim3(64), 0, ctx->stream, (const u32*)ps.sc, (const u32*)(ctx->nsolid.as<u32>() + pl.F), nkp,
+                           (const u64*)ctx->gstats.as<u64>(), ctx->back_dev.as<u64>());
+        CKL("k_gather_back");
+    }
     CK(hipMemcpyAsync(ctx->back_host, ctx->back_dev.p, 10 * 8, hipMemcpyDeviceToHost, ctx->stream));
     CK(hipStreamSynchronize(ctx->stream));
+    ctx->pblk.busy[0] = ctx->pblk.busy[1] = false;
     const u64* bh = ctx->back_host;
     ps.flags = (u32)bh[0]; ps.nsolid = (u32)bh[1]; if (!ps.opt1) ps.nkeys = (u32)bh[2];
     ps.ovf2 = (u32)bh[3]; ps.ovf1 = (u32)bh[4]; ps.ext = (u32)bh[5];
@@ -1091,7 +1154,7 @@
     DigitSpec ds{4u, G, 0u, ctx->cfg.world_size, npass, lo};
     std::vector<u64> slice(G, uslice);
     if (!ctx->tune.no_sample) {
-        auto hist = [&](const ChunkDesc* dd, const u32* d_nch, u64 n, u32* mat) { return launch_hist_m<1, 0, 4>(ctx, nullptr, dd, d_nch, n, mat, ds, G); };
+        auto hist = [&](const DescSpec& sp, ChunkDesc* dout, u32* mat) { return launch_hist_m<1, 0, 4>(ctx, nullptr, nullptr, nullptr, sp.nch, mat, ds, G, sp, dout); };
         u64 ntiles = 0, nts = 0, stot = 0;
         { const int e = positional_sample(ctx, nwords, Tile<1>::WORDS, G, hist, &ntiles, &nts, &stot); if (e) return e; }
         if (stot >= (u64)G * 4096) {
@@ -1652,12 +1715,13 @@
     (void)hipSetDevice(ctx->cfg.device);
     (void)hipStreamSynchronize(ctx->stream);
     DevBuf* bufs[] = {&ctx->reads_own, &ctx->raw_in, &ctx->raw_blk, &ctx->raw_boff, &ctx->raw_bstate, &ctx->raw_state, &ctx->packed, &ctx->inval, &ctx->bufA, &ctx->bufB, &ctx->mat1, &ctx->mat2, &ctx->sums,
-                      &ctx->descs1, &ctx->descs2, &ctx->seg, &ctx->fstart, &ctx->nsolid, &ctx->scalars, &ctx->ghist, &ctx->gstats, &ctx->chain_next, &ctx->smp_mat, &ctx->smp_descs, &ctx->boff, &ctx->hv_lut, &ctx->hv_collect, &ctx->hv_buf, &ctx->dbg, &ctx->l0buf,
+                      &ctx->descs1, &ctx->descs2, &ctx->seg, &ctx->fstart, &ctx->nsolid, &ctx->scalars, &ctx->ghist, &ctx->gstats, &ctx->chain_next, &ctx->smp_mat, &ctx->smp_descs, &ctx->pblk.dev, &ctx->boff, &ctx->hv_lut, &ctx->hv_collect, &ctx->hv_buf, &ctx->dbg, &ctx->l0buf,
                       &ctx->out_ab, &ctx->srt_ab, &ctx->srt_tmp,
                       &ctx->srt_idx, &ctx->srt_idx2, &ctx->srt_k, &ctx->srt_k2, &ctx->abund2, &ctx->acc_ab, &ctx->u_val,
                       &ctx->s_val, &ctx->m_flag, &ctx->m_pos, &ctx->m_sum, &ctx->gh2d,
                       &ctx->sk_sums, &ctx->sk_cbase, &ctx->sk_keys, &ctx->cur_state, &ctx->smp_keys, &ctx->back_dev};
     if (ctx->back_host) (void)hipHostFree(ctx->back_host);
+    for (int i = 0; i < 2; ++i) if (ctx->pblk.host[i]) (void)hipHostFree(ctx->pblk.host[i]);
     ctx->rs.release();
     ctx->sender.release(); ctx->l0_sender.release();
     ctx->query.release();
diff --git a/dsk_amd/csrc/engine.h b/dsk_amd/csrc/engine.h
--- a/dsk_amd/csrc/engine.h
+++ b/dsk_amd/csrc/engine.h
@@ -235,9 +235,10 @@
     RowSort rs;
     DevBuf smp_keys;
     DevBuf smp_mat, smp_descs, boff;
+    struct ParamBlock { char* host[2] = {nullptr, nullptr}; size_t cap[2] = {0, 0}; bool busy[2] = {false, false}; u32 next = 0; DevBuf dev; } pblk;
     DevBuf dbg, l0buf; DevBuf hv_lut, hv_collect, hv_buf;
-    std::vector<unsigned char> h_hv_lut; std::vector<u32> h_hv_cnt, h_hv_step; std::vector<u64> h_hv_coll, h_hv_keys;
-    std::vector<ChunkDesc> h_descs_s, h_descs1, h_descs2; std::vector<u64> h_cbeg; std::vector<u32> h_boff; std::vector<u64> h_mom;
+    std::vector<unsigned char> h_hv_lut; std::vector<u32> h_hv_cnt; std::vector<u64> h_hv_coll, h_hv_keys;
+    std::vector<ChunkDesc> h_descs1, h_descs2; std::vector<u64> h_cbeg; std::vector<u32> h_boff; std::vector<u64> h_mom;
     DevBuf out_w[4], srt_w[4], acc_w[4];
     DevBuf out_ab, srt_ab, srt_tmp, srt_idx, srt_idx2, srt_k, srt_k2, abund2, acc_ab;
     u64 max_keys_per_pass = 0;
diff --git a/dsk_amd/csrc/kernels.h b/dsk_amd/csrc/kernels.h
--- a/dsk_amd/csrc/kernels.h
+++ b/dsk_amd/csrc/kernels.h
@@ -142,12 +142,13 @@
 __global__ __launch_bounds__(SC_NT) void k_hist(const u64* __restrict__ packed, const u32* __restrict__ inval,
                                                 const typename KeyT<W>::T* __restrict__ keys,
                                                 const ChunkDesc* __restrict__ descs, const u32* __restrict__ d_nchunks,
-                                                u32* __restrict__ matrix, int k, DigitSpec ds, u32 P) {
+                                                u32* __restrict__ matrix, int k, DigitSpec ds, u32 P, DescSpec sp, ChunkDesc* __restrict__ descs_out) {
     __shared__ u32 lh[MAX_BINS + 1];
     constexpr int KPT = Tile<W>::KPT;
-    const u32 nchunks = *d_nchunks;
+    const u32 nchunks = descs ? *d_nchunks : sp.nch;
     for (u32 g = blockIdx.x; g < nchunks; g += gridDim.x) {
-        const ChunkDesc d = descs[g];
+        const ChunkDesc d = descs ? descs[g] : chunk_desc(sp, g);
+        if (!descs && descs_out && threadIdx.x == 0) descs_out[g] = d;
         for (u32 b = threadIdx.x; b <= P; b += SC_NT) lh[b] = 0;
         __syncthreads();
         const u64 step = SRC == 0 ? Tile<W>::WORDS : Tile<W>::KEYS;
@@ -2063,19 +2064,19 @@
 #define HV_SLOTS 16
 #define HV_COLLECT 2048
 #define HV_BLOCK_KEYS 32
+struct HvSteps { u32 v[HV_SLOTS]; };
 template <int W, int SRC, int MODE>
 __global__ __launch_bounds__(SC_NT) void k_collect_heavy(const u64* __restrict__ packed, const u32* __restrict__ inval, const typename KeyT<W>::T* __restrict__ keys,
-                                                         const ChunkDesc* __restrict__ descs, const u32* __restrict__ d_nchunks, int k, DigitSpec ds, u32 P,
-                                                         const unsigned char* __restrict__ lut, u32* __restrict__ kept, typename KeyT<W>::T* __restrict__ out, const u32* __restrict__ keep_step) {
+                                                         const ChunkDesc* __restrict__ descs, u32 nchunks, int k, DigitSpec ds, u32 P,
+                                                         const unsigned char* __restrict__ lut, u32* __restrict__ kept, typename KeyT<W>::T* __restrict__ out, HvSteps keep_step) {
     typedef typename KeyT<W>::T Key;
     constexpr int KPT = Tile<W>::KPT;
     __shared__ unsigned char slut[MAX_BINS + 8];
     __shared__ u32 lcnt[HV_SLOTS], lstep[HV_SLOTS];
     const int lane = threadIdx.x & 63;
     for (u32 b = threadIdx.x; b < P; b += SC_NT) slut[b] = lut[b];
-    if (threadIdx.x < HV_SLOTS) { const u32 st = keep_step[threadIdx.x]; lstep[threadIdx.x] = st; lcnt[threadIdx.x] = (blockIdx.x * 7919u) % st; }
+    if (threadIdx.x < HV_SLOTS) { const u32 st = keep_step.v[threadIdx.x]; lstep[threadIdx.x] = st; lcnt[threadIdx.x] = (blockIdx.x * 7919u) % st; }
     __syncthreads();
-    const u32 nchunks = *d_nchunks;
     for (u32 g = blockIdx.x; g < nchunks; g += gridDim.x) {
         const ChunkDesc d = descs[g];
         const u64 step = SRC == 0 ? Tile<W>::WORDS : Tile<W>::KEYS;
diff --git a/dsk_amd/csrc/layouts.h b/dsk_amd/csrc/layouts.h
--- a/dsk_amd/csrc/layouts.h
+++ b/dsk_amd/csrc/layouts.h
@@ -46,6 +46,36 @@
     u32 stride;
 };
 
+struct DescSpec { u64 n_units, ntiles, tile; u32 tpc, nch; u64 sq; u32 sr; };
+__host__ __device__ inline ChunkDesc chunk_desc(const DescSpec& s, u32 g) {
+    ChunkDesc d;
+    if (s.tpc) {
+        d.begin = (u64)g * s.tpc * s.tile;
+        const u64 e = ((u64)g + 1) * s.tpc * s.tile;
+        d.end = e < s.n_units ? e : s.n_units;
+        if (d.begin > d.end) d.begin = d.end;
+    } else {
+        const u64 t = (u64)g * s.sq + (g * s.sr) / s.nch;
+        d.begin = t * s.tile;
+        const u64 e = (t + 1) * s.tile;
+        d.end = e < s.n_units ? e : s.n_units;
+    }
+    d.flat_base = g; d.stride = s.nch;
+    return d;
+}
+inline DescSpec level1_spec(u64 n_units, u64 tile, u64 max_chunks) {
+    const u64 ntiles = (n_units + tile - 1) / tile > 1 ? (n_units + tile - 1) / tile : 1;
+    u64 nch = ntiles < max_chunks ? ntiles : max_chunks;
+    const u64 tpc = (ntiles + nch - 1) / nch;
+    nch = (ntiles + tpc - 1) / tpc;
+    return DescSpec{n_units, ntiles, tile, (u32)tpc, (u32)nch, 0ull, 0u};
+}
+inline DescSpec sample_spec(u64 n_units, u64 tile) {
+    const u64 ntiles = (n_units + tile - 1) / tile > 1 ? (n_units + tile - 1) / tile : 1;
+    const u32 nch = (u32)(ntiles < 1024 ? ntiles : 1024);
+    return DescSpec{n_units, ntiles, tile, 0u, nch, ntiles / nch, (u32)(ntiles % nch)};
+}
+
 #define SK_MAX_OWNERS 64
 #define SK_BUCKETS 4096
 struct SkParams {
```

Result: slower. 26.72 billion (-3.2%).
